# Banus/pano360

Hardware: AMD Instinct MI355X
Metric: blended megapixels/sec (multiband) (higher is better)
Workload: dtype f32; 1 GPU; cfg3: 32 synthetic 3840x2160 frames per image set, spherical warp + multiband blend L=5, native resolution (MAX_RESOLUTION uncapped); frames=32

## Files before the change

include/pano360.h:

```cpp
#ifndef PANO360_H
#define PANO360_H

#include <stddef.h>
#include <stdint.h>

#ifdef __cplusplus
extern "C" {
#endif

#define PANO_OK 0
#define PANO_EINVAL (-1)
#define PANO_EHIP (-2)
#define PANO_ELIMIT (-3)
#define PANO_ESOLVE (-4)

#define PANO_MAX_TAPS 129
#define PANO_MAX_LEVELS 8
#define PANO_TAP_LEAD 7
#define PANO_TAP_PAD 40
#ifndef PANO_INTERIOR_BLOCK
#define PANO_INTERIOR_BLOCK 4
#endif

typedef struct pano_patch {
    float *planes;
    uint8_t *mask;
    float *blurred;
    float *scratch;
    int32_t y0, x0, h, w;
    int32_t vy0, vx0, vh, vw;
    int32_t ay0, ax0, ah, aw;
    int32_t vpitch, apitch;
    int32_t index;
    int32_t tiles_off;
} pano_patch;

typedef struct pano_layout {
    int64_t planes_floats;
    int64_t blurred_floats;
    int64_t scratch_floats;
    int32_t n_records, n_tiles;
    int32_t max_vw, max_vh, max_aw, max_ah;
    int32_t missing;
} pano_layout;

typedef struct pano_camera {
    double proj[9];
    const uint8_t *frame;
    const double *hat_x;
    const double *hat_y;
    int32_t sh, sw;
    int32_t y0, x0, h, w;
} pano_camera;

typedef struct pano_pair {
    double minv[9];
    int32_t i, j;
} pano_pair;

typedef struct pano_sift_keypoint {
    float x, y;
    float size;
    float angle;
    float response;
    int32_t octave;
    int32_t r, c;
} pano_sift_keypoint;


const char *pano_version(void);
const char *pano_last_error(void);
int pano_device_count(void);
int pano_pitch(int w);
int pano_interior_block(void);

typedef struct pano_ctx pano_ctx;
#define PANO_OPT_BLUR_KERNEL 0
#define PANO_OPT_OWN_PRUNE 1
#define PANO_OPT_BLUR_SEGMENTS 2
#define PANO_OPT_BLUR_LEAN 3
#define PANO_OPT_STITCH_STREAMS 4
#define PANO_OPT_STITCH_ASYNC 5
#define PANO_OPT_BLUR_SEG_LEN 6
#define PANO_OPT_SIFT_GRAPH 7
#define PANO_OPT_LEVEL_CLASSES 8
#define PANO_OPT_COUNT 9
#define PANO_BLUR_MFMA 0
#define PANO_BLUR_VALU 1
int pano_ctx_create(int device, void *stream, pano_ctx **out);
int pano_ctx_destroy(pano_ctx *ctx);
int pano_ctx_set_stream(pano_ctx *ctx, void *stream);
int pano_ctx_set_option(pano_ctx *ctx, int option, int value);
int pano_ctx_get_option(const pano_ctx *ctx, int option, int *value);

int pano_timing_enable(pano_ctx *ctx, int on);
int pano_kernel_count(void);
const char *pano_kernel_name(int kid);
int pano_timing_read(pano_ctx *ctx, int kid, double *total_ms, int *launches);

int pano_add_weights(pano_ctx *ctx, const uint8_t *frame, int h, int w,
                     const float *lut255, const double *hat_x, const double *hat_y,
                     float *rgba);

int pano_warp_spherical(pano_ctx *ctx, const uint8_t *frame, int sh, int sw,
                        const double *proj, const double *sin_t, const double *cos_t,
                        const double *tan_p, const float *lut255, const double *hat_x,
                        const double *hat_y, int gx0, int gy0, int pw, int ph,
                        float *planes, uint8_t *mask, float *map_x, float *map_y);

int pano_warp_windows(pano_ctx *ctx, const pano_camera *cams, const pano_patch *patches,
                      int n, int max_vw, int max_vh, const double *sin_t,
                      const double *cos_t, const double *tan_p, const float *lut,
                      int lut_stride, const uint8_t *need);

int pano_ownership(pano_ctx *ctx, const pano_patch *patches, int n, int H, int W,
                   int16_t *owner, uint8_t *valid);

int pano_ownership_cameras(pano_ctx *ctx, const pano_camera *cams, int n, int H, int W,
                           int xs0, int xs1, const double *sin_t, const double *cos_t,
                           const double *tan_p, int16_t *owner, uint8_t *valid);

int pano_owned_regions(pano_ctx *ctx, const int16_t *owner, int H, int W, int xs0, int xs1,
                       int n, int min_gap, int max_spans, uint8_t *marks,
                       int32_t *regions);

int pano_ownership_regions(pano_ctx *ctx, const pano_camera *cams, int n, int H, int W,
                           int xs0, int xs1, const double *sin_t, const double *cos_t,
                           const double *tan_p, int16_t *owner, uint8_t *valid,
                           int min_gap, int max_spans, uint8_t *marks, int32_t *regions);

int pano_blur_tile_grid(const pano_ctx *ctx);
int pano_blur_tiles(pano_ctx *ctx, const pano_patch *patches, int n, int max_aw,
                    int max_ah, int W, int radius, const uint8_t *interior,
                    uint8_t *tile_flags, uint8_t *warp_need);
int pano_multiband_blur_prepare(pano_ctx *ctx, const pano_patch *patches, int n,
                                int max_aw, int max_ah, int W, const uint8_t *interior,
                                uint8_t *tile_flags);
int pano_multiband_blur(pano_ctx *ctx, const pano_patch *patches, int n, int max_aw,
                        int max_vh, int max_ah, const int16_t *owner, int W,
                        const float *taps, const int *ntaps, int n_blur,
                        const uint8_t *interior, uint8_t *tile_flags);

int pano_interior_map(pano_ctx *ctx, const int16_t *owner, int H, int W, int xs0, int xs1,
                      int radius, int16_t *block_owner, uint8_t *interior);
int pano_interior_classes(pano_ctx *ctx, const int16_t *owner, int H, int W, int xs0, int xs1,
                          const int *radii, int n_radii, int16_t *block_owner, uint8_t *interior,
                          uint8_t *classes);

int pano_layout_windows(int tile_grid, const int32_t *regions, int n, int max_spans,
                        const int32_t *rects, const uint8_t *have, int radius,
                        int xs0, int xs1, int n_blur, pano_patch *records, int cap,
                        pano_layout *out);
int pano_layout_place(pano_patch *records, int n_records, void *planes, void *blurred,
                      void *scratch);

int pano_multiband_compose(pano_ctx *ctx, const pano_patch *patches, int n, int H, int W,
                           int xs0, int xs1, int n_levels, const int16_t *owner,
                           const uint8_t *valid, const uint8_t *interior,
                           const uint8_t *classes, const pano_camera *cams,
                           const double *sin_t, const double *cos_t, const double *tan_p,
                           const float *lut, int lut_stride, uint8_t *mosaic,
                           float *mosaic_f32);

int pano_blend_cameras(pano_ctx *ctx, const pano_camera *cams, int n, int H, int W,
                       int xs0, int xs1, int linear, const double *sin_t,
                       const double *cos_t, const double *tan_p, const float *lut,
                       int lut_stride, uint8_t *mosaic, uint8_t *valid);

int pano_overlap_blocks(int h, int w);
int pano_overlap_stats(pano_ctx *ctx, const pano_camera *cams, const pano_pair *pairs,
                       int n_pairs, int h, int w, int bw0, const float *lut255,
                       double *partials, double *stats);

int pano_linear_blend(pano_ctx *ctx, const pano_patch *patches, int n, int H, int W,
                      uint8_t *mosaic);

int pano_no_blend(pano_ctx *ctx, const pano_patch *patches, int n, int H, int W,
                  uint8_t *mosaic);

int pano_crop_rect(pano_ctx *ctx, const uint8_t *valid, int H, int W, int32_t *heights,
                   int64_t *result);

int pano_blur_plane(pano_ctx *ctx, const float *src, float *dst, float *tmp, int h, int w,
                    int pitch, const float *taps, int ntaps);

int pano_pyr_down(pano_ctx *ctx, const float *src, int h, int w, float *dst);

int pano_gray_u8(pano_ctx *ctx, const uint8_t *bgr, int h, int w, float *out);
int pano_scale_step(pano_ctx *ctx, const float *src, int h, int w, const float *taps, int ntaps,
                    float *dst, float *dog);
int pano_scale_space(pano_ctx *ctx, const uint8_t *frame, int h, int w, int n_octaves,
                     int n_layers, const float *taps, const int *ntaps, float *const *gauss,
                     float *const *dog, float *work);
int pano_resize_up2(pano_ctx *ctx, const float *src, int h, int w, float *dst);
int pano_decimate2(pano_ctx *ctx, const float *src, int h, int w, float *dst);
int pano_subtract(pano_ctx *ctx, const float *a, const float *b, size_t n, float *out);

int pano_pyr_down_image(pano_ctx *ctx, const void *src, int h, int w, int c, int is_f64,
                        void *dst);
int pano_pyr_up_image(pano_ctx *ctx, const void *src, int sh, int sw, int c, int is_f64,
                      const void *other, int mode, void *dst, int oh, int ow);
int pano_u8_to_f32(pano_ctx *ctx, const uint8_t *src, size_t n, float *dst);
int pano_laplacian_mix(pano_ctx *ctx, const float *la, const float *lb, const void *gm, size_t n,
                       int is_f64, void *out);
int pano_clip_u8(pano_ctx *ctx, const void *src, size_t n, int is_f64, uint8_t *dst);

#define PANO_POISSON_CHUNK 32
int pano_poisson_blend(pano_ctx *ctx, const uint8_t *src, uint8_t *tgt, const uint8_t *mask,
                       int h, int w, int c, double rtol, int max_iters, double *solution,
                       int32_t *iters, double *resid);

#define PANO_SEAM_U8 0
#define PANO_SEAM_I16 1
#define PANO_SEAM_I32 2
#define PANO_SEAM_F32 3
#define PANO_SEAM_F64 4
#define PANO_SEAM_RESIDENT_CELLS 81408
#define PANO_SEAM_BATCH 64
int pano_seam_levels(pano_ctx *ctx, const void *img1, const void *img2, int dtype, int h, int w,
                     int c, int shrink, int16_t *level, int32_t *bad);
int pano_seam_flood(pano_ctx *ctx, const int16_t *level, int rows, int cols, int border,
                    int path, int8_t *labels, int32_t *stats);
int pano_seam_mask(pano_ctx *ctx, const int8_t *labels, int rows, int cols,
                   const int32_t *xtab, const int32_t *ytab, uint8_t *mask, int h, int w);
int pano_alpha_blend(pano_ctx *ctx, const void *img1, const void *img2, int dtype,
                     const void *mask, int mask_f64, int64_t mask_sy, int64_t mask_sx,
                     int64_t mask_sc, int h, int w, int c, uint8_t *out);

int pano_resize_u8(pano_ctx *ctx, const uint8_t *src, int sh, int sw, int c,
                   const int32_t *xtab, const int32_t *ytab, uint8_t *dst, int oh, int ow);

int pano_sift_extrema(pano_ctx *ctx, const float *dog, int rows, int cols, int octave,
                      int n_layers, float contrast_thr, float edge_thr, float sigma,
                      pano_sift_keypoint *cands, int *count, int max_cands);
int pano_sift_orient(pano_ctx *ctx, const float *const *gauss, const int *dims,
                     int n_layers, const pano_sift_keypoint *cands, const int *n_cands,
                     int max_cands, pano_sift_keypoint *kpts, int *count, int max_kpts);
int pano_sift_describe(pano_ctx *ctx, const float *const *gauss, const int *dims,
                       int first_octave, const pano_sift_keypoint *kpts, int n,
                       const int *n_dev, float *desc);
size_t pano_sift_sort_work_bytes(int n);
int pano_sift_sort_unique(pano_ctx *ctx, const pano_sift_keypoint *kpts, int n, const int *n_dev,
                          int first_octave, void *work, pano_sift_keypoint *out, int *n_out);

typedef struct pano_sift_args {
    const uint8_t *frame;
    uint8_t *frame_copy;
    int32_t h, w, n_octaves, n_layers;
    const float *taps;
    const int32_t *ntaps;
    float *const *gauss;
    float *const *dog;
    float *work;
    int32_t detect;
    float contrast_thr, edge_thr, sigma;
    int32_t first_octave, max_keypoints;
    const float *const *gauss_dev;
    const int32_t *dims_dev;
    pano_sift_keypoint *cands, *kpts;
    int32_t *counts;
    void *sort_work;
    float *desc;
} pano_sift_args;
int pano_sift_detect(pano_ctx *ctx, const pano_sift_args *args);
int pano_sift_detect_replaying(const pano_ctx *ctx);

size_t pano_knn2_work_bytes(int nq, int nt, int d);
int pano_knn2(pano_ctx *ctx, const float *query, int nq, const float *train, int nt, int d,
              float scale, void *work, int32_t *idx, float *dist, int *rescans);

int pano_match_pack(pano_ctx *ctx, const int32_t *idx, const float *dist, int nq, double ratio,
                    const float *kp_query, const float *kp_train, int nt, float *pts,
                    int32_t *match, int32_t *count);

size_t pano_hom_ransac_work_bytes(int n_pairs, int max_iters);
int pano_hom_ransac(pano_ctx *ctx, const float *pts, const int32_t *offsets, const int32_t *counts,
                    int n_pairs, int max_iters, float thresh, uint64_t seed, void *work,
                    double *hom, uint8_t *mask, int32_t *n_inliers, int32_t *hyp_inliers);

size_t pano_ba_work_bytes(int n_pairs);
int pano_ba_residuals(pano_ctx *ctx, const double *rows, const int32_t *pairs, int n_pairs,
                      const double *hom, double *ssq);
int pano_ba_normal(pano_ctx *ctx, const double *rows, const int32_t *pairs, int n_pairs,
                   const int32_t *slot, int n_active, const double *jtab, const double *hom_r,
                   double lambda, void *work, double *jtj, double *jtr);

#define PANO_JPEG_FIELDS 32
#define PANO_JPEG_CHUNK 1024
#define PANO_JPEG_SUBSEQ 1024
#define PANO_JPEG_HUFF_BYTES 1424
enum {
    PANO_JD_W, PANO_JD_H, PANO_JD_NC, PANO_JD_HMAX, PANO_JD_VMAX, PANO_JD_MCUX, PANO_JD_MCUY,
    PANO_JD_RI,
    PANO_JD_NINT,
    PANO_JD_BPM,
    PANO_JD_ORIENT, PANO_JD_DATA_OFF, PANO_JD_DATA_LEN, PANO_JD_TAB_OFF,
    PANO_JD_CHUNK0,
    PANO_JD_INT0,
    PANO_JD_SUB0,
    PANO_JD_BLK0, PANO_JD_PIX0,
    PANO_JD_DST_OFF,
    PANO_JD_PLANE0, PANO_JD_PLANE1, PANO_JD_PLANE2,
    PANO_JD_PITCH0, PANO_JD_PITCH1, PANO_JD_PITCH2,
    PANO_JD_OUT_OFF,
    PANO_JD_COMP_U,
    PANO_JD_SAMP,
    PANO_JD_TABSEL
};
enum {
    PANO_JB_N, PANO_JB_CHUNKS, PANO_JB_INTS, PANO_JB_SUBS, PANO_JB_BLOCKS, PANO_JB_PIXELS,
    PANO_JB_OUT_BYTES, PANO_JB_W_KEPT, PANO_JB_W_RST, PANO_JB_W_KEPTX, PANO_JB_W_RSTX,
    PANO_JB_W_DSTLEN, PANO_JB_W_ISTART, PANO_JB_W_IEND, PANO_JB_W_INSUB, PANO_JB_W_ISUBX,
    PANO_JB_W_STATE0, PANO_JB_W_STATE1, PANO_JB_W_CNTX, PANO_JB_W_FLAG, PANO_JB_W_COEF,
    PANO_JB_WORK_BYTES, PANO_JB_PACKED_BYTES
};
int pano_jpeg_decode(pano_ctx *ctx, const int64_t *desc, int n, const uint8_t *packed,
                     int64_t packed_bytes, void *work, int64_t work_bytes, uint8_t *out,
                     int64_t out_bytes);

#define PANO_JPEG_MAX_SIDE 65500
#define PANO_JPEG_BGR 1
size_t pano_jpeg_encode_work_bytes(int h, int w, int subsampling);
int pano_jpeg_encode(pano_ctx *ctx, const uint8_t *img, int h, int w, int64_t pitch, int flags,
                     int subsampling, const uint8_t *qt, void *work, int64_t work_bytes,
                     const uint8_t **stream, int64_t *stream_bytes);

#define PANO_EGROW 1
typedef struct pano_stitch_args {
    const pano_camera *cams;
    const int32_t *rects;
    const uint8_t *have;
    const double *sin_t, *cos_t, *tan_p;
    const float *lut;
    const float *taps;
    const int32_t *ntaps;
    int16_t *owner;
    uint8_t *valid;
    uint8_t *marks;
    int32_t *regions;
    int32_t *regions_host;
    int16_t *block_owner;
    uint8_t *interior;
    pano_patch *records_host;
    pano_patch *table;
    float *planes, *blurred, *scratch;
    uint8_t *tile_flags, *need;
    uint8_t *mosaic;
    float *mosaic_f32;
    int64_t planes_floats, blurred_floats, scratch_floats;
    int32_t n, H, W, xs0, xs1, own0, own1;
    int32_t lut_stride, n_levels, radius, shortcut, warp_need, max_spans, min_gap;
    int32_t cap_records, cap_tiles;
    int32_t used_need;
    int32_t trust_layout;
    uint8_t *classes;
    pano_layout layout;
} pano_stitch_args;
int pano_stitch_multiband(pano_ctx *ctx, pano_stitch_args *args, int resume);
int pano_stitch_verify(pano_ctx *ctx);
int pano_stitch_counts(const pano_ctx *ctx, int *device_layouts, int *fallbacks);

#ifdef __cplusplus
}
#endif
#endif
```

pano360_amd/_lib.py:

```python
import ctypes as C
import os
import subprocess

_HERE = os.path.dirname(os.path.abspath(__file__))
LIB_PATH = os.environ.get("PANO_LIB") or os.path.join(_HERE, "libpano360_hip.so")

MAX_TAPS = 129
MAX_LEVELS = 8
TAP_LEAD = 7
TAP_PAD = 40
OPT_BLUR_KERNEL, OPT_OWN_PRUNE, OPT_BLUR_SEGMENTS, OPT_BLUR_LEAN, OPT_STITCH_STREAMS = 0, 1, 2, 3, 4
OPT_STITCH_ASYNC = 5
OPT_BLUR_SEG_LEN = 6
OPT_SIFT_GRAPH = 7
OPT_LEVEL_CLASSES = 8
BLUR_MFMA, BLUR_VALU = 0, 1


class PanoError(RuntimeError):
    """A C-ABI call returned a negative status."""


class Patch(C.Structure):
    _fields_ = [("planes", C.c_void_p), ("mask", C.c_void_p),
                ("blurred", C.c_void_p), ("scratch", C.c_void_p),
                ("y0", C.c_int32), ("x0", C.c_int32), ("h", C.c_int32), ("w", C.c_int32),
                ("vy0", C.c_int32), ("vx0", C.c_int32), ("vh", C.c_int32), ("vw", C.c_int32),
                ("ay0", C.c_int32), ("ax0", C.c_int32), ("ah", C.c_int32), ("aw", C.c_int32),
                ("vpitch", C.c_int32), ("apitch", C.c_int32),
                ("index", C.c_int32), ("tiles_off", C.c_int32)]


class Layout(C.Structure):
    _fields_ = [("planes_floats", C.c_int64), ("blurred_floats", C.c_int64),
                ("scratch_floats", C.c_int64), ("n_records", C.c_int32), ("n_tiles", C.c_int32),
                ("max_vw", C.c_int32), ("max_vh", C.c_int32), ("max_aw", C.c_int32),
                ("max_ah", C.c_int32), ("missing", C.c_int32)]


class SiftArgs(C.Structure):
    _fields_ = [("frame", C.c_void_p), ("frame_copy", C.c_void_p),
                ("h", C.c_int32), ("w", C.c_int32), ("n_octaves", C.c_int32), ("n_layers", C.c_int32),
                ("taps", C.c_void_p), ("ntaps", C.c_void_p), ("gauss", C.c_void_p),
                ("dog", C.c_void_p), ("work", C.c_void_p), ("detect", C.c_int32),
                ("contrast_thr", C.c_float), ("edge_thr", C.c_float), ("sigma", C.c_float),
                ("first_octave", C.c_int32), ("max_keypoints", C.c_int32),
                ("gauss_dev", C.c_void_p), ("dims_dev", C.c_void_p), ("cands", C.c_void_p),
                ("kpts", C.c_void_p), ("counts", C.c_void_p), ("sort_work", C.c_void_p),
                ("desc", C.c_void_p)]


class StitchArgs(C.Structure):
    _fields_ = ([(k, C.c_void_p) for k in (
        "cams", "rects", "have", "sin_t", "cos_t", "tan_p", "lut", "taps", "ntaps", "owner",
        "valid", "marks", "regions", "regions_host", "block_owner", "interior", "records_host",
        "table", "planes", "blurred", "scratch", "tile_flags", "need", "mosaic", "mosaic_f32")]
        + [(k, C.c_int64) for k in ("planes_floats", "blurred_floats", "scratch_floats")]
        + [(k, C.c_int32) for k in (
            "n", "H", "W", "xs0", "xs1", "own0", "own1", "lut_stride", "n_levels", "radius",
            "shortcut", "warp_need", "max_spans", "min_gap", "cap_records", "cap_tiles",
            "used_need", "trust_layout")]
        + [("classes", C.c_void_p), ("layout", Layout)])


EINVAL = -1
ESOLVE = -4
SEAM_DTYPES = {"uint8": 0, "int16": 1, "int32": 2, "float32": 3, "float64": 4}
SEAM_RESIDENT_CELLS = 81408
EGROW = 1


class Pair(C.Structure):
    _fields_ = [("minv", C.c_double * 9), ("i", C.c_int32), ("j", C.c_int32)]


class SiftKeypoint(C.Structure):
    _fields_ = [("x", C.c_float), ("y", C.c_float), ("size", C.c_float), ("angle", C.c_float),
                ("response", C.c_float), ("octave", C.c_int32), ("r", C.c_int32), ("c", C.c_int32)]


class Camera(C.Structure):
    _fields_ = [("proj", C.c_double * 9), ("frame", C.c_void_p),
                ("hat_x", C.c_void_p), ("hat_y", C.c_void_p),
                ("sh", C.c_int32), ("sw", C.c_int32),
                ("y0", C.c_int32), ("x0", C.c_int32), ("h", C.c_int32), ("w", C.c_int32)]


_vp, _i = C.c_void_p, C.c_int
_SIGNATURES = {
    "pano_version": (C.c_char_p, []),
    "pano_last_error": (C.c_char_p, []),
    "pano_device_count": (_i, []),
    "pano_pitch": (_i, [_i]),
    "pano_interior_block": (_i, []),
    "pano_ctx_create": (_i, [_i, _vp, C.POINTER(C.c_void_p)]),
    "pano_ctx_destroy": (_i, [_vp]),
    "pano_ctx_set_stream": (_i, [_vp, _vp]),
    "pano_ctx_set_option": (_i, [_vp, _i, _i]),
    "pano_ctx_get_option": (_i, [_vp, _i, C.POINTER(C.c_int)]),
    "pano_timing_enable": (_i, [_vp, _i]),
    "pano_kernel_count": (_i, []),
    "pano_kernel_name": (C.c_char_p, [_i]),
    "pano_timing_read": (_i, [_vp, _i, C.POINTER(C.c_double), C.POINTER(C.c_int)]),
    "pano_add_weights": (_i, [_vp, _vp, _i, _i, _vp, _vp, _vp, _vp]),
    "pano_warp_spherical": (_i, [_vp, _vp, _i, _i, _vp, _vp, _vp, _vp, _vp, _vp, _vp, _i, _i, _i,
                                 _i, _vp, _vp, _vp, _vp]),
    "pano_warp_windows": (_i, [_vp, _vp, _vp, _i, _i, _i, _vp, _vp, _vp, _vp, _i, _vp]),
    "pano_blur_tiles": (_i, [_vp, _vp, _i, _i, _i, _i, _i, _vp, _vp, _vp]),
    "pano_ownership": (_i, [_vp, _vp, _i, _i, _i, _vp, _vp]),
    "pano_ownership_cameras": (_i, [_vp, _vp, _i, _i, _i, _i, _i, _vp, _vp, _vp, _vp, _vp]),
    "pano_owned_regions": (_i, [_vp, _vp, _i, _i, _i, _i, _i, _i, _i, _vp, _vp]),
    "pano_ownership_regions": (_i, [_vp, _vp, _i, _i, _i, _i, _i, _vp, _vp, _vp, _vp, _vp,
                                    _i, _i, _vp, _vp]),
    "pano_multiband_blur": (_i, [_vp, _vp, _i, _i, _i, _i, _vp, _i, _vp, C.POINTER(C.c_int), _i,
                                 _vp, _vp]),
    "pano_multiband_blur_prepare": (_i, [_vp, _vp, _i, _i, _i, _i, _vp, _vp]),
    "pano_layout_windows": (_i, [_i, _vp, _i, _i, _vp, _vp, _i, _i, _i, _i, _vp, _i, _vp]),
    "pano_layout_place": (_i, [_vp, _i, _vp, _vp, _vp]),
    "pano_interior_map": (_i, [_vp, _vp, _i, _i, _i, _i, _i, _vp, _vp]),
    "pano_interior_classes": (_i, [_vp, _vp, _i, _i, _i, _i, _vp, _i, _vp, _vp, _vp]),
    "pano_multiband_compose": (_i, [_vp, _vp, _i, _i, _i, _i, _i, _i, _vp, _vp, _vp, _vp, _vp, _vp,
                                    _vp, _vp, _vp, _i, _vp, _vp]),
    "pano_blend_cameras": (_i, [_vp, _vp, _i, _i, _i, _i, _i, _i, _vp, _vp, _vp, _vp, _i, _vp,
                                _vp]),
    "pano_blur_tile_grid": (_i, [_vp]),
    "pano_overlap_blocks": (_i, [_i, _i]),
    "pano_overlap_stats": (_i, [_vp, _vp, _vp, _i, _i, _i, _i, _vp, _vp, _vp]),
    "pano_linear_blend": (_i, [_vp, _vp, _i, _i, _i, _vp]),
    "pano_no_blend": (_i, [_vp, _vp, _i, _i, _i, _vp]),
    "pano_crop_rect": (_i, [_vp, _vp, _i, _i, _vp, _vp]),
    "pano_blur_plane": (_i, [_vp, _vp, _vp, _vp, _i, _i, _i, _vp, _i]),
    "pano_pyr_down": (_i, [_vp, _vp, _i, _i, _vp]),
    "pano_gray_u8": (_i, [_vp, _vp, _i, _i, _vp]),
    "pano_scale_step": (_i, [_vp, _vp, _i, _i, _vp, _i, _vp, _vp]),
    "pano_scale_space": (_i, [_vp, _vp, _i, _i, _i, _i, _vp, _vp, _vp, _vp, _vp]),
    "pano_resize_up2": (_i, [_vp, _vp, _i, _i, _vp]),
    "pano_decimate2": (_i, [_vp, _vp, _i, _i, _vp]),
    "pano_subtract": (_i, [_vp, _vp, _vp, C.c_size_t, _vp]),
    "pano_pyr_down_image": (_i, [_vp, _vp, _i, _i, _i, _i, _vp]),
    "pano_pyr_up_image": (_i, [_vp, _vp, _i, _i, _i, _i, _vp, _i, _vp, _i, _i]),
    "pano_u8_to_f32": (_i, [_vp, _vp, C.c_size_t, _vp]),
    "pano_laplacian_mix": (_i, [_vp, _vp, _vp, _vp, C.c_size_t, _i, _vp]),
    "pano_clip_u8": (_i, [_vp, _vp, C.c_size_t, _i, _vp]),
    "pano_poisson_blend": (_i, [_vp, _vp, _vp, _vp, _i, _i, _i, C.c_double, _i, _vp, _vp, _vp]),
    "pano_seam_levels": (_i, [_vp, _vp, _vp, _i, _i, _i, _i, _i, _vp, _vp]),
    "pano_seam_flood": (_i, [_vp, _vp, _i, _i, _i, _i, _vp, _vp]),
    "pano_seam_mask": (_i, [_vp, _vp, _i, _i, _vp, _vp, _vp, _i, _i]),
    "pano_alpha_blend": (_i, [_vp, _vp, _vp, _i, _vp, _i, C.c_int64, C.c_int64, C.c_int64, _i, _i,
                              _i, _vp]),
    "pano_resize_u8": (_i, [_vp, _vp, _i, _i, _i, _vp, _vp, _vp, _i, _i]),
    "pano_sift_extrema": (_i, [_vp, _vp, _i, _i, _i, _i, C.c_float, C.c_float, C.c_float, _vp,
                               _vp, _i]),
    "pano_sift_orient": (_i, [_vp, _vp, _vp, _i, _vp, _vp, _i, _vp, _vp, _i]),
    "pano_sift_describe": (_i, [_vp, _vp, _vp, _i, _vp, _i, _vp, _vp]),
    "pano_sift_sort_work_bytes": (C.c_size_t, [_i]),
    "pano_sift_sort_unique": (_i, [_vp, _vp, _i, _vp, _i, _vp, _vp, _vp]),
    "pano_knn2_work_bytes": (C.c_size_t, [_i, _i, _i]),
    "pano_knn2": (_i, [_vp, _vp, _i, _vp, _i, _i, C.c_float, _vp, _vp, _vp, _vp]),
    "pano_hom_ransac_work_bytes": (C.c_size_t, [_i, _i]),
    "pano_hom_ransac": (_i, [_vp, _vp, _vp, _vp, _i, _i, C.c_float, C.c_uint64, _vp, _vp, _vp, _vp,
                             _vp]),
    "pano_match_pack": (_i, [_vp, _vp, _vp, _i, C.c_double, _vp, _vp, _i, _vp, _vp, _vp]),
    "pano_ba_work_bytes": (C.c_size_t, [_i]),
    "pano_ba_residuals": (_i, [_vp, _vp, _vp, _i, _vp, _vp]),
    "pano_ba_normal": (_i, [_vp, _vp, _vp, _i, _vp, _i, _vp, _vp, C.c_double, _vp, _vp, _vp]),
    "pano_jpeg_decode": (_i, [_vp, _vp, _i, _vp, C.c_int64, _vp, C.c_int64, _vp, C.c_int64]),
    "pano_jpeg_encode_work_bytes": (C.c_size_t, [_i, _i, _i]),
    "pano_jpeg_encode": (_i, [_vp, _vp, _i, _i, C.c_int64, _i, _i, _vp, _vp, C.c_int64,
                             C.POINTER(C.c_void_p), C.POINTER(C.c_int64)]),
    "pano_sift_detect": (_i, [_vp, _vp]),
    "pano_sift_detect_replaying": (_i, [_vp]),
    "pano_stitch_multiband": (_i, [_vp, _vp, _i]),
    "pano_stitch_counts": (_i, [_vp, _vp, _vp]),
    "pano_stitch_verify": (_i, [_vp]),
}
EXPORTS = tuple(_SIGNATURES)


def sources_digest():
    import hashlib
    src = os.path.join(_HERE, "csrc")
    files = sorted(os.path.join(src, f) for f in os.listdir(src)
                   if f.endswith((".hip", ".h", ".inc")) or f == "Makefile")
    files.append(os.path.join(os.path.dirname(_HERE), "include", "pano360.h"))
    h = hashlib.sha256()
    for path in files:
        if not os.path.exists(path):
            continue
        h.update(os.path.basename(path).encode() + b"\0")
        with open(path, "rb") as fid:
            h.update(fid.read())
    return h.hexdigest()


BUILD_RECORD = os.path.join(_HERE, "csrc", ".build_stamp")


def build(force=False):
    import json
    src = os.path.join(_HERE, "csrc")
    digest = sources_digest()
    have = None
    try:
        with open(BUILD_RECORD) as fid:
            have = json.load(fid).get("sources_sha256")
    except (OSError, ValueError):
        pass
    full = force or have != digest or not os.path.exists(LIB_PATH)
    before = os.path.getmtime(LIB_PATH) if os.path.exists(LIB_PATH) else None
    cmd = ["make", "-C", src, "-s", "-j4"] + (["-B"] if full else [])
    subprocess.check_call(cmd)
    after = os.path.getmtime(LIB_PATH)
    mode = "full" if full else ("incremental" if after != before else "up to date")
    with open(BUILD_RECORD, "w") as fid:
        json.dump({"sources_sha256": digest, "mode": mode}, fid)
    return LIB_PATH


_lib = None


def lib():
    global _lib
    if _lib is None:
        if not os.path.exists(LIB_PATH):
            raise PanoError(
                f"{LIB_PATH} is missing: build it with "
                "`python -c 'import __graft_entry__ as g; g.build()'` "
                "(there is no CPU fallback)")
        import torch
        handle = C.CDLL(LIB_PATH)
        for name, (res, args) in _SIGNATURES.items():
            fn = getattr(handle, name)
            fn.restype, fn.argtypes = res, args
        _lib = handle
    return _lib


def check(status, what):
    if status != 0:
        msg = lib().pano_last_error().decode("utf-8", "replace")
        raise PanoError(f"{what} failed ({status}): {msg}")
```

pano360_amd/csrc/api.hip:

```cpp
#include <stdarg.h>
#include <stdio.h>
#include <stdlib.h>
#include <string.h>

#include <vector>

#include "common.h"
#include "layout.h"

static thread_local char g_error[512] = "";

void pano_set_error(const char *fmt, ...) {
    va_list ap;
    va_start(ap, fmt);
    vsnprintf(g_error, sizeof(g_error), fmt, ap);
    va_end(ap);
}

extern "C" const char *pano_version(void) { return "pano360_hip 0.1 (gfx950)"; }

extern "C" const char *pano_last_error(void) { return g_error; }

extern "C" int pano_device_count(void) {
    int n = 0;
    if (hipGetDeviceCount(&n) != hipSuccess) {
        (void)hipGetLastError();
        return 0;
    }
    return n;
}

extern "C" int pano_pitch(int w) { return pano_pitch_of(w); }

extern "C" int pano_interior_block(void) { return PANO_INTERIOR_BLOCK; }

extern "C" int pano_ctx_create(int device, void *stream, pano_ctx **out) {
    PANO_REQUIRE(out, "pano_ctx_create: null output");
    *out = nullptr;
    PANO_REQUIRE(device >= 0 && device < pano_device_count(), "pano_ctx_create: no device %d",
                 device);
    PANO_HIP(hipSetDevice(device));
    if (int rc = pano_blur_mfma_opt_in()) return rc;
    if (int rc = pano_blur_valu_opt_in()) return rc;
    pano_ctx *ctx = new pano_ctx();
    ctx->device = device;
    ctx->stream = (hipStream_t)stream;
    ctx->opt[PANO_OPT_BLUR_KERNEL] = PANO_BLUR_MFMA;
    ctx->opt[PANO_OPT_OWN_PRUNE] = 1;
    ctx->opt[PANO_OPT_BLUR_SEGMENTS] = 1;
    ctx->opt[PANO_OPT_BLUR_LEAN] = 1;
    ctx->opt[PANO_OPT_STITCH_STREAMS] = 1;
    ctx->opt[PANO_OPT_STITCH_ASYNC] = 0;
    ctx->opt[PANO_OPT_BLUR_SEG_LEN] = 0;
    ctx->opt[PANO_OPT_SIFT_GRAPH] = 1;
    ctx->opt[PANO_OPT_LEVEL_CLASSES] = 0;
    *out = ctx;
    return PANO_OK;
}

int pano_ctx_enter(pano_ctx *ctx) {
    if (!ctx->in_stitch) ctx->geom_valid = false;
    PANO_HIP(hipSetDevice(ctx->device));
    return PANO_OK;
}

static void timing_clear(pano_ctx *ctx) {
    for (int k = 0; k < PK_COUNT; ++k) {
        for (hipEvent_t e : ctx->t_begin[k]) (void)hipEventDestroy(e);
        for (hipEvent_t e : ctx->t_end[k]) (void)hipEventDestroy(e);
        ctx->t_begin[k].clear();
        ctx->t_end[k].clear();
    }
}

static void tap_set_free(PanoTapSet &ts) {
    if (ts.taps) (void)hipFree(ts.taps);
    if (ts.tables) (void)hipFree(ts.tables);
    if (ts.ready) (void)hipEventDestroy(ts.ready);
    free(ts.host);
    ts.taps = nullptr;
    ts.tables = nullptr;
    ts.ready = nullptr;
    ts.host = nullptr;
}

extern "C" int pano_ctx_destroy(pano_ctx *ctx) {
    if (!ctx) return PANO_OK;
    PANO_HIP(hipSetDevice(ctx->device));
    if (hipStreamSynchronize(ctx->stream) != hipSuccess) {
        (void)hipGetLastError();
        (void)hipDeviceSynchronize();
    }
    timing_clear(ctx);
    for (PanoTapSet &ts : ctx->tap_sets) tap_set_free(ts);
    if (ctx->item_buf) (void)hipFree(ctx->item_buf);
    if (ctx->item_counter) (void)hipFree(ctx->item_counter);
    if (ctx->sift_raw) (void)hipFree(ctx->sift_raw);
    if (ctx->enc_dev) (void)hipFree(ctx->enc_dev);
    if (ctx->enc_out) (void)hipFree(ctx->enc_out);
    if (ctx->enc_host) (void)hipHostFree(ctx->enc_host);
    if (ctx->poisson_dev) (void)hipFree(ctx->poisson_dev);
    if (ctx->poisson_host) (void)hipHostFree(ctx->poisson_host);
    if (ctx->seam_dev) (void)hipFree(ctx->seam_dev);
    if (ctx->seam_host) (void)hipHostFree(ctx->seam_host);
    pano_sift_graphs_free(ctx);
    if (ctx->lay_sum_host) (void)hipHostFree(ctx->lay_sum_host);
    if (ctx->lay_rects_dev) (void)hipFree(ctx->lay_rects_dev);
    if (ctx->lay_have_dev) (void)hipFree(ctx->lay_have_dev);
    if (ctx->side) {
        (void)hipStreamSynchronize(ctx->side);
        (void)hipStreamDestroy(ctx->side);
    }
    if (ctx->ev_fork) (void)hipEventDestroy(ctx->ev_fork);
    if (ctx->ev_join) (void)hipEventDestroy(ctx->ev_join);
    if (ctx->ev_regions) (void)hipEventDestroy(ctx->ev_regions);
    if (ctx->ev_upload) (void)hipEventDestroy(ctx->ev_upload);
    if (ctx->ev_copy) (void)hipEventDestroy(ctx->ev_copy);
    delete ctx;
    return PANO_OK;
}

int pano_ctx_side_stream(pano_ctx *ctx) {
    if (!ctx->ev_regions) PANO_HIP(hipEventCreateWithFlags(&ctx->ev_regions, hipEventDisableTiming));
    if (!ctx->ev_upload) PANO_HIP(hipEventCreateWithFlags(&ctx->ev_upload, hipEventDisableTiming));
    if (!ctx->ev_fork) PANO_HIP(hipEventCreateWithFlags(&ctx->ev_fork, hipEventDisableTiming));
    if (!ctx->ev_join) PANO_HIP(hipEventCreateWithFlags(&ctx->ev_join, hipEventDisableTiming));
    if (!ctx->ev_copy) PANO_HIP(hipEventCreateWithFlags(&ctx->ev_copy, hipEventDisableTiming));
    if (!ctx->side) PANO_HIP(hipStreamCreateWithFlags(&ctx->side, hipStreamNonBlocking));
    return PANO_OK;
}

extern "C" int pano_ctx_set_stream(pano_ctx *ctx, void *stream) {
    PANO_REQUIRE(ctx, "pano_ctx_set_stream: null context");
    if ((hipStream_t)stream != ctx->stream) ctx->geom_valid = false;
    ctx->stream = (hipStream_t)stream;
    return PANO_OK;
}

extern "C" int pano_ctx_set_option(pano_ctx *ctx, int option, int value) {
    PANO_REQUIRE(ctx, "pano_ctx_set_option: null context");
    PANO_REQUIRE(option >= 0 && option < PANO_OPT_COUNT, "pano_ctx_set_option: option %d", option);
    if (option == PANO_OPT_BLUR_KERNEL)
        PANO_REQUIRE(value == PANO_BLUR_MFMA || value == PANO_BLUR_VALU,
                     "pano_ctx_set_option: blur kernel %d", value);
    else if (option == PANO_OPT_STITCH_ASYNC)
        PANO_REQUIRE(value >= 0 && value <= 2, "pano_ctx_set_option: option %d takes 0, 1 or 2", option);
    else if (option == PANO_OPT_OWN_PRUNE)
        PANO_REQUIRE(value >= 0 && value <= 3, "pano_ctx_set_option: option %d takes 0 .. 3", option);
    else if (option == PANO_OPT_BLUR_SEG_LEN)
        PANO_REQUIRE(value == -1 || value == 0 || (value >= 4 && value <= 2047),
                     "pano_ctx_set_option: option %d takes -1, 0 or 4 .. 2047", option);
    else
        PANO_REQUIRE(value == 0 || value == 1, "pano_ctx_set_option: option %d takes 0 or 1", option);
    const bool changed = ctx->opt[option] != value;
    ctx->opt[option] = value;
    ctx->prepared_table = ctx->flags_table = ctx->list_table = nullptr;
    ctx->geom_valid = false;
    if (changed && option == PANO_OPT_BLUR_KERNEL)
        ctx->lay_prev_valid = ctx->lay_prev_verified = false;
    return PANO_OK;
}

extern "C" int pano_ctx_get_option(const pano_ctx *ctx, int option, int *value) {
    PANO_REQUIRE(ctx && value, "pano_ctx_get_option: null pointer");
    PANO_REQUIRE(option >= 0 && option < PANO_OPT_COUNT, "pano_ctx_get_option: option %d", option);
    *value = ctx->opt[option];
    return PANO_OK;
}

static uint64_t tap_hash(const float *taps, const int *ntaps, int n, size_t floats) {
    uint64_t h = 1469598103934665603ull;
    auto eat = [&](const void *p, size_t bytes) {
        const unsigned char *b = (const unsigned char *)p;
        for (size_t i = 0; i < bytes; ++i) h = (h ^ b[i]) * 1099511628211ull;
    };
    eat(&n, sizeof(n));
    eat(ntaps, n * sizeof(int));
    eat(taps, floats * sizeof(float));
    return h;
}

#define PANO_TAP_SETS_MAX 64
int pano_ctx_tap_set(pano_ctx *ctx, const float *taps, const int *ntaps, int n, size_t table_bytes,
                     PanoTapSet **out, bool *fresh) {
    size_t floats = 0;
    for (int k = 0; k < n; ++k) floats += (size_t)ntaps[k] + PANO_TAP_PAD;
    const uint64_t key = tap_hash(taps, ntaps, n, floats);
    *fresh = false;
    for (PanoTapSet &ts : ctx->tap_sets)
        if (ts.key == key && ts.n == n && !memcmp(ts.ntaps, ntaps, n * sizeof(int)) &&
            ts.floats == floats && !memcmp(ts.host, taps, floats * sizeof(float))) {
            ts.used = ++ctx->tick;
            if (ctx->stream != ts.built_on) PANO_HIP(hipStreamWaitEvent(ctx->stream, ts.ready, 0));
            if (table_bytes && !ts.tables) {
                PANO_HIP(hipMalloc((void **)&ts.tables, table_bytes));
                *fresh = true;
            }
            *out = &ts;
            return PANO_OK;
        }
    if (ctx->tap_sets.size() >= PANO_TAP_SETS_MAX) {
        size_t old = 0;
        for (size_t i = 1; i < ctx->tap_sets.size(); ++i)
            if (ctx->tap_sets[i].used < ctx->tap_sets[old].used) old = i;
        PANO_HIP(hipDeviceSynchronize());
        tap_set_free(ctx->tap_sets[old]);
        ctx->tap_sets.erase(ctx->tap_sets.begin() + old);
    }
    PanoTapSet ts = {};
    ts.key = key;
    ts.n = n;
    memcpy(ts.ntaps, ntaps, n * sizeof(int));
    ts.floats = floats;
    ts.host = (float *)malloc(floats * sizeof(float));
    PANO_REQUIRE(ts.host, "pano_ctx_tap_set: out of host memory");
    memcpy(ts.host, taps, floats * sizeof(float));
    PANO_HIP(hipMalloc((void **)&ts.taps, floats * sizeof(float)));
    PANO_HIP(hipMemcpyAsync(ts.taps, taps, floats * sizeof(float), hipMemcpyHostToDevice,
                            ctx->stream));
    PANO_HIP(hipEventCreateWithFlags(&ts.ready, hipEventDisableTiming));
    PANO_HIP(hipEventRecord(ts.ready, ctx->stream));
    ts.built_on = ctx->stream;
    if (table_bytes) {
        PANO_HIP(hipMalloc((void **)&ts.tables, table_bytes));
        *fresh = true;
    }
    ts.used = ++ctx->tick;
    ctx->tap_sets.push_back(ts);
    *out = &ctx->tap_sets.back();
    return PANO_OK;
}

int pano_ctx_tap_set_built(pano_ctx *ctx, PanoTapSet *set) {
    PANO_HIP(hipEventRecord(set->ready, ctx->stream));
    set->built_on = ctx->stream;
    return PANO_OK;
}

static const char *const g_kernel_names[] = {
    "add_weights_kernel", "warp_spherical_kernel", "ownership_kernel", "blur_rows_kernel",
    "blur_cols_kernel",   "multiband_compose_kernel", "linear_blend_kernel",
    "no_blend_kernel",    "crop_heights_kernel", "crop_rows_kernel", "pyr_down_kernel",
    "ownership_cameras_kernel", "owned_boxes_kernel", "warp_windows_kernel",
    "blend_cameras_kernel", "owned_spans_kernel",
    "block_owner_kernel", "tile_flags_kernel", "overlap_stats_kernel",
    "blur_mfma_kernel", "sift_extrema_kernel", "sift_orient_kernel", "sift_describe_kernel",
    "scale_step_kernel", "knn2_kernel", "blur_lean_kernel", "blur_lean5_kernel",
    "ransac_score_kernel", "ransac_finish_kernel", "match_pack_kernel",
    "ba_residual_kernel", "ba_pair_kernel", "ba_assemble_kernel",
    "jpeg_destuff_kernel", "jpeg_scan_kernel", "jpeg_intervals_kernel", "jpeg_huff_sync_kernel",
    "jpeg_huff_write_kernel", "jpeg_dc_kernel", "jpeg_idct_kernel", "jpeg_pixels_kernel",
    "jpeg_enc_blocks_kernel", "jpeg_enc_count_kernel", "jpeg_enc_scan_kernel", "jpeg_enc_emit_kernel",
    "jpeg_enc_stuff_kernel"};
static_assert(sizeof(g_kernel_names) / sizeof(g_kernel_names[0]) == PK_COUNT,
              "one name per PanoKernelId, in enum order");

void pano_timing_edge(pano_ctx *ctx, int kid, hipStream_t stream, bool begin) {
    hipEvent_t ev;
    if (hipEventCreate(&ev) != hipSuccess) return;
    (void)hipEventRecord(ev, stream);
    (begin ? ctx->t_begin : ctx->t_end)[kid].push_back(ev);
}

extern "C" int pano_timing_enable(pano_ctx *ctx, int on) {
    PANO_REQUIRE(ctx, "pano_timing_enable: null context");
    timing_clear(ctx);
    ctx->timing_on = on != 0;
    return PANO_OK;
}

extern "C" int pano_kernel_count(void) { return PK_COUNT; }

extern "C" const char *pano_kernel_name(int kid) {
    return kid >= 0 && kid < PK_COUNT ? g_kernel_names[kid] : "";
}

extern "C" int pano_timing_read(pano_ctx *ctx, int kid, double *total_ms, int *launches) {
    PANO_REQUIRE(ctx && kid >= 0 && kid < PK_COUNT && total_ms && launches,
                 "pano_timing_read: bad argument");
    double sum = 0.0;
    const size_t nb = ctx->t_begin[kid].size(), ne = ctx->t_end[kid].size();
    const size_t n = ne < nb ? ne : nb;
    for (size_t i = 0; i < n; ++i) {
        PANO_HIP(hipEventSynchronize(ctx->t_end[kid][i]));
        float ms = 0.f;
        PANO_HIP(hipEventElapsedTime(&ms, ctx->t_begin[kid][i], ctx->t_end[kid][i]));
        sum += ms;
    }
    *total_ms = sum;
    *launches = (int)n;
    return PANO_OK;
}

extern "C" int pano_layout_windows(int tile_grid, const int32_t *regions, int n, int max_spans,
                                   const int32_t *rects, const uint8_t *have, int radius,
                                   int xs0, int xs1, int n_blur, pano_patch *records, int cap,
                                   pano_layout *out) {
    PANO_REQUIRE(regions && rects && records && out, "pano_layout_windows: null pointer");
    PANO_REQUIRE(tile_grid == 0 || tile_grid == 32, "pano_layout_windows: tile grid %d", tile_grid);
    PANO_REQUIRE(n >= 0 && max_spans >= 1 && radius >= 0 && n_blur >= 0 && cap >= 0,
                 "pano_layout_windows: bad argument");
    const bool grid32 = tile_grid == 32;
    const int stride = 5 + 2 * max_spans;
    pano_layout lay = {};
    lay.missing = 0;
    long planes = 0, blurred = 0, scratch = 0, tiles = 0;
    int k = 0;
    for (int i = 0; i < n; ++i) {
        const int32_t *rg = regions + (size_t)i * stride;
        const int spans = rg[4] < max_spans ? rg[4] : max_spans;
        for (int sp = 0; sp < spans; ++sp) {
            pano_patch rec;
            LayoutSizes sz;
            if (!layout_record(rg, sp, rects + 4 * i, i, radius, xs0, xs1, n_blur, grid32, rec, sz))
                continue;
            PANO_REQUIRE(k < cap, "pano_layout_windows: more than %d records", cap);
            if (have && !have[i]) ++lay.missing;
            pano_patch &r = records[k++];
            r = rec;
            PANO_REQUIRE(layout_record_fits(r),
                         "pano_layout_windows: a plane of record %d exceeds 2 GiB", k - 1);
            r.planes = (float *)(uintptr_t)planes;
            r.blurred = (float *)(uintptr_t)(blurred + sz.lead);
            r.scratch = (float *)(uintptr_t)scratch;
            PANO_REQUIRE(tiles < (1l << 31), "pano_layout_windows: tile count overflow");
            r.tiles_off = (int)tiles;
            planes += sz.planes;
            blurred += sz.blurred;
            scratch += sz.scratch;
            tiles += sz.tiles;
            lay.max_vw = r.vw > lay.max_vw ? r.vw : lay.max_vw;
            lay.max_vh = r.vh > lay.max_vh ? r.vh : lay.max_vh;
            lay.max_aw = r.aw > lay.max_aw ? r.aw : lay.max_aw;
            lay.max_ah = r.ah > lay.max_ah ? r.ah : lay.max_ah;
        }
    }
    lay.n_records = k;
    lay.n_tiles = (int)tiles;
    lay.planes_floats = planes;
    lay.blurred_floats = blurred + 32;
    lay.scratch_floats = scratch;
    *out = lay;
    return PANO_OK;
}

extern "C" int pano_layout_place(pano_patch *records, int n_records, void *planes, void *blurred,
                                 void *scratch) {
    PANO_REQUIRE(records || n_records == 0, "pano_layout_place: null pointer");
    uintptr_t bbase = (uintptr_t)blurred;
    bbase += (uintptr_t)(-(intptr_t)bbase) % 128;
    for (int k = 0; k < n_records; ++k) {
        pano_patch &r = records[k];
        r.planes = (float *)planes + (uintptr_t)r.planes;
        r.blurred = blurred ? (float *)bbase + (uintptr_t)r.blurred : nullptr;
        r.scratch = scratch ? (float *)scratch + (uintptr_t)r.scratch : nullptr;
    }
    return PANO_OK;
}
```

pano360_amd/csrc/blur.hip:

```cpp
#include "common.h"

#define ROW_TW 512
#define ROW_RMAX 64
#define ROW_TILE (ROW_TW + 2 * ROW_RMAX + 16)
#define ROW_LDS (ROW_TILE + (ROW_TILE / 8) * 4 + 8)

#define COL_TW 64
#define COL_TH 128
#define COL_STEPS(ntaps) (((ntaps) + 7 + 7) & ~7)

struct LevelDesc {
    const float *wz;
    int ntaps;
    int start;
    int steps;
};

struct Levels {
    LevelDesc lv[PANO_MAX_LEVELS];
    int n;
    int rmax;
    int need;
};

// ... 34 lines not shown
    const int y = blockIdx.y * 4 + wv;
    const int yc = y < p.vh ? y : p.vh - 1;
    float *tile = s_row[wv];
    const float *__restrict__ src =
        c == alpha_ch ? nullptr : p.planes + (size_t)c * p.vh * p.vpitch;
    const int16_t *__restrict__ orow =
        owner + (size_t)(p.y0 + p.vy0 + yc) * W + p.x0;

    for (int i0 = lane; i0 < L.need; i0 += 256) {
        float v[4];
#pragma unroll
        for (int u = 0; u < 4; ++u) {
            const int i = i0 + 64 * u < L.need ? i0 + 64 * u : L.need - 1;
            const int pcol = reflect_101(p.ax0 + xt - L.rmax + i, p.w);
            if (src) {
                int vc = pcol - p.vx0;
                vc = vc < 0 ? 0 : (vc >= p.vw ? p.vw - 1 : vc);
                v[u] = src[(size_t)yc * p.vpitch + vc];
            } else {
                v[u] = orow[pcol] == p.index ? 1.0f : 0.0f;
            }
        }
#pragma unroll
        for (int u = 0; u < 4; ++u)
            if (i0 + 64 * u < L.need) tile[row_pos(i0 + 64 * u)] = v[u];
    }
    __syncthreads();

    const float *base = tile + 12 * lane;
    const int x = xt + 8 * lane;
    for (int k = 0; k < L.n; ++k) {
        const kptr_f32 wz = (kptr_f32)(uintptr_t)L.lv[k].wz;
        const int start = L.lv[k].start, steps = L.lv[k].steps;
        float acc[8];
#pragma unroll
        for (int o = 0; o < 8; ++o) acc[o] = 0.0f;
        for (int s = 0; s < steps; s += 2) {
            const int q0 = start + 4 * s, q1 = q0 + 4;
            const float4 va = *(const float4 *)(base + q0 + ((q0 >> 3) << 2));
            const float4 vb = *(const float4 *)(base + q1 + ((q1 >> 3) << 2));
            float wq[15];
#pragma unroll
            for (int j = 0; j < 15; ++j) wq[j] = wz[4 * s + j];
            const float in[8] = {va.x, va.y, va.z, va.w, vb.x, vb.y, vb.z, vb.w};
#pragma unroll
            for (int i = 0; i < 8; ++i) {
#pragma unroll
                for (int o = 0; o < 8; ++o)
                    acc[o] = __builtin_fmaf(wq[i + 7 - o], in[i], acc[o]);
            }
        }
        if (y < p.vh) {
            float *d = p.scratch + ((size_t)(k * nch + c) * p.vh + y) * p.apitch + x;
            if (x + 8 <= p.apitch) {
                *(float4 *)d = make_float4(acc[0], acc[1], acc[2], acc[3]);
                *(float4 *)(d + 4) = make_float4(acc[4], acc[5], acc[6], acc[7]);
            } else {
#pragma unroll
                for (int o = 0; o < 8; ++o)
                    if (x + o < p.aw) d[o] = acc[o];
            }
        }
    }
}

struct ColTrip {
    float w[15];
    float4 v[8];
};

__device__ __forceinline__ void col_trip_load(ColTrip &t, const float *base, kptr_f32 wz, int q) {
#pragma unroll
    for (int j = 0; j < 15; ++j) t.w[j] = wz[q + j];
#pragma unroll
    for (int s = 0; s < 8; ++s) t.v[s] = *(const float4 *)(base + (q + s) * COL_TW);
}

__device__ __forceinline__ void col_trip_fma(const ColTrip &t, float4 (&acc)[8]) {
#pragma unroll
    for (int s = 0; s < 8; ++s) {
#pragma unroll
        for (int o = 0; o < 8; ++o) {
            const float wgt = t.w[s + 7 - o];
            acc[o].x = __builtin_fmaf(wgt, t.v[s].x, acc[o].x);
            acc[o].y = __builtin_fmaf(wgt, t.v[s].y, acc[o].y);
            acc[o].z = __builtin_fmaf(wgt, t.v[s].z, acc[o].z);
            acc[o].w = __builtin_fmaf(wgt, t.v[s].w, acc[o].w);
        }
    }
}

template <bool TABLE>
__global__ __launch_bounds__(256) void blur_cols_kernel(
    const pano_patch *__restrict__ table, pano_patch single, int nch, int level,
    const float *wz_global, int ntaps, const uint8_t *__restrict__ flags) {
    const kptr_f32 wz = (kptr_f32)(uintptr_t)wz_global;
    extern __shared__ __attribute__((aligned(16))) float s_col[];
    const int pid = blockIdx.z / nch, c = blockIdx.z - pid * nch;
    const pano_patch p = TABLE ? table[pid] : single;
    const int x0 = blockIdx.x * COL_TW, y0 = blockIdx.y * COL_TH;
    if (x0 >= p.aw || y0 >= p.ah) return;
    if (p.h > 2 * (ntaps >> 1) + 2 && !col_tile_active(flags, p, blockIdx.x, blockIdx.y)) return;

    const float *__restrict__ src = p.scratch + (size_t)(level * nch + c) * p.vh * p.apitch;
    float *__restrict__ dst = p.blurred + (size_t)(level * nch + c) * p.ah * p.apitch;
    const int tx = threadIdx.x, ty = threadIdx.y;
    const int R = ntaps >> 1;
    const int steps = COL_STEPS(ntaps);
    const int rows = 8 * 15 + steps;
    const int x = x0 + 4 * tx;

    const int xl = x < p.apitch ? x : p.apitch - 4;
    const int wave4 = (ty >> 2) << 2;
    for (int r0 = 0; r0 < rows; r0 += 16) {
        const int r = r0 + ty;
        int vr = reflect_101(p.ay0 + y0 - R + (r < rows ? r : rows - 1), p.h) - p.vy0;
        vr = vr < 0 ? 0 : (vr >= p.vh ? p.vh - 1 : vr);
        __builtin_amdgcn_global_load_lds(
            (const __attribute__((address_space(1))) void *)(src + (size_t)vr * p.apitch + xl),
            (__attribute__((address_space(3))) void *)(s_col + (r0 + wave4) * COL_TW), 16, 0, 0);
    }
    __syncthreads();

    float4 acc[8];
#pragma unroll
    for (int o = 0; o < 8; ++o) acc[o] = make_float4(0.f, 0.f, 0.f, 0.f);
    const float *base = s_col + (8 * ty) * COL_TW + 4 * tx;
    for (int q = 0; q < steps; q += 8) {
        ColTrip a;
        col_trip_load(a, base, wz, q);
        col_trip_fma(a, acc);
    }
    if (x < p.apitch) {
#pragma unroll
        for (int o = 0; o < 8; ++o) {
            const int y = y0 + 8 * ty + o;
            if (y < p.ah) *(float4 *)(dst + (size_t)y * p.apitch + x) = acc[o];
        }
    }
}

__global__ __launch_bounds__(64) void tile_flags_kernel(const pano_patch *__restrict__ table,
                                                        const uint8_t *__restrict__ interior,
                                                        int W8, uint8_t *__restrict__ flags) {
    const pano_patch p = table[blockIdx.z];
    const int ntx = (p.aw + COL_TW - 1) / COL_TW, nty = (p.ah + COL_TH - 1) / COL_TH;
    const int tx = blockIdx.x, ty = blockIdx.y;
    if (tx >= ntx || ty >= nty) return;
    const int gx0 = p.x0 + p.ax0 + tx * COL_TW, gy0 = p.y0 + p.ay0 + ty * COL_TH;
    int gx1 = gx0 + COL_TW, gy1 = gy0 + COL_TH;
    const int ax1 = p.x0 + p.ax0 + p.aw, ay1 = p.y0 + p.ay0 + p.ah;
    gx1 = gx1 < ax1 ? gx1 : ax1;
    gy1 = gy1 < ay1 ? gy1 : ay1;
    const int bx0 = gx0 / PANO_INTERIOR_BLOCK, bx1 = (gx1 - 1) / PANO_INTERIOR_BLOCK;
    const int by0 = gy0 / PANO_INTERIOR_BLOCK, by1 = (gy1 - 1) / PANO_INTERIOR_BLOCK;
    const int nbx = bx1 - bx0 + 1, total = nbx * (by1 - by0 + 1);
    bool active = false;
    for (int i = threadIdx.x; i < total; i += 64)
        active |= interior[(size_t)(by0 + i / nbx) * W8 + bx0 + i % nbx] == 0;
    if (__ballot(active) && threadIdx.x == 0) flags[p.tiles_off + ty * ntx + tx] = 1;
    if (!__ballot(active) && threadIdx.x == 0) flags[p.tiles_off + ty * ntx + tx] = 0;
}

static int check_taps(int ntaps, const char *who) {
    PANO_REQUIRE(ntaps >= 1 && (ntaps & 1) && ntaps <= PANO_MAX_TAPS,
                 "%s: aperture %d must be odd and within [1, %d]", who, ntaps, PANO_MAX_TAPS);
    return PANO_OK;
}

static int make_levels(const float *taps, const int *ntaps, int n_blur, Levels *L,
                       const float **col_wz, const char *who) {
    PANO_REQUIRE(n_blur >= 1 && n_blur < PANO_MAX_LEVELS, "%s: %d blur levels", who, n_blur);
    L->n = n_blur;
    L->rmax = 0;
    for (int k = 0; k < n_blur; ++k) {
        if (int rc = check_taps(ntaps[k], who)) return rc;
        if (ntaps[k] / 2 > L->rmax) L->rmax = ntaps[k] / 2;
    }
    L->need = 0;
    size_t off = 0;
    for (int k = 0; k < n_blur; ++k) {
        const int delta = L->rmax - ntaps[k] / 2, extra = delta & 3;
        L->lv[k].wz = taps + off;
        L->lv[k].ntaps = ntaps[k];
        L->lv[k].start = delta - extra;
        L->lv[k].steps = (((ntaps[k] + extra + 7 + 3) >> 2) + 1) & ~1;
        col_wz[k] = taps + off + extra;
        const int need = 8 * 63 + L->lv[k].start + 4 * L->lv[k].steps;
        if (need > L->need) L->need = need;
        off += (size_t)ntaps[k] + PANO_TAP_PAD;
    }
    PANO_REQUIRE(L->need <= ROW_TILE, "%s: row tile %d exceeds %d", who, L->need, ROW_TILE);
    return PANO_OK;
}

static int launch_blur(pano_ctx *ctx, const pano_patch *table, const pano_patch &single, int n,
                       int nch, int alpha_ch, int max_aw, int max_vh, int max_ah,
                       const int16_t *owner, int W, const float *host_taps, const int *ntaps,
                       int n_blur, const uint8_t *interior, uint8_t *tile_flags, const char *who) {
    const hipStream_t stream = ctx->stream;
    PanoTapSet *set = nullptr;
    bool fresh = false;
    if (int rc = pano_ctx_tap_set(ctx, host_taps, ntaps, n_blur, 0, &set, &fresh)) return rc;
    Levels L = {};
    const float *col_wz[PANO_MAX_LEVELS];
    if (int rc = make_levels(set->taps, ntaps, n_blur, &L, col_wz, who)) return rc;
    const uint8_t *flags = nullptr;
    if (interior && table) {
        dim3 grid(ceil_div(max_aw, COL_TW), ceil_div(max_ah, COL_TH), n);
        PANO_TIMED(PK_TILE_FLAGS, stream,
                   hipLaunchKernelGGL(tile_flags_kernel, grid, dim3(64), 0, stream, table, interior,
                                      ceil_div(W, PANO_INTERIOR_BLOCK), tile_flags));
        PANO_LAUNCH_CHECK("tile_flags_kernel");
        flags = tile_flags;
    }
    {
        dim3 block(64, 4), grid(ceil_div(max_aw, ROW_TW), ceil_div(max_vh, 4), n * nch);
        if (table)
            PANO_TIMED(PK_BLUR_ROWS, stream,
                       hipLaunchKernelGGL(blur_rows_kernel<true>, grid, block, 0, stream, table,
                                          single, nch, alpha_ch, L, owner, W, flags));
        else
            PANO_TIMED(PK_BLUR_ROWS, stream,
                       hipLaunchKernelGGL(blur_rows_kernel<false>, grid, block, 0, stream, table,
                                          single, nch, alpha_ch, L, owner, W, flags));
        PANO_LAUNCH_CHECK("blur_rows_kernel");
    }
    for (int k = 0; k < n_blur; ++k) {
        const int rows = (8 * 15 + COL_STEPS(ntaps[k]) + 15) & ~15;
        const size_t lds = (size_t)rows * COL_TW * sizeof(float);
        dim3 block(16, 16), grid(ceil_div(max_aw, COL_TW), ceil_div(max_ah, COL_TH), n * nch);
#define LAUNCH_COLS(T)                                                                 \
    PANO_TIMED(PK_BLUR_COLS, stream,                                                   \
               hipLaunchKernelGGL(blur_cols_kernel<T>, grid, block, lds, stream, table, \
                                  single, nch, k, col_wz[k], ntaps[k], flags))
        if (table) LAUNCH_COLS(true); else LAUNCH_COLS(false);
#undef LAUNCH_COLS
        PANO_LAUNCH_CHECK("blur_cols_kernel");
    }
    return PANO_OK;
}

int pano_blur_valu_opt_in(void) {
    const void *fns[] = {(const void *)blur_cols_kernel<true>,
                         (const void *)blur_cols_kernel<false>};
    for (const void *fn : fns)
        PANO_HIP(hipFuncSetAttribute(fn, hipFuncAttributeMaxDynamicSharedMemorySize, 160 * 1024));
    return PANO_OK;
}

extern "C" int pano_blur_plane(pano_ctx *ctx, const float *src, float *dst, float *tmp, int h,
                               int w, int pitch, const float *taps, int ntaps) {
    PANO_ENTER(ctx, "pano_blur_plane");
    PANO_REQUIRE(src && dst && tmp && taps, "pano_blur_plane: null pointer");
    PANO_REQUIRE(h > 0 && w > 0 && pitch >= w && (pitch & 3) == 0,
                 "pano_blur_plane: bad shape %dx%d pitch %d", h, w, pitch);
    if (int rc = check_taps(ntaps, "pano_blur_plane")) return rc;
    pano_patch p = {};
    p.planes = const_cast<float *>(src);
    p.scratch = tmp;
    p.blurred = dst;
    p.h = p.vh = p.ah = h;
    p.w = p.vw = p.aw = w;
    p.vpitch = p.apitch = pitch;
    return launch_blur(ctx, nullptr, p, 1, 1, -1, w, h, h, nullptr, 0, taps, &ntaps, 1, nullptr,
                       nullptr, "pano_blur_plane");
}

extern "C" int pano_blur_tile_grid(const pano_ctx *ctx) {
    return ctx && !pano_blur_uses_mfma(ctx) ? 0 : 32;
}

extern "C" int pano_multiband_blur(pano_ctx *ctx, const pano_patch *patches, int n, int max_aw,
                                   int max_vh, int max_ah, const int16_t *owner, int W,
                                   const float *taps, const int *ntaps, int n_blur,
                                   const uint8_t *interior, uint8_t *tile_flags) {
    PANO_ENTER(ctx, "pano_multiband_blur");
    PANO_REQUIRE(patches && owner && taps && ntaps, "pano_multiband_blur: null pointer");
    PANO_REQUIRE(n >= 0 && n <= 32767 && W > 0, "pano_multiband_blur: bad argument");
    PANO_REQUIRE(max_aw >= 0 && max_vh >= 0 && max_ah >= 0, "pano_multiband_blur: bad extents");
    PANO_REQUIRE(!interior || tile_flags, "pano_multiband_blur: interior map without tile_flags");
    if (n == 0 || n_blur == 0 || max_aw == 0 || max_vh == 0 || max_ah == 0) return PANO_OK;
    PANO_REQUIRE(n_blur >= 1 && n_blur < PANO_MAX_LEVELS, "pano_multiband_blur: %d blur levels", n_blur);
    for (int k = 0; k < n_blur; ++k)
        if (int rc = check_taps(ntaps[k], "pano_multiband_blur")) return rc;
    if (pano_blur_uses_mfma(ctx))
        return pano_launch_blur_mfma(ctx, patches, n, max_aw, max_ah, owner, W, taps, ntaps, n_blur,
                                     interior, tile_flags);
    pano_patch none = {};
    return launch_blur(ctx, patches, none, n, 4, 3, max_aw, max_vh, max_ah, owner, W, taps, ntaps,
                       n_blur, interior, tile_flags, "pano_multiband_blur");
}

extern "C" int pano_blur_tiles(pano_ctx *ctx, const pano_patch *patches, int n, int max_aw,
                               int max_ah, int W, int radius, const uint8_t *interior,
                               uint8_t *tile_flags, uint8_t *warp_need) {
    PANO_ENTER(ctx, "pano_blur_tiles");
    PANO_REQUIRE(patches && interior && tile_flags, "pano_blur_tiles: null pointer");
    PANO_REQUIRE(n >= 0 && n <= 32767 && W > 0 && max_aw >= 0 && max_ah >= 0 && radius >= 0,
                 "pano_blur_tiles: bad argument");
    PANO_REQUIRE(pano_blur_uses_mfma(ctx), "pano_blur_tiles: needs the 32 x 32 tile grid");
    if (n == 0 || max_aw == 0 || max_ah == 0) return PANO_OK;
    return pano_tiles_blur_mfma(ctx, patches, n, max_aw, max_ah, W, radius, interior, tile_flags,
                                warp_need);
}

extern "C" int pano_multiband_blur_prepare(pano_ctx *ctx, const pano_patch *patches, int n,
                                           int max_aw, int max_ah, int W,
                                           const uint8_t *interior, uint8_t *tile_flags) {
    PANO_ENTER(ctx, "pano_multiband_blur_prepare");
    PANO_REQUIRE(patches, "pano_multiband_blur_prepare: null pointer");
    PANO_REQUIRE(n >= 0 && n <= 32767 && W > 0 && max_aw >= 0 && max_ah >= 0,
                 "pano_multiband_blur_prepare: bad argument");
    PANO_REQUIRE(!interior || tile_flags,
                 "pano_multiband_blur_prepare: interior map without tile_flags");
    if (n == 0 || max_aw == 0 || max_ah == 0 || !pano_blur_uses_mfma(ctx)) return PANO_OK;
    return pano_prepare_blur_mfma(ctx, patches, n, max_aw, max_ah, W, interior, tile_flags);
}

__global__ __launch_bounds__(256) void pyr_down_kernel(const float *__restrict__ src,
                                                       int h, int w,
                                                       float *__restrict__ dst,
                                                       int oh, int ow) {
    const int x = blockIdx.x * 64 + threadIdx.x, y = blockIdx.y * 4 + threadIdx.y;
    if (x >= ow || y >= oh) return;
    int cx[5], cy[5];
#pragma unroll
    for (int k = 0; k < 5; ++k) {
        cx[k] = reflect_101(2 * x - 2 + k, w);
        cy[k] = reflect_101(2 * y - 2 + k, h);
    }
    float rowv[5];
#pragma unroll
    for (int k = 0; k < 5; ++k) {
        const float *s = src + (size_t)cy[k] * w;
        rowv[k] = s[cx[2]] * 6.0f + (s[cx[1]] + s[cx[3]]) * 4.0f + s[cx[0]] + s[cx[4]];
    }
    dst[(size_t)y * ow + x] =
        (rowv[2] * 6.0f + (rowv[1] + rowv[3]) * 4.0f + rowv[0] + rowv[4]) * (1.0f / 256.0f);
}

extern "C" int pano_pyr_down(pano_ctx *ctx, const float *src, int h, int w, float *dst) {
    PANO_ENTER(ctx, "pano_pyr_down");
    PANO_REQUIRE(src && dst, "pano_pyr_down: null pointer");
    PANO_REQUIRE(h > 0 && w > 0, "pano_pyr_down: bad shape %dx%d", h, w);
    const int oh = (h + 1) / 2, ow = (w + 1) / 2;
    dim3 block(64, 4), grid(ceil_div(ow, 64), ceil_div(oh, 4));
    PANO_TIMED(PK_PYR_DOWN, (hipStream_t)stream,
               hipLaunchKernelGGL(pyr_down_kernel, grid, block, 0, (hipStream_t)stream, src,
                                  h, w, dst, oh, ow));
    PANO_LAUNCH_CHECK("pyr_down_kernel");
    return PANO_OK;
}
```

pano360_amd/csrc/blur_mfma.hip:

```cpp
#include <stdlib.h>
#include <string.h>

#include <type_traits>

#include "common.h"

#if defined(__HIP_DEVICE_COMPILE__) && !defined(__gfx950__)
#error "blur_mfma.hip is written for gfx950 (MI355X): its inline-asm wait states are that chip's"
#endif

typedef _Float16 half8 __attribute__((ext_vector_type(8)));
typedef _Float16 half4 __attribute__((ext_vector_type(4)));
typedef short shortx4 __attribute__((ext_vector_type(4)));
typedef float f32x16 __attribute__((ext_vector_type(16)));
typedef short short8 __attribute__((ext_vector_type(8)));
typedef float float4u __attribute__((ext_vector_type(4), aligned(4)));
#define GLOBAL_AS __attribute__((address_space(1)))
typedef const GLOBAL_AS float *gcf32;
typedef GLOBAL_AS float *gf32;
typedef const GLOBAL_AS int16_t *gci16;
typedef const GLOBAL_AS float4u *gcf32x4;

#define MB_XT 64
#define MB_PITCH 168
// ... 1021 lines not shown
#pragma unroll
                        for (int m = 0; m < 3; ++m) {
                            if (m == 0 && first) {
                                f32x16 zero;
#pragma unroll
                                for (int q = 0; q < 16; ++q) zero[q] = 0.0f;
                                A[k] = __builtin_amdgcn_mfma_f32_32x32x16_f16(
                                    t_hi[buf], operand_b(m_hi[s2]), zero, 0, 0, 0);
                            } else {
                                A[k] = __builtin_amdgcn_mfma_f32_32x32x16_f16(
                                    m == 1 ? t_lo[buf] : t_hi[buf],
                                    operand_b(m == 2 ? m_lo[s2] : m_hi[s2]), A[k], 0, 0, 0);
                            }
                            MS_PIN();
                            const int hg = b * 3 + m;
                            if (s2 == 0) {
#pragma unroll
                                for (int c = 0; c < PAIRS_PER; ++c) {
                                    const int pr = hg * PAIRS_PER + c;
                                    if (pr < 4)
                                        ms_split2(mid[8 + 2 * pr], mid[9 + 2 * pr], mid_scale,
                                                  m_hi[1][pr], m_lo[1][pr]);
                                }
                            } else if (COMMIT) {
                                if (hg == 0)
                                    commit_wait(pf, std::integral_constant<int, stores_before_commit>{});
                                if (hg < 3) commit_piece(pf, okv, off_nxt, hg);
                            }
                            fill(G0 + KSL * PR + s2 * GAPS_H + hg);
                            if (LAST && s2 == 1 && hg == GAPS_H - 1) prepare_next();
                            MS_PIN();
                        }
                    }
                };
                level(std::integral_constant<int, C>{}, std::integral_constant<int, 0>{}, std::true_type{},
                      std::integral_constant<bool, CB == 0>{}, acc, s_tx, s_ty);
                if constexpr (CB != 0)
                    level(std::integral_constant<int, CB>{}, std::integral_constant<int, GR_A + GC_A>{},
                          std::false_type{}, std::true_type{}, acc_b, s_tx_b, s_ty_b);
            }
            MS_PIN();
        };
        block(std::true_type{});
        prev_store = (inf >> (DMAX + 2)) & 1u;
        prev_o = t - DMAX;
        prev_u = U;
        const bool run_on = more && band_of(next) == t + 1;
        word = next;
        next = nn;
        {
            const int tmp = off_cur;
            off_cur = off_nxt;
            off_nxt = tmp;
        }
        ++i;
        return run_on;
    };
    while (i < nlist) {
#pragma unroll
        for (int k = 0; k < NB; ++k)
#pragma unroll
            for (int q = 0; q < 16; ++q) {
                acc[k][q] = 0.0f;
                if (CB) acc_b[CB ? k : 0][q] = 0.0f;
            }
        for (;;) {
            if (!step(std::integral_constant<int, 0>{})) break;
            if (!step(std::integral_constant<int, 1>{})) break;
            if (!step(std::integral_constant<int, 2>{})) break;
            if constexpr (NB > 3) {
                if (!step(std::integral_constant<int, 3>{})) break;
                if (!step(std::integral_constant<int, 4>{})) break;
            }
        }
        if (prev_store) store_prev_generic();
        s_at = OOB;
        store_edge = false;
    }
}

template <bool FIVE>
__device__ __forceinline__ void lean_kernel_body(
    const pano_patch *__restrict__ table, const MbLevels &L, const unsigned char *__restrict__ tables,
    const int16_t *__restrict__ owner, int W, const uint8_t *__restrict__ flags,
    const int2 *__restrict__ items, unsigned char *smem) {
    constexpr int GROUP = 4;
    const int tid = threadIdx.x, wv = tid >> 6, lane = tid & 63;
    constexpr bool five = FIVE;
    const int ngroups = five ? 1 : (L.n + GROUP - 1) / GROUP;
    const int per = 8 * ngroups, blk = blockIdx.x / per, within = blockIdx.x - blk * per;
    const int grp = within >> 3, pair = blk * 8 + (within & 7);
    const int ch = pair & 3, slot = pair >> 2;
    const int2 item = items[slot];
    if (item.x < 0) return;
    const int pid = item.x & 0xffff, tx0 = item.x >> 16;
    const pano_patch p = table[pid];
    const MbGeom g = mb_geom(p);
    const int l0 = GROUP * grp, nl = five ? 5 : (L.n - l0 < GROUP ? L.n - l0 : GROUP);
    MbShared sh;
    sh.CM = 1;
    for (int k = 0; k < nl; ++k) {
        const int ck = mb_c_of(L.ntaps[l0 + k]);
        sh.CM = ck > sh.CM ? ck : sh.CM;
    }
    const int n_seg = item.y >> 16, seg = (item.y >> 12) & 15, nty_all = g.O1 - g.O0 + 1;
    const int o_begin = n_seg > 1 ? nty_all * seg / n_seg : 0;
    const int o_end = n_seg > 1 ? nty_all * (seg + 1) / n_seg : nty_all;
    const int q = __builtin_amdgcn_readfirstlane(wv >> 1);
    const int lv = mb_level_of_pair(nl, q);
    const bool live = lv >= 0;
    const int level = l0 + (live ? lv : 0);
    const int ntaps = L.ntaps[level], c = mb_c_of(ntaps);
    const int lv_b = mb_second_level_of_pair(nl, q);
    const int level_b = l0 + (lv_b >= 0 ? lv_b : 0);
    int dmax_of[GROUP], rel = 0, my_tx = 0, my_ty = 0, my_tx_b = 0, my_ty_b = 0;
    for (int k = 0; k < GROUP; ++k) {
        const int lk = mb_level_of_pair(nl, k);
        dmax_of[k] = -1;
        if (lk < 0) continue;
        const int ck = mb_c_of(L.ntaps[l0 + lk]);
        dmax_of[k] = (ck + 1) / 2;
        if (k == q) {
            my_tx = rel;
            my_ty = rel + mb_tx_bytes(2 + 2 * ck);
        }
        rel += mb_table_bytes(L.ntaps[l0 + lk]);
        const int lk2 = mb_second_level_of_pair(nl, k);
        if (lk2 >= 0) {
            const int ck2 = mb_c_of(L.ntaps[l0 + lk2]);
            if (k == q) {
                my_tx_b = rel;
                my_ty_b = rel + mb_tx_bytes(2 + 2 * ck2);
            }
            rel += mb_table_bytes(L.ntaps[l0 + lk2]);
        }
    }
    sh.P = mb_pitch_of(sh.CM);
    sh.hi = (_Float16 *)smem;
    sh.lo = sh.hi + 32 * sh.P;
    sh.need = (uint8_t *)(sh.lo + 32 * sh.P);
    sh.any = sh.need + 2 * MB_NEED_LEN;
    sh.info = (uint16_t *)(sh.any + MB_NEED_LEN);
    sh.col = (short *)(sh.info + 2 * MB_NEED_LEN);
    uint32_t *list = (uint32_t *)sh.info;
    my_tx += mb_fixed_bytes(sh.CM);
    my_ty += mb_fixed_bytes(sh.CM);
    my_tx_b += mb_fixed_bytes(sh.CM);
    my_ty_b += mb_fixed_bytes(sh.CM);
    const int dmaxm = (sh.CM + 1) / 2;
    sh.t_lo = g.O0 - dmaxm;
    sh.t_hi = g.O1 + dmaxm;
    for (int which = 0; which < (lv_b >= 0 ? 2 : 1); ++which)
    if (live) {
        const uint4 *from = (const uint4 *)(tables + L.tab_off[which ? level_b : level]);
        uint4 *to = (uint4 *)(smem + (which ? my_tx_b : my_tx));
        const int n16 = mb_table_bytes(L.ntaps[which ? level_b : level]) >> 4;
        constexpr int DEPTH = 8;
        for (int i0 = tid & 127; i0 < n16; i0 += 128 * DEPTH) {
            uint4 v[DEPTH];
#pragma unroll
            for (int j = 0; j < DEPTH; ++j) v[j] = from[min(i0 + 128 * j, n16 - 1)];
#pragma unroll
            for (int j = 0; j < DEPTH; ++j) to[min(i0 + 128 * j, n16 - 1)] = v[j];
        }
    }
    const int X0 = g.gx0 + 32 * tx0;
    const int nty = g.O1 - g.O0 + 1;
    if (wv < 2) {
        const int txg = ((X0 - g.gx0) >> 5) + wv;
        for (int i = lane; i < nty + 2 * MB_NEED_PAD; i += 64) {
            const int o = i - MB_NEED_PAD;
            bool v = txg < g.ntx && o >= o_begin && o < o_end;
            if (v && flags) v = flags[p.tiles_off + o * g.ntx + txg] != 0;
            sh.need[wv * MB_NEED_LEN + i] = v ? 1 : 0;
        }
    }
    int *const s_count = (int *)sh.any;
    __syncthreads();
    if (wv == 0) {
        int count = 0;
        for (int base = 0; base <= sh.t_hi - sh.t_lo; base += 64) {
            const int i = base + lane, t = sh.t_lo + i;
            const int o = t - g.O0 + MB_NEED_PAD;
            bool any = false;
            unsigned w = 0;
            if (i <= sh.t_hi - sh.t_lo) {
#pragma unroll
                for (int col = 0; col < 2; ++col)
#pragma unroll
                    for (int d = -2; d <= 2; ++d)
                        w |= (sh.need[col * MB_NEED_LEN + o - d] ? 1u : 0u) << (16 + 8 * col + d + 2);
                const unsigned reach_bits = dmaxm >= 2 ? 0x1fu : 0x0eu;
                any = (((w >> 16) | (w >> 24)) & reach_bits) != 0;
                w |= (unsigned)(unsigned short)(short)t;
            }
            const unsigned long long bal = __ballot(any);
            if (any) list[count + __popcll(bal & ((1ull << lane) - 1ull))] = w;
            count += __popcll(bal);
        }
        if (lane == 0) *s_count = count;
    }
    __syncthreads();
    const int nlist = *s_count;
    const half8 *s_tx = (const half8 *)(smem + my_tx), *s_ty = (const half8 *)(smem + my_ty);
    const int out_level = L.out[level];
    const int second = (mb_fixed_bytes(sh.CM) + rel + 15) / 16 * 8;
#define ML_BODY_FN ms_body
    const bool edge = mb_item_edge(p, g.gx0, tx0, sh.CM);
    if constexpr (FIVE)
    if (lv_b >= 0) {
        const half8 *s_tx_b = (const half8 *)(smem + my_tx_b), *s_ty_b = (const half8 *)(smem + my_ty_b);
#define MS_DUAL(SH, ED)                                                                        \
    ms_body<2, SH, 1, ED>(p, ch, out_level, live, s_tx, s_ty, sh, list, nlist, owner, W, tx0,  \
                          second, L.out[level_b], s_tx_b, s_ty_b)
        if (edge) {
            if (ch == 3) MS_DUAL(true, true); else MS_DUAL(false, true);
        } else {
            if (ch == 3) MS_DUAL(true, false); else MS_DUAL(false, false);
        }
#undef MS_DUAL
        return;
    }
    if (edge) {
        switch (c) {
#define MS_EDGE(CC)                                                                            \
    if (ch == 3)                                                                               \
        ms_body<CC, true, 0, true>(p, ch, out_level, live, s_tx, s_ty, sh, list, nlist, owner, W, tx0, second); \
    else                                                                                       \
        ms_body<CC, false, 0, true>(p, ch, out_level, live, s_tx, s_ty, sh, list, nlist, owner, W, tx0, second); \
    break;
            case 1: MS_EDGE(1)
            case 2: MS_EDGE(2)
            default: MS_EDGE(3)
#undef MS_EDGE
        }
        return;
    }
    switch (c) {
#define ML_BODY(CC)                                                                            \
    if (ch == 3)                                                                               \
        ML_BODY_FN<CC, true>(p, ch, out_level, live, s_tx, s_ty, sh, list, nlist, owner, W, tx0, second); \
    else                                                                                       \
        ML_BODY_FN<CC, false>(p, ch, out_level, live, s_tx, s_ty, sh, list, nlist, owner, W, tx0, second); \
    break;
        case 1: ML_BODY(1)
        case 2: ML_BODY(2)
        case 3: ML_BODY(3)
        default: ML_BODY(4)
#undef ML_BODY
    }
}

__global__ __launch_bounds__(MB_THREADS_OF(4), 1) void blur_lean_kernel(
    const pano_patch *__restrict__ table, MbLevels L, const unsigned char *__restrict__ tables,
    const int16_t *__restrict__ owner, int W, const uint8_t *__restrict__ flags,
    const int2 *__restrict__ items) {
    extern __shared__ __attribute__((aligned(16))) unsigned char smem[];
    lean_kernel_body<false>(table, L, tables, owner, W, flags, items, smem);
}

__global__ __launch_bounds__(MB_THREADS_OF(4), 1) void blur_lean5_kernel(
    const pano_patch *__restrict__ table, MbLevels L, const unsigned char *__restrict__ tables,
    const int16_t *__restrict__ owner, int W, const uint8_t *__restrict__ flags,
    const int2 *__restrict__ items) {
    extern __shared__ __attribute__((aligned(16))) unsigned char smem[];
    lean_kernel_body<true>(table, L, tables, owner, W, flags, items, smem);
}

__global__ __launch_bounds__(256) void tile_flags32_kernel(const pano_patch *__restrict__ table,
                                                           const uint8_t *__restrict__ interior,
                                                           int W8, uint8_t *__restrict__ flags) {
    const pano_patch p = table[blockIdx.z];
    if (p.aw <= 0 || p.ah <= 0) return;
    const MbGeom g = mb_geom(p);
    const int tx = blockIdx.x * 32 + (threadIdx.x & 31), ty = blockIdx.y * 8 + (threadIdx.x >> 5);
    if (tx >= g.ntx || ty > g.O1 - g.O0) return;
    int x0 = g.gx0 + 32 * tx, y0 = 32 * (g.O0 + ty), x1 = x0 + 32, y1 = y0 + 32;
    x0 = max(x0, p.ax0);
    y0 = max(y0, p.ay0);
    x1 = min(x1, p.ax0 + p.aw);
    y1 = min(y1, p.ay0 + p.ah);
    const int bx0 = (p.x0 + x0) / PANO_INTERIOR_BLOCK, bx1 = (p.x0 + x1 - 1) / PANO_INTERIOR_BLOCK;
    const int by0 = (p.y0 + y0) / PANO_INTERIOR_BLOCK, by1 = (p.y0 + y1 - 1) / PANO_INTERIOR_BLOCK;
    bool active = false;
    static_assert(PANO_INTERIOR_BLOCK == 4, "a 32-pixel tile spans at most nine interior blocks");
    if (bx0 + 8 <= W8) {
        typedef uint64_t u64_any __attribute__((aligned(1)));
        const int nb = bx1 - bx0 + 1;
        const uint64_t ones = nb >= 8 ? 0x0101010101010101ull : (0x0101010101010101ull >> (8 * (8 - nb)));
        for (int by = by0; by <= by1; ++by) {
            const uint8_t *row = interior + (size_t)by * W8 + bx0;
            active |= (*(const u64_any *)row & ones) != ones;
            if (nb == 9) active |= row[8] == 0;
        }
    } else {
        for (int by = by0; by <= by1; ++by)
            for (int bx = bx0; bx <= bx1; ++bx) active |= interior[(size_t)by * W8 + bx] == 0;
    }
    flags[p.tiles_off + ty * g.ntx + tx] = active ? 1 : 0;
}

__global__ __launch_bounds__(256) void warp_need_kernel(const pano_patch *__restrict__ table,
                                                        const uint8_t *__restrict__ flags, int hx,
                                                        int vy, uint8_t *__restrict__ need) {
    const pano_patch p = table[blockIdx.z];
    if (p.aw <= 0 || p.ah <= 0) return;
    const MbGeom g = mb_geom(p);
    const int nty = g.O1 - g.O0 + 1;
    const int tx = blockIdx.x * 32 + (threadIdx.x & 31), ty = blockIdx.y * 8 + (threadIdx.x >> 5);
    if (tx >= g.ntx || ty >= nty) return;
    bool any = false;
    for (int y = max(ty - vy, 0); y <= min(ty + vy, nty - 1) && !any; ++y)
        for (int x = max(tx - hx, 0); x <= min(tx + hx, g.ntx - 1) && !any; ++x)
            any = flags[p.tiles_off + y * g.ntx + x] != 0;
    need[p.tiles_off + ty * g.ntx + tx] = any ? 1 : 0;
}

#define MB_SORT_BINS 2048
__global__ __launch_bounds__(256) void mb_items_kernel(const pano_patch *__restrict__ table,
                                                       const uint8_t *__restrict__ flags,
                                                       int2 *__restrict__ items,
                                                       int *__restrict__ counter, int cap) {
    __shared__ int16_t s_start[1024];
    __shared__ unsigned long long s_any[4];
    __shared__ int s_base;
    const pano_patch p = table[blockIdx.x];
    const int tid = threadIdx.x, lane = tid & 63, wave = tid >> 6;
    if (p.aw <= 0 || p.ah <= 0) return;
    const MbGeom g = mb_geom(p);
    const int nty = g.O1 - g.O0 + 1;
    const uint8_t *rec = flags ? flags + p.tiles_off : nullptr;
    __shared__ uint8_t s_flags[16384];
    if (rec && nty * g.ntx <= (int)sizeof(s_flags)) {
        for (int i = tid; i < nty * g.ntx; i += 256) s_flags[i] = rec[i];
        __syncthreads();
        rec = s_flags;
    }
    int count = 0;
    bool covered = false;
    for (int c0 = 0; c0 < g.ntx; c0 += 64) {
        const int tx = c0 + lane;
        bool any = false;
        if (tx < g.ntx) {
            any = rec == nullptr;
            if (rec)
#pragma unroll 4
                for (int ty = wave; ty < nty; ty += 4) any |= rec[ty * g.ntx + tx] != 0;
        }
        const unsigned long long mine = __ballot(any);
        __syncthreads();
        if (lane == 0) s_any[wave] = mine;
        __syncthreads();
        unsigned long long m = s_any[0] | s_any[1] | s_any[2] | s_any[3];
        if (covered) m &= ~1ull;
        covered = false;
        while (m) {
            const int b = __ffsll((long long)m) - 1;
            if (tid == 0 && count < 1024) s_start[count] = (int16_t)(c0 + b);
            ++count;
            m &= ~(3ull << b);
            covered = b == 63;
        }
    }
    count = count < 1024 ? count : 1024;
    if (tid == 0) s_base = atomicAdd(counter, count);
    __syncthreads();
    const int base = s_base;
    for (int k = wave; k < count; k += 4) {
        const int tx0 = s_start[k];
        const bool two = tx0 + 1 < g.ntx;
        int bands = 0;
        for (int r0 = 0; r0 < nty; r0 += 64) {
            const int ty = r0 + lane;
            bool reach = false;
            if (ty < nty) {
                reach = rec == nullptr;
                for (int d = -2; d <= 2 && rec; ++d) {
                    const int y = ty + d;
                    if (y < 0 || y >= nty) continue;
                    reach |= rec[y * g.ntx + tx0] != 0;
                    if (two) reach |= rec[y * g.ntx + tx0 + 1] != 0;
                }
            }
            bands += __popcll(__ballot(reach));
        }
        if (lane == 0 && base + k < cap)
            items[base + k] = make_int2((int)blockIdx.x | (tx0 << 16), bands + 4);
    }
}

#define MB_SEG_MAX 8
#define MB_SEG_LEAD 8
#define MB_SEG_SLOTS 192
__global__ __launch_bounds__(256) void mb_sort_kernel(const int2 *__restrict__ items,
                                                      int *__restrict__ counter, int cap, int scap,
                                                      int wgs_per_item, int slots,
                                                      int2 *__restrict__ sorted,
                                                      const pano_patch *__restrict__ table, int cm,
                                                      int force_t) {
    __shared__ int s_hist[MB_SORT_BINS];
    __shared__ int s_lmax, s_lsum, s_total;
    const int tid = threadIdx.x;
    const int n = min(*counter, cap);
    (void)table, (void)cm;
    int T = 0;
    constexpr int NCAND = 13, HL = 128;
    constexpr int MINE = 4;
    __shared__ int s_segs[NCAND], s_est[NCAND];
    __shared__ __align__(16) unsigned short s_len[NCAND][HL];
    const bool consider = slots > 0 && n > 0 && !force_t && (long long)n * wgs_per_item < 3ll * slots &&
                          n <= MINE * 256;
    if (slots > 0 && n > 0) {
        if (tid == 0) s_lmax = s_lsum = 0;
        if (tid < NCAND) s_segs[tid] = 0, s_est[tid] = 0x7fffffff;
        for (int i = tid; i < NCAND * HL / 2; i += 256) ((unsigned int *)&s_len[0][0])[i] = 0u;
        __syncthreads();
        int lmax = 0, lsum = 0, mine[MINE];
#pragma unroll
        for (int r = 0; r < MINE; ++r) {
            const int i = tid + 256 * r;
            mine[r] = 0;
            if (i < n) {
                const int2 it = items[i];
                lmax = max(lmax, it.y);
                lsum += it.y;
                mine[r] = it.y;
            }
        }
        for (int i = tid + 256 * MINE; i < n; i += 256) {
            const int2 it = items[i];
            lmax = max(lmax, it.y);
            lsum += it.y;
        }
        atomicMax(&s_lmax, lmax);
        atomicAdd(&s_lsum, lsum);
        __syncthreads();
        const int Lmax = s_lmax, Lsum = s_lsum;
        auto cand = [&](const int c) {
            if (c == 0) return 1 << 20;
            const int mul = c == 1 ? 32769 : c == 2 ? 21846 : c == 3 ? 16385 : c == 4 ? 13108
                          : c == 5 ? 10923 : c == 6 ? 9363 : 8193;
            const int t = c < 8 ? (int)((unsigned)((Lmax + c) * mul) >> 16) : 8 * (c - 6);
            return max(t, 8);
        };
        auto div_small = [](const int a, const int b, const float rcp_b) {
            int q = (int)((float)a * rcp_b);
            q -= q * b > a ? 1 : 0;
            q += (q + 1) * b <= a ? 1 : 0;
            return q;
        };
        if (consider) {
            const bool by_wave = n <= 64 * MINE;
            const int lane = tid & 63, wave = tid >> 6;
            if (by_wave) {
#pragma unroll
                for (int r = 0; r < MINE; ++r) {
                    const int i = lane + 64 * r;
                    mine[r] = i < n ? items[i].y : 0;
                }
            }
            const int rounds = by_wave ? (n + 63) >> 6 : (n + 255) >> 8;
#pragma unroll 1
            for (int c = by_wave ? wave : 0; c < NCAND; c += by_wave ? 4 : 1) {
                const int t = cand(c);
                const float rcp_t = 1.0f / (float)t;
                int segs = 0;
#pragma unroll
                for (int r = 0; r < MINE; ++r) {
                    if (r >= rounds) break;
                    const int len = mine[r];
                    if (len > 0) {
                        const int ns = min(MB_SEG_MAX, div_small(len + t - 1, t, rcp_t));
                        const int wl = min(div_small(len + ns - 1, ns, 1.0f / (float)ns) + MB_SEG_LEAD, HL - 1);
                        segs += ns;
                        atomicAdd((unsigned int *)&s_len[c][wl & ~1], (unsigned int)ns << (16 * (wl & 1)));
                    }
                }
                for (int off = 32; off > 0; off >>= 1) segs += __shfl_xor(segs, off, 64);
                if (lane == 0 && segs) atomicAdd(&s_segs[c], segs);
            }
        }
        __syncthreads();
        __shared__ int s_got[NCAND][4], s_lmin[NCAND];
        if (tid < NCAND) {
            s_got[tid][0] = s_got[tid][1] = s_got[tid][2] = s_got[tid][3] = 0;
            s_lmin[tid] = HL;
        }
        __syncthreads();
        static_assert(HL == 16 * 8 && NCAND * 16 <= 256, "16 chunks of eight bins per candidate");
        if (consider && tid < NCAND * 16) {
            const int c = tid >> 4, chunk = 15 - (tid & 15);
            const int W = s_segs[c] * wgs_per_item;
            const uint4 q = *(const uint4 *)&s_len[c][8 * chunk];
            const unsigned int word[4] = {q.x, q.y, q.z, q.w};
            int cnt[8], total = 0;
#pragma unroll
            for (int e = 0; e < 8; ++e) {
                cnt[e] = (int)((word[e >> 1] >> (16 * (e & 1))) & 0xffffu) * wgs_per_item;
                total += cnt[e];
            }
            int seen = total;
#pragma unroll
            for (int off = 1; off < 16; off <<= 1) {
                const int v = __shfl_up(seen, off, 16);
                if ((tid & 15) >= off) seen += v;
            }
            seen -= total;
            if (total) {
                const int want[4] = {1, slots, slots + 1, 2 * slots + 1 - W};
                int lmin = HL;
#pragma unroll
                for (int e = 7; e >= 0; --e) {
                    if (!cnt[e]) continue;
#pragma unroll
                    for (int u = 0; u < 4; ++u)
                        if (want[u] > seen && want[u] <= seen + cnt[e]) s_got[c][u] = 8 * chunk + e;
                    seen += cnt[e];
                    lmin = 8 * chunk + e;
                }
                atomicMin(&s_lmin[c], lmin);
            }
        }
        __syncthreads();
        if (consider && tid < NCAND) {
            const int c = tid, t = cand(c), segs = s_segs[c];
            int est = 0x7fffffff;
            if (c == 0 || (t < Lmax && segs > n && segs <= scap && segs <= n + MB_SEG_SLOTS)) {
                const int W = segs * wgs_per_item, lmin = s_lmin[c];
                const int *got = s_got[c];
                const int share = (int)(((long long)Lsum + (long long)segs * MB_SEG_LEAD) *
                                        wgs_per_item / slots);
                if (W <= slots)
                    est = got[0];
                else if (W <= 2 * slots)
                    est = max(max(got[0], got[1] + got[2]), max(got[3] + lmin, share));
                else
                    est = max(got[0], share + lmin / 2);
            }
            s_est[c] = est;
        }
        __syncthreads();
        const int base = s_est[0];
        int best = base;
        for (int c = 1; c < NCAND && consider; ++c) {
            const int m = s_est[c];
            if (m < best && (long long)m * 100 <= (long long)base * 85) {
                best = m;
                T = cand(c);
            }
        }
        if (force_t) {
            T = 0;
            if (force_t >= 4) {
                __syncthreads();
                if (tid == 0) s_segs[0] = 0;
                __syncthreads();
                int segs = 0;
                for (int i = tid; i < n; i += 256) segs += min(MB_SEG_MAX, (items[i].y + force_t - 1) / force_t);
                if (segs) atomicAdd(&s_segs[0], segs);
                __syncthreads();
                if (s_segs[0] <= scap && s_segs[0] <= n + MB_SEG_SLOTS) T = force_t;
            }
        }
        __syncthreads();
    }
    auto segments_of = [&](const int2 it) {
        return T ? min(MB_SEG_MAX, (it.y + T - 1) / T) : 1;
    };
    auto entry = [&](const int2 it, const int seg, const int ns) {
        const int len = ns == 1 ? it.y : (it.y + ns - 1) / ns + 4;
        return make_int2(it.x, min(len, MB_SORT_BINS - 1) | seg << 12 | (ns == 1 ? 0 : ns) << 16);
    };
    for (int i = tid; i < MB_SORT_BINS; i += 256) s_hist[i] = 0;
    if (tid == 0) s_total = 0;
    __syncthreads();
    for (int i = tid; i < n; i += 256) {
        const int2 it = items[i];
        const int ns = segments_of(it);
        for (int seg = 0; seg < ns; ++seg)
            atomicAdd(&s_hist[MB_SORT_BINS - 1 - (entry(it, seg, ns).y & 0xfff)], 1);
        atomicAdd(&s_total, ns);
    }
    __syncthreads();
    const int total = s_total;
    __shared__ int s_part[256];
    constexpr int PER = MB_SORT_BINS / 256;
    int mine[PER], sum = 0;
#pragma unroll
    for (int j = 0; j < PER; ++j) {
        mine[j] = s_hist[tid * PER + j];
        sum += mine[j];
    }
    s_part[tid] = sum;
    __syncthreads();
    for (int off = 1; off < 256; off <<= 1) {
        const int v = tid >= off ? s_part[tid - off] : 0;
        __syncthreads();
        s_part[tid] += v;
        __syncthreads();
    }
    int run = s_part[tid] - sum;
#pragma unroll
    for (int j = 0; j < PER; ++j) {
        s_hist[tid * PER + j] = run;
        run += mine[j];
    }
    __syncthreads();
    for (int i = tid; i < n; i += 256) {
        const int2 it = items[i];
        const int ns = segments_of(it);
        for (int seg = 0; seg < ns; ++seg) {
            const int2 e = entry(it, seg, ns);
            sorted[atomicAdd(&s_hist[MB_SORT_BINS - 1 - (e.y & 0xfff)], 1)] = e;
        }
    }
    for (int i = total + tid; i < scap; i += 256) sorted[i] = make_int2(-1, 0);
    __syncthreads();
    if (tid == 0) *counter = 0;
}

static inline int mb_sorted_slots(int cap) { return (cap + MB_SEG_SLOTS + 1) & ~1; }


static int launch_tile_flags(pano_ctx *ctx, const pano_patch *table, int n, int ntx_max,
                             int nty_max, int W, const uint8_t *interior, uint8_t *tile_flags) {
    const hipStream_t stream = ctx->stream;
    dim3 grid(ceil_div(ntx_max, 32), ceil_div(nty_max, 8), n);
    PANO_TIMED(PK_TILE_FLAGS, stream,
               hipLaunchKernelGGL(tile_flags32_kernel, grid, dim3(256), 0, stream, table, interior,
                                  ceil_div(W, PANO_INTERIOR_BLOCK), tile_flags));
    PANO_LAUNCH_CHECK("tile_flags32_kernel");
    return PANO_OK;
}

int pano_tiles_blur_mfma(pano_ctx *ctx, const pano_patch *table, int n, int max_aw, int max_ah,
                         int W, int radius, const uint8_t *interior, uint8_t *tile_flags,
                         uint8_t *warp_need) {
    const hipStream_t stream = ctx->stream;
    const int ntx_max = (max_aw + 62) / 32, nty_max = (max_ah + 62) / 32;
    if (int rc = launch_tile_flags(ctx, table, n, ntx_max, nty_max, W, interior, tile_flags))
        return rc;
    ctx->flags_table = table;
    ctx->flags_n = n;
    ctx->blur_cm = (radius + 15) / 16 < 1 ? 1 : (radius + 15) / 16;
    if (warp_need) {
        const int cm = (radius + 15) / 16 < 1 ? 1 : (radius + 15) / 16;
        const int hx = (16 * cm + 31) / 32 + 1, vy = (cm + 1) / 2;
        dim3 grid(ceil_div(ntx_max, 32), ceil_div(nty_max, 8), n);
        hipLaunchKernelGGL(warp_need_kernel, grid, dim3(256), 0, stream, table, tile_flags, hx, vy,
                           warp_need);
        PANO_LAUNCH_CHECK("warp_need_kernel");
    }
    return PANO_OK;
}

int pano_prepare_blur_mfma(pano_ctx *ctx, const pano_patch *table, int n, int max_aw, int max_ah,
                           int W, const uint8_t *interior, uint8_t *tile_flags) {
    const hipStream_t stream = ctx->stream;
    const int ntx_max = (max_aw + 62) / 32, nty_max = (max_ah + 62) / 32;
    PANO_REQUIRE(nty_max <= MB_NEED_MAX, "pano_multiband_blur: %d rows of tiles exceed %d", nty_max,
                 MB_NEED_MAX);
    const uint8_t *flags = nullptr;
    if (interior) {
        if (ctx->flags_table != table || ctx->flags_n != n)
            if (int rc = launch_tile_flags(ctx, table, n, ntx_max, nty_max, W, interior, tile_flags))
                return rc;
        ctx->flags_table = nullptr;
        flags = tile_flags;
    }
    const int cap = n * ceil_div(ntx_max, 2);
    if (cap > ctx->item_cap) {
        if (ctx->item_buf) {
            PANO_HIP(hipStreamSynchronize(stream));
            PANO_HIP(hipFree(ctx->item_buf));
            ctx->item_buf = nullptr;
        }
        ctx->item_cap = cap * 2;
        PANO_HIP(hipMalloc((void **)&ctx->item_buf,
                           ((size_t)ctx->item_cap * 2 + MB_SEG_SLOTS + 2) * sizeof(int2)));
    }
    if (!ctx->item_counter) {
        PANO_HIP(hipMalloc((void **)&ctx->item_counter, sizeof(int)));
        PANO_HIP(hipMemsetAsync(ctx->item_counter, 0, sizeof(int), stream));
    }
    hipLaunchKernelGGL(mb_items_kernel, dim3(n), dim3(256), 0, stream, table, flags, ctx->item_buf,
                       ctx->item_counter, cap);
    PANO_LAUNCH_CHECK("mb_items_kernel");
    const int force_t = ctx->opt[PANO_OPT_BLUR_SEG_LEN];
    hipLaunchKernelGGL(mb_sort_kernel, dim3(1), dim3(256), 0, stream, ctx->item_buf,
                       ctx->item_counter, cap, mb_sorted_slots(cap), 4,
                       ctx->opt[PANO_OPT_BLUR_SEGMENTS] ? 256 : 0,
                       ctx->item_buf + ctx->item_cap, table,
                       ctx->opt[PANO_OPT_BLUR_SEGMENTS] ? (ctx->blur_cm > 0 ? ctx->blur_cm : 3) : 0,
                       force_t);
    PANO_LAUNCH_CHECK("mb_sort_kernel");
    ctx->prepared_table = ctx->list_table = table;
    ctx->prepared_n = ctx->list_n = n;
    return PANO_OK;
}

int pano_blur_mfma_opt_in(void) {
    PANO_HIP(hipFuncSetAttribute((const void *)blur_mfma_kernel<2>,
                                 hipFuncAttributeMaxDynamicSharedMemorySize, 160 * 1024));
    PANO_HIP(hipFuncSetAttribute((const void *)blur_mfma_kernel<4>,
                                 hipFuncAttributeMaxDynamicSharedMemorySize, 160 * 1024));
    PANO_HIP(hipFuncSetAttribute((const void *)blur_lean_kernel,
                                 hipFuncAttributeMaxDynamicSharedMemorySize, 160 * 1024));
    PANO_HIP(hipFuncSetAttribute((const void *)blur_lean5_kernel,
                                 hipFuncAttributeMaxDynamicSharedMemorySize, 160 * 1024));
    return PANO_OK;
}

static int launch_levels(pano_ctx *ctx, const pano_patch *table, int n, int max_aw,
                         const int16_t *owner, int W, const float *host_taps_all,
                         const int *ntaps_all, int lev0, int cnt, int rmax_all, int group,
                         const uint8_t *flags) {
    const hipStream_t stream = ctx->stream;
    const int *ntaps = ntaps_all + lev0;
    size_t skip = 0;
    for (int k = 0; k < lev0; ++k) skip += (size_t)ntaps_all[k] + PANO_TAP_PAD;
    const float *host_taps = host_taps_all + skip;
    int ord[PANO_MAX_LEVELS];
    if (group == 2) {
        int by_size[PANO_MAX_LEVELS];
        for (int k = 0; k < cnt; ++k) by_size[k] = k;
        for (int a = 1; a < cnt; ++a)
            for (int b = a; b > 0 && ntaps[by_size[b]] > ntaps[by_size[b - 1]]; --b) {
                const int tmp = by_size[b];
                by_size[b] = by_size[b - 1];
                by_size[b - 1] = tmp;
            }
        for (int i = 0, lo = 0, hi = cnt - 1; i < cnt; ++i)
            ord[i] = (i & 1) ? by_size[hi--] : by_size[lo++];
    } else {
        for (int k = 0; k < cnt; ++k) ord[k] = k;
    }
    MbLevels L = {};
    L.n = cnt;
    int total = 0;
    for (int i = 0; i < cnt; ++i) {
        L.tab_off[i] = total;
        total += mb_table_bytes(ntaps[ord[i]]);
    }
    PanoTapSet *set = nullptr;
    bool fresh = false;
    if (int rc = pano_ctx_tap_set(ctx, host_taps, ntaps, cnt, (size_t)total, &set, &fresh))
        return rc;
    size_t first[PANO_MAX_LEVELS], off = 0;
    for (int k = 0; k < cnt; ++k) {
        first[k] = off + PANO_TAP_LEAD + ((rmax_all - ntaps[k] / 2) & 3);
        off += (size_t)ntaps[k] + PANO_TAP_PAD;
    }
    for (int i = 0; i < cnt; ++i) {
        L.w[i] = set->taps + first[ord[i]];
        L.ntaps[i] = ntaps[ord[i]];
        L.out[i] = lev0 + ord[i];
    }
    unsigned char *tables = set->tables;
    if (fresh) {
        hipLaunchKernelGGL(mb_tables_kernel, dim3(cnt), dim3(128), 0, stream, L, tables);
        PANO_LAUNCH_CHECK("mb_tables_kernel");
        if (int rc = pano_ctx_tap_set_built(ctx, set)) return rc;
    }
    const int ntx_max = (max_aw + 62) / 32;
    const int cap = mb_sorted_slots(n * ceil_div(ntx_max, 2));
    const int2 *sorted = ctx->item_buf + ctx->item_cap;
    const int ngroups = ceil_div(cnt, group);
    int lds = 0;
    for (int gidx = 0; gidx < ngroups; ++gidx) {
        int bytes = 0, cm = 1;
        for (int i = group * gidx; i < cnt && i < group * (gidx + 1); ++i) {
            bytes += mb_table_bytes(L.ntaps[i]);
            cm = mb_c_of(L.ntaps[i]) > cm ? mb_c_of(L.ntaps[i]) : cm;
        }
        bytes += mb_fixed_bytes(cm);
        lds = bytes > lds ? bytes : lds;
    }
    PANO_REQUIRE(lds <= 160 * 1024, "pano_multiband_blur: %d bytes of LDS tables", lds);
    PANO_REQUIRE((long long)cap * 4 * ngroups < (1ll << 31), "pano_multiband_blur: %d work items",
                 cap);
    dim3 grid((unsigned)cap * 4 * ngroups, 1, 1);
    int lean = ctx->opt[PANO_OPT_BLUR_LEAN] && group == 4 ? 1 : 0;
    const bool five = lean && cnt == 5 && mb_c_of(L.ntaps[0]) == 1 &&
                      mb_c_of(L.ntaps[1]) == 2;
    if (cnt > 4 && !five) lean = 0;
    for (int i = 0; i < cnt; ++i)
        if (L.ntaps[i] < 3) lean = 0;
    for (int i = 0; i < cnt; ++i)
        if (mb_c_of(L.ntaps[i]) > 3) lean = 0;
    int lds_lean = 0;
    for (int gidx = 0; gidx < (five ? 1 : ngroups); ++gidx) {
        int bytes = 0, cm = 1;
        for (int i = group * gidx; i < cnt && (five || i < group * (gidx + 1)); ++i) {
            bytes += mb_table_bytes(L.ntaps[i]);
            cm = mb_c_of(L.ntaps[i]) > cm ? mb_c_of(L.ntaps[i]) : cm;
        }
        bytes = (bytes + mb_fixed_bytes(cm) + 15) / 16 * 16 + 2 * 32 * mb_pitch_of(cm) * 2;
        lds_lean = bytes > lds_lean ? bytes : lds_lean;
    }
    if (lds_lean > 160 * 1024) lean = 0;
    if (lean) {
        if (five) {
            grid = dim3((unsigned)cap * 4, 1, 1);
            PANO_TIMED(PK_BLUR_LEAN5, stream,
                       hipLaunchKernelGGL(blur_lean5_kernel, grid, dim3(MB_THREADS_OF(4)), lds_lean,
                                          stream, table, L, tables, owner, W, flags, sorted));
            PANO_LAUNCH_CHECK("blur_lean5_kernel");
        } else {
            PANO_TIMED(PK_BLUR_LEAN, stream,
                       hipLaunchKernelGGL(blur_lean_kernel, grid, dim3(MB_THREADS_OF(4)), lds_lean,
                                          stream, table, L, tables, owner, W, flags, sorted));
            PANO_LAUNCH_CHECK("blur_lean_kernel");
        }
        return PANO_OK;
    }
    if (group == 2)
        PANO_TIMED(PK_BLUR_MFMA, stream,
                   hipLaunchKernelGGL(blur_mfma_kernel<2>, grid, dim3(MB_THREADS_OF(2)), lds, stream,
                                      table, L, tables, owner, W, flags, sorted));
    else
        PANO_TIMED(PK_BLUR_MFMA, stream,
                   hipLaunchKernelGGL(blur_mfma_kernel<4>, grid, dim3(MB_THREADS_OF(4)), lds, stream,
                                      table, L, tables, owner, W, flags, sorted));
    PANO_LAUNCH_CHECK("blur_mfma_kernel");
    return PANO_OK;
}

int pano_launch_blur_mfma(pano_ctx *ctx, const pano_patch *table, int n, int max_aw, int max_ah,
                          const int16_t *owner, int W, const float *host_taps, const int *ntaps,
                          int n_blur, const uint8_t *interior, uint8_t *tile_flags) {
    bool narrow = true;
    int rmax = 0;
    for (int k = 0; k < n_blur; ++k) {
        if (mb_c_of(ntaps[k]) > 3) narrow = false;
        rmax = ntaps[k] / 2 > rmax ? ntaps[k] / 2 : rmax;
    }
    if (ctx->prepared_table != table || ctx->prepared_n != n)
        if (int rc = pano_prepare_blur_mfma(ctx, table, n, max_aw, max_ah, W, interior, tile_flags))
            return rc;
    ctx->prepared_table = nullptr;
    const uint8_t *flags = interior ? tile_flags : nullptr;
    if (narrow && n_blur == 5 && ctx->opt[PANO_OPT_BLUR_LEAN] &&
        mb_c_of(ntaps[0]) == 1 && mb_c_of(ntaps[1]) == 2 && ntaps[0] >= 3)
        return launch_levels(ctx, table, n, max_aw, owner, W, host_taps, ntaps, 0, 5, rmax, 4, flags);
    if (narrow && (n_blur == 5 || n_blur == 6)) {
        const bool beside = ctx->opt[PANO_OPT_STITCH_STREAMS] != 0 && !ctx->timing_on;
        const hipStream_t main_stream = ctx->stream;
        if (beside) {
            if (int rc = pano_ctx_side_stream(ctx)) return rc;
            PANO_HIP(hipEventRecord(ctx->ev_fork, main_stream));
            PANO_HIP(hipStreamWaitEvent(ctx->side, ctx->ev_fork, 0));
        }
        if (int rc = launch_levels(ctx, table, n, max_aw, owner, W, host_taps, ntaps, 0, 4, rmax, 4,
                                   flags))
            return rc;
        if (beside) ctx->stream = ctx->side;
        const int rc2 = launch_levels(ctx, table, n, max_aw, owner, W, host_taps, ntaps, 4, n_blur - 4,
                                      rmax, 2, flags);
        ctx->stream = main_stream;
        if (rc2) return rc2;
        if (beside) {
            PANO_HIP(hipEventRecord(ctx->ev_join, ctx->side));
            PANO_HIP(hipStreamWaitEvent(main_stream, ctx->ev_join, 0));
        }
        return PANO_OK;
    }
    const int group = narrow && (n_blur <= 2 || n_blur == 5 || n_blur == 6) ? 2 : 4;
    return launch_levels(ctx, table, n, max_aw, owner, W, host_taps, ntaps, 0, n_blur, rmax, group,
                         flags);
}
```

pano360_amd/csrc/common.h:

```cpp
#pragma once
#include <hip/hip_runtime.h>
#include <stdint.h>

#include <vector>

#include "../../include/pano360.h"

void pano_set_error(const char *fmt, ...);

#define PANO_REQUIRE(cond, ...)          \
    do {                                 \
        if (!(cond)) {                   \
            pano_set_error(__VA_ARGS__); \
            return PANO_EINVAL;          \
        }                                \
    } while (0)

#define PANO_HIP(call)                                                         \
    do {                                                                       \
        hipError_t e_ = (call);                                                \
        if (e_ != hipSuccess) {                                                \
            pano_set_error("%s failed: %s", #call, hipGetErrorString(e_));     \
            return PANO_EHIP;                                                  \
        }                                                                      \
    } while (0)

#define PANO_LAUNCH_CHECK(name)                                                \
    do {                                                                       \
        hipError_t e_ = hipGetLastError();                                     \
        if (e_ != hipSuccess) {                                                \
            pano_set_error("launch of %s failed: %s", name,                    \
                           hipGetErrorString(e_));                             \
            return PANO_EHIP;                                                  \
        }                                                                      \
    } while (0)

enum PanoKernelId {
    PK_ADD_WEIGHTS = 0,
    PK_WARP,
    PK_OWNERSHIP,
    PK_BLUR_ROWS,
    PK_BLUR_COLS,
    PK_COMPOSE,
    PK_LINEAR,
    PK_NOBLEND,
    PK_CROP_HEIGHTS,
    PK_CROP_ROWS,
    PK_PYR_DOWN,
    PK_OWNERSHIP_CAMS,
    PK_OWNED_BOXES,
    PK_WARP_WINDOWS,
    PK_BLEND_CAMERAS,
    PK_OWNED_SPANS,
    PK_INTERIOR,
    PK_TILE_FLAGS,
    PK_OVERLAP,
    PK_BLUR_MFMA,
    PK_SIFT_EXTREMA,
    PK_SIFT_ORIENT,
    PK_SIFT_DESCRIBE,
    PK_SCALE_STEP,
    PK_KNN2,
    PK_BLUR_LEAN,
    PK_BLUR_LEAN5,
    PK_RANSAC_SCORE,
    PK_RANSAC_FINISH,
    PK_MATCH_PACK,
    PK_BA_RESIDUAL,
    PK_BA_PAIRS,
    PK_BA_ASSEMBLE,
    PK_JPEG_DESTUFF,
    PK_JPEG_SCAN,
    PK_JPEG_INTERVALS,
    PK_JPEG_HUFF_SYNC,
    PK_JPEG_HUFF_WRITE,
    PK_JPEG_DC,
    PK_JPEG_IDCT,
    PK_JPEG_PIXELS,
    PK_JPEG_ENC_BLOCKS,
    PK_JPEG_ENC_COUNT,
    PK_JPEG_ENC_SCAN,
    PK_JPEG_ENC_EMIT,
    PK_JPEG_ENC_STUFF,
    PK_COUNT
};
struct PanoTapSet {
    uint64_t key;
    int n, ntaps[PANO_MAX_LEVELS];
    float *taps;
    unsigned char *tables;
    uint64_t used;
    float *host;
    size_t floats;
    hipEvent_t ready;
    hipStream_t built_on;
};

struct LayoutSummary;
struct PanoSiftGraph {
    uint64_t key;
    hipGraphExec_t exec;
    int seen;
    uint64_t used;
};

#define GEOM_BUFS 11
#define STITCH_SIG 13
struct pano_ctx {
    int device;
    hipStream_t stream;
    int opt[PANO_OPT_COUNT];
    bool timing_on;
    std::vector<hipEvent_t> t_begin[PK_COUNT], t_end[PK_COUNT];
    int2 *item_buf;
    int *item_counter;
    int blur_cm;
    int item_cap;
    const pano_patch *prepared_table, *flags_table;
    int prepared_n, flags_n;
    const pano_patch *list_table;
    int list_n;
    std::vector<PanoTapSet> tap_sets;
    uint64_t tick;
    hipEvent_t ev_regions, ev_upload, ev_fork, ev_join, ev_copy;
    hipStream_t side;
    bool upload_pending;
    LayoutSummary *lay_sum_host;
    int32_t *lay_rects_dev;
    uint8_t *lay_have_dev;
    int lay_cap_n;
    std::vector<int32_t> lay_rects_host;
    std::vector<uint8_t> lay_have_host;
    pano_layout lay_prev;
    int lay_prev_sig[STITCH_SIG];
    bool lay_prev_valid;
    bool lay_prev_verified;
    bool trusted_pending;
    int lay_prev_used_need;
    bool geom_valid, in_stitch;
    const void *geom_bufs[GEOM_BUFS];
    int lay_count[2];
    uint32_t *sift_raw;
    size_t sift_raw_cap;
    bool sift_capturing;
    std::vector<PanoSiftGraph> sift_graphs;
    uint8_t *enc_dev, *enc_out, *enc_host;
    size_t enc_dev_cap, enc_out_cap, enc_host_cap;
    uint8_t *poisson_dev, *poisson_host;
    size_t poisson_cap;
    uint8_t *seam_dev, *seam_host;
};

int pano_ctx_enter(pano_ctx *ctx);
void pano_sift_graphs_free(pano_ctx *ctx);
int pano_sift_raw_reserve(pano_ctx *ctx, int rows, int cols);
int pano_zero_i32(hipStream_t s, int *p, int n);
int pano_ctx_side_stream(pano_ctx *ctx);
int pano_ctx_tap_set(pano_ctx *ctx, const float *taps, const int *ntaps, int n, size_t table_bytes,
                     PanoTapSet **out, bool *fresh);
int pano_ctx_tap_set_built(pano_ctx *ctx, PanoTapSet *set);

#define PANO_ENTER(ctx, who)                                       \
    PANO_REQUIRE((ctx) != nullptr, "%s: null context", who);       \
    if (int rc_ = pano_ctx_enter(ctx)) return rc_;                 \
    void *const stream = (void *)(ctx)->stream;                    \
    (void)stream

#define PANO_ENTER_READONLY(ctx, who)                              \
    const bool geom_keep_ = (ctx) != nullptr && (ctx)->geom_valid; \
    PANO_ENTER(ctx, who);                                          \
    (ctx)->geom_valid = geom_keep_

void pano_timing_edge(pano_ctx *ctx, int kid, hipStream_t stream, bool begin);

#define PANO_TIMED(kid, stream, ...)                                        \
    do {                                                                    \
        if (ctx->timing_on) pano_timing_edge(ctx, kid, stream, true);       \
        __VA_ARGS__;                                                        \
        if (ctx->timing_on) pano_timing_edge(ctx, kid, stream, false);      \
    } while (0)

static inline int pano_pitch_of(int w) { return (w + 3) & ~3; }

int pano_launch_blur_mfma(pano_ctx *ctx, const pano_patch *table, int n, int max_aw, int max_ah,
                          const int16_t *owner, int W, const float *taps, const int *ntaps,
                          int n_blur, const uint8_t *interior, uint8_t *tile_flags);
int pano_prepare_blur_mfma(pano_ctx *ctx, const pano_patch *table, int n, int max_aw, int max_ah,
                           int W, const uint8_t *interior, uint8_t *tile_flags);
int pano_tiles_blur_mfma(pano_ctx *ctx, const pano_patch *table, int n, int max_aw, int max_ah,
                         int W, int radius, const uint8_t *interior, uint8_t *tile_flags,
                         uint8_t *warp_need);
int pano_blur_mfma_opt_in(void);
int pano_blur_valu_opt_in(void);
static inline bool pano_blur_uses_mfma(const pano_ctx *ctx) {
    return ctx->opt[PANO_OPT_BLUR_KERNEL] == PANO_BLUR_MFMA;
}
static inline int ceil_div(int a, int b) { return (a + b - 1) / b; }

typedef const __attribute__((address_space(4))) float *kptr_f32;

__device__ __forceinline__ int reflect_edge(int p, int len) {
    if ((unsigned)p < (unsigned)len) return p;
    int per = 2 * len;
    int m = p % per;
    if (m < 0) m += per;
    return m < len ? m : per - 1 - m;
}

__device__ __forceinline__ int reflect_101(int p, int len) {
    if ((unsigned)p < (unsigned)len) return p;
    if (len == 1) return 0;
    int per = 2 * len - 2;
    int m = p % per;
    if (m < 0) m += per;
    return m < len ? m : per - m;
}

__device__ __forceinline__ int cv_round(float v) {
    const float r = rintf(v);
    return fabsf(r) < 2147483648.0f ? (int)r : (int)0x80000000;
}

__device__ __forceinline__ int sat16(int v) {
    return v < -32768 ? -32768 : (v > 32767 ? 32767 : v);
}
```

pano360_amd/csrc/layout.h:

```cpp
#pragma once
#include "common.h"

__host__ __device__ static inline void reflect_closed(long lo, long hi, long n, long &a, long &b) {
    if (n == 1) {
        a = 0;
        b = 1;
        return;
    }
    if (lo < -(n - 1) || hi > 2 * n - 1) {
        a = 0;
        b = n;
        return;
    }
    a = lo > 0 ? lo : 0;
    b = hi < n ? hi : n;
    if (lo < 0) {
        a = a < 1 ? a : 1;
        b = b > 1 - lo ? b : 1 - lo;
    }
    if (hi > n) {
        a = a < 2 * n - 1 - hi ? a : 2 * n - 1 - hi;
        b = b > n - 1 ? b : n - 1;
    }
    a = a > 0 ? a : 0;
    b = b < n ? b : n;
}

struct LayoutSizes {
    long planes, blurred, scratch, tiles, lead;
};

__host__ __device__ static inline bool layout_record(const int32_t *rg, int sp, const int32_t *rect,
                                                     int i, int radius, int xs0, int xs1,
                                                     int n_blur, bool grid32, pano_patch &r,
                                                     LayoutSizes &sz) {
    const long ymin = rg[0], ymax = rg[1];
    const long y0 = rect[0], y1 = rect[1], x0 = rect[2], x1 = rect[3];
    const long h = y1 - y0, w = x1 - x0;
    const long xmin = rg[5 + 2 * sp], xmax = rg[6 + 2 * sp];
    if (ymax < ymin || xmax < xmin) return false;
    long ay0 = ymin - y0 - radius, ay1 = ymax - y0 + 1 + radius;
    long ax0 = xmin - x0 - radius, ax1 = xmax - x0 + 1 + radius;
    ay0 = ay0 > 0 ? ay0 : 0;
    ay1 = ay1 < h ? ay1 : h;
    ax0 = ax0 > 0 ? ax0 : 0;
    ax1 = ax1 < w ? ax1 : w;
    ax0 = ax0 > xs0 - x0 ? ax0 : xs0 - x0;
    ax1 = ax1 < xs1 - x0 ? ax1 : xs1 - x0;
    if (ax1 <= ax0) return false;
    long vy0, vy1, vx0, vx1;
    reflect_closed(ay0 - radius, ay1 + radius, h, vy0, vy1);
    reflect_closed(ax0 - radius, ax1 + radius, w, vx0, vx1);
    vy0 = vy0 < ay0 ? vy0 : ay0;
    vy1 = vy1 > ay1 ? vy1 : ay1;
    vx0 = vx0 < ax0 ? vx0 : ax0;
    vx1 = vx1 > ax1 ? vx1 : ax1;
    vx0 &= ~3l;
    vx1 = (vx1 + 3) & ~3l;
    vx1 = vx1 < w ? vx1 : w;
    r = pano_patch{};
    r.y0 = (int)y0, r.x0 = (int)x0, r.h = (int)h, r.w = (int)w;
    r.index = i;
    r.vy0 = (int)vy0, r.vx0 = (int)vx0, r.vh = (int)(vy1 - vy0), r.vw = (int)(vx1 - vx0);
    r.ay0 = (int)ay0, r.ax0 = (int)ax0, r.ah = (int)(ay1 - ay0), r.aw = (int)(ax1 - ax0);
    r.vpitch = (r.vw + 3) & ~3;
    sz = LayoutSizes{};
    if (grid32) {
        r.apitch = (r.aw + 31) & ~31;
        sz.lead = r.ax0 & 31;
        sz.blurred = (long)n_blur * 4 * r.ah * r.apitch + 32;
        sz.tiles = (long)(((r.ax0 + r.aw - 1) >> 5) - (r.ax0 >> 5) + 1) *
                   (((r.ay0 + r.ah - 1) >> 5) - (r.ay0 >> 5) + 1);
    } else {
        r.apitch = (r.aw + 3) & ~3;
        sz.blurred = (long)n_blur * 4 * r.ah * r.apitch;
        sz.scratch = (long)n_blur * 4 * r.vh * r.apitch;
        sz.tiles = (long)((r.aw + 63) / 64) * ((r.ah + 127) / 128);
    }
    sz.planes = 3l * r.vh * r.vpitch;
    return true;
}

__host__ __device__ static inline bool layout_record_fits(const pano_patch &r) {
    return (long)r.vh * r.vpitch * 4 < (1l << 31) && (long)r.ah * r.apitch * 4 < (1l << 31);
}

struct LayoutSummary {
    int64_t planes_floats, blurred_floats, scratch_floats;
    int32_t n_records, n_tiles;
    int32_t max_vw, max_vh, max_aw, max_ah;
    int32_t missing;
    int32_t ok;
    int32_t why;
    int32_t pad;
};
```

pano360_amd/csrc/stitch.hip:

```cpp
#include <string.h>

#include "common.h"
#include "layout.h"


#define LAY_THREADS 512
__global__ __launch_bounds__(LAY_THREADS) void layout_windows_kernel(
    const int32_t *__restrict__ regions, const int32_t *__restrict__ rects,
    const uint8_t *__restrict__ have, int n, int max_spans, int radius, int xs0, int xs1,
    int n_blur, int grid32, float *planes, float *blurred, float *scratch, long cap_planes,
    long cap_blurred, long cap_scratch, int cap_tiles, int want_tiles, int b_nr, int b_vw,
    int b_vh, int b_aw, int b_ah, pano_patch *__restrict__ table,
    LayoutSummary *__restrict__ summary, LayoutSummary expect, int check_expect,
    int *__restrict__ sticky) {
    __shared__ long s_planes[LAY_THREADS], s_blurred[LAY_THREADS], s_scratch[LAY_THREADS];
    __shared__ int s_tiles[LAY_THREADS], s_slot[LAY_THREADS];
    __shared__ long s_run[4];
    __shared__ int s_count, s_max[4], s_missing, s_bad;
    const int tid = threadIdx.x, stride = 5 + 2 * max_spans;
    if (tid == 0) {
        s_run[0] = s_run[1] = s_run[2] = s_run[3] = 0;
        s_count = s_missing = s_bad = 0;
        s_max[0] = s_max[1] = s_max[2] = s_max[3] = 0;
    }
    __syncthreads();
    const int total = n * max_spans;
    for (int base = 0; base < total; base += LAY_THREADS) {
        const int c = base + tid, i = c / max_spans, sp = c - i * max_spans;
        pano_patch rec = pano_patch{};
        LayoutSizes sz = LayoutSizes{};
        bool ok = false;
        if (c < total) {
            const int32_t *rg = regions + (size_t)i * stride;
            const int spans = rg[4] < max_spans ? rg[4] : max_spans;
            if (sp < spans)
                ok = layout_record(rg, sp, rects + 4 * i, i, radius, xs0, xs1, n_blur, grid32 != 0,
                                   rec, sz);
        }
        s_slot[tid] = ok ? 1 : 0;
        s_planes[tid] = sz.planes;
        s_blurred[tid] = sz.blurred;
        s_scratch[tid] = sz.scratch;
        s_tiles[tid] = (int)(sz.tiles < (1l << 30) ? sz.tiles : (1l << 30));
        if (ok) {
            atomicMax(&s_max[0], rec.vw);
            atomicMax(&s_max[1], rec.vh);
            atomicMax(&s_max[2], rec.aw);
            atomicMax(&s_max[3], rec.ah);
            if (have && !have[i]) atomicAdd(&s_missing, 1);
            if (!layout_record_fits(rec)) atomicOr(&s_bad, 8);
        }
        __syncthreads();
        if (tid < 64) {
            long pl = s_run[0], bl = s_run[1], sc = s_run[2], tl = s_run[3];
            int k = s_count;
            const int cnt = min(LAY_THREADS, total - base);
            for (int t0 = 0; t0 < cnt; t0 += 64) {
                const int t = t0 + tid;
                const int has = s_slot[t];
                long v[4] = {has ? s_planes[t] : 0, has ? s_blurred[t] : 0, has ? s_scratch[t] : 0,
                             has ? (long)s_tiles[t] : 0};
                int one = has;
                const long own[4] = {v[0], v[1], v[2], v[3]};
#pragma unroll
                for (int off = 1; off < 64; off <<= 1) {
                    const int o1 = __shfl_up(one, off, 64);
                    long o[4];
#pragma unroll
                    for (int q = 0; q < 4; ++q) o[q] = __shfl_up(v[q], off, 64);
                    if (tid >= off) {
                        one += o1;
#pragma unroll
                        for (int q = 0; q < 4; ++q) v[q] += o[q];
                    }
                }
                s_slot[t] = has ? k + one - 1 : -1;
                s_planes[t] = pl + v[0] - own[0];
                s_blurred[t] = bl + v[1] - own[1];
                s_scratch[t] = sc + v[2] - own[2];
                const long toff = tl + v[3] - own[3];
                s_tiles[t] = (int)(toff < (1l << 30) ? toff : (1l << 30));
                k += __shfl(one, 63, 64);
                pl += __shfl(v[0], 63, 64);
                bl += __shfl(v[1], 63, 64);
                sc += __shfl(v[2], 63, 64);
                tl += __shfl(v[3], 63, 64);
            }
            for (int t = cnt + tid; t < LAY_THREADS; t += 64) s_slot[t] = -1;
            if (tid == 0) {
                s_run[0] = pl, s_run[1] = bl, s_run[2] = sc, s_run[3] = tl;
                s_count = k;
            }
        }
        __syncthreads();
        const int k = s_slot[tid];
        if (k >= 0 && k < b_nr) {
            rec.planes = planes + s_planes[tid];
            rec.blurred = blurred ? blurred + s_blurred[tid] + sz.lead : nullptr;
            rec.scratch = scratch ? scratch + s_scratch[tid] : nullptr;
            rec.tiles_off = s_tiles[tid];
            table[k] = rec;
        }
        __syncthreads();
    }
    const int nr = s_count;
    const long need_planes = s_run[0], need_blurred = s_run[1] + 32, need_scratch = s_run[2];
    int why = s_bad;
    if (need_planes > cap_planes || (n_blur > 0 && nr > 0 && (need_blurred > cap_blurred ||
                                                              need_scratch > cap_scratch)) ||
        (want_tiles && s_run[3] > cap_tiles))
        why |= 1;
    if (s_max[0] > b_vw || s_max[1] > b_vh || s_max[2] > b_aw || s_max[3] > b_ah) why |= 2;
    if (nr > b_nr) why |= 4;
    if (s_missing) why |= 16;
    for (int k = (why ? 0 : nr) + tid; k < b_nr; k += LAY_THREADS) table[k] = pano_patch{};
    if (tid == 0) {
        LayoutSummary out;
        out.planes_floats = need_planes;
        out.blurred_floats = need_blurred;
        out.scratch_floats = need_scratch;
        out.n_records = nr;
        out.n_tiles = (int)(s_run[3] < (1l << 30) ? s_run[3] : (1l << 30));
        out.max_vw = s_max[0], out.max_vh = s_max[1], out.max_aw = s_max[2], out.max_ah = s_max[3];
        out.missing = s_missing;
        out.ok = why == 0;
        out.why = why;
        out.pad = 0;
        *summary = out;
        if (check_expect &&
            !(out.ok && out.planes_floats == expect.planes_floats &&
              out.blurred_floats == expect.blurred_floats && out.scratch_floats == expect.scratch_floats &&
              out.n_records == expect.n_records && out.n_tiles == expect.n_tiles &&
              out.max_vw == expect.max_vw && out.max_vh == expect.max_vh && out.max_aw == expect.max_aw &&
              out.max_ah == expect.max_ah && out.missing == 0))
            *(volatile int *)sticky = 1;
    }
}

static int ensure_layout_buffers(pano_ctx *ctx, int n) {
    if (!ctx->lay_sum_host) {
        PANO_HIP(hipHostMalloc((void **)&ctx->lay_sum_host, sizeof(LayoutSummary) + 64, hipHostMallocDefault));
        memset(ctx->lay_sum_host, 0, sizeof(LayoutSummary) + 64);
    }
    if (n > ctx->lay_cap_n) {
        PANO_HIP(hipStreamSynchronize(ctx->stream));
        if (ctx->lay_rects_dev) PANO_HIP(hipFree(ctx->lay_rects_dev));
        if (ctx->lay_have_dev) PANO_HIP(hipFree(ctx->lay_have_dev));
        ctx->lay_rects_dev = nullptr;
        ctx->lay_have_dev = nullptr;
        PANO_HIP(hipMalloc((void **)&ctx->lay_rects_dev, (size_t)n * 4 * sizeof(int32_t)));
        PANO_HIP(hipMalloc((void **)&ctx->lay_have_dev, (size_t)n));
        ctx->lay_cap_n = n;
        ctx->lay_rects_host.clear();
        ctx->lay_have_host.clear();
    }
    return PANO_OK;
}

static LayoutSummary layout_expectation(const pano_layout &v) {
    LayoutSummary e = {};
    e.planes_floats = v.planes_floats, e.blurred_floats = v.blurred_floats;
    e.scratch_floats = v.scratch_floats;
    e.n_records = v.n_records, e.n_tiles = v.n_tiles;
    e.max_vw = v.max_vw, e.max_vh = v.max_vh, e.max_aw = v.max_aw, e.max_ah = v.max_ah;
    return e;
}
static int *layout_sticky(pano_ctx *ctx) {
    return (int *)((unsigned char *)ctx->lay_sum_host + sizeof(LayoutSummary));
}

static void stitch_signature(const pano_stitch_args *a, int tile_grid, int *sig) {
    const int v[STITCH_SIG] = {a->n, a->H, a->W, a->xs0, a->xs1, a->own0, a->own1, a->n_levels,
                               a->radius, a->max_spans, a->shortcut, a->min_gap, tile_grid};
    for (int k = 0; k < STITCH_SIG; ++k) sig[k] = v[k];
}

static int stitch_interior_map(pano_ctx *ctx, const pano_stitch_args *a, int n_blur) {
    if (a->classes && n_blur > 0 && ctx->opt[PANO_OPT_LEVEL_CLASSES]) {
        int radii[PANO_MAX_LEVELS];
        bool ascending = true;
        for (int k = 0; k < n_blur; ++k) {
            radii[k] = a->ntaps[k] / 2;
            if (k && radii[k] < radii[k - 1]) ascending = false;
        }
        if (ascending && radii[n_blur - 1] == a->radius)
            return pano_interior_classes(ctx, a->owner, a->H, a->W, a->own0, a->own1, radii, n_blur,
                                         a->block_owner, a->interior, a->classes);
    }
    return pano_interior_map(ctx, a->owner, a->H, a->W, a->own0, a->own1, a->radius, a->block_owner,
                             a->interior);
}

static bool stitch_has_classes(const pano_ctx *ctx, const pano_stitch_args *a, int n_blur) {
    if (!a->classes || n_blur <= 0 || !ctx->opt[PANO_OPT_LEVEL_CLASSES]) return false;
    for (int k = 0; k < n_blur; ++k)
        if (k && a->ntaps[k] / 2 < a->ntaps[k - 1] / 2) return false;
    return a->ntaps[n_blur - 1] / 2 == a->radius;
}

#define ON_SIDE(ctx, call)                  \
    do {                                    \
        const hipStream_t main_ = (ctx)->stream; \
        (ctx)->stream = (ctx)->side;        \
        const int rc_side_ = (call);        \
        (ctx)->stream = main_;              \
        if (rc_side_) return rc_side_;      \
    } while (0)

static int queue_tail(pano_ctx *ctx, pano_stitch_args *a, const pano_layout &lay, bool device_table,
                      int need_choice, bool two_streams, bool interior, int n_blur, int tile_grid,
                      bool kept = false) {
    const hipStream_t s = ctx->stream;
    const bool use_blur = n_blur > 0 && lay.n_records > 0;
    const int nr = lay.n_records;
    if (!device_table) {
        if (lay.planes_floats > a->planes_floats || (use_blur && lay.blurred_floats > a->blurred_floats) ||
            (use_blur && lay.scratch_floats > a->scratch_floats) ||
            (interior && lay.n_tiles > a->cap_tiles))
            return PANO_EGROW;
        PANO_REQUIRE(lay.planes_floats == 0 || a->planes, "pano_stitch_multiband: no plane arena");
        if (int rc = pano_layout_place(a->records_host, lay.n_records, a->planes, a->blurred, a->scratch))
            return rc;
        if (nr) {
            PANO_HIP(hipMemcpyAsync(a->table, a->records_host, (size_t)nr * sizeof(pano_patch),
                                    hipMemcpyHostToDevice, s));
            PANO_HIP(hipEventRecord(ctx->ev_upload, s));
            ctx->upload_pending = true;
        }
    }
    a->used_need = 0;
    if (kept) {
        a->used_need = need_choice == 1;
        two_streams = false;
    } else if (interior && tile_grid == 32 && nr && a->tile_flags && a->need) {
        bool on = need_choice == 1;
        if (need_choice < 0) {
            double sum = 0.0;
            for (int k = 0; k < nr; ++k) sum += a->records_host[k].aw;
            on = sum / nr >= 768.0;
        }
        if (on) {
            if (two_streams) {
                PANO_HIP(hipEventRecord(ctx->ev_join, ctx->side));
                PANO_HIP(hipStreamWaitEvent(s, ctx->ev_join, 0));
            }
            if (int rc = pano_blur_tiles(ctx, a->table, nr, lay.max_aw, lay.max_ah, a->W, a->radius,
                                         a->interior, a->tile_flags, a->need))
                return rc;
            a->used_need = 1;
        }
    }
    const bool fork2 = two_streams && interior && n_blur && nr &&
                       !a->used_need && tile_grid == 32 && a->tile_flags;
    if (fork2) {
        if (device_table) {
            PANO_HIP(hipEventRecord(ctx->ev_upload, s));
        }
        PANO_HIP(hipStreamWaitEvent(ctx->side, ctx->ev_upload, 0));
        ON_SIDE(ctx, pano_multiband_blur_prepare(ctx, a->table, nr, lay.max_aw, lay.max_ah, a->W,
                                                 a->interior, a->tile_flags));
        PANO_HIP(hipEventRecord(ctx->ev_join, ctx->side));
    } else if (two_streams && interior) {
        PANO_HIP(hipEventRecord(ctx->ev_join, ctx->side));
    }
    if (int rc = pano_warp_windows(ctx, a->cams, a->table, nr, lay.max_vw, lay.max_vh, a->sin_t,
                                   a->cos_t, a->tan_p, a->lut, a->lut_stride,
                                   a->used_need ? a->need : nullptr))
        return rc;
    if (two_streams && interior) PANO_HIP(hipStreamWaitEvent(s, ctx->ev_join, 0));
    if (kept && use_blur) {
        ctx->prepared_table = a->table;
        ctx->prepared_n = nr;
    }
    if (n_blur)
        if (int rc = pano_multiband_blur(ctx, a->table, nr, lay.max_aw, lay.max_vh, lay.max_ah,
                                         a->owner, a->W, a->taps, (const int *)a->ntaps, n_blur,
                                         interior ? a->interior : nullptr,
                                         interior ? a->tile_flags : nullptr))
            return rc;
    return pano_multiband_compose(ctx, a->table, nr, a->H, a->W, a->xs0, a->xs1, a->n_levels,
                                  a->owner, a->valid, interior ? a->interior : nullptr,
                                  interior && stitch_has_classes(ctx, a, n_blur) ? a->classes : nullptr,
                                  interior ? a->cams : nullptr, interior ? a->sin_t : nullptr,
                                  interior ? a->cos_t : nullptr, interior ? a->tan_p : nullptr,
                                  a->lut, a->lut_stride, a->mosaic, a->mosaic_f32);
}

static void geometry_buffers(const pano_stitch_args *a, const void *out[GEOM_BUFS]) {
    const void *v[GEOM_BUFS] = {a->owner, a->valid, a->table, a->interior, a->tile_flags, a->need,
                                a->planes, a->blurred, a->scratch, a->sin_t, a->classes};
    for (int k = 0; k < GEOM_BUFS; ++k) out[k] = v[k];
}
static void geometry_left(pano_ctx *ctx, const pano_stitch_args *a) {
    geometry_buffers(a, ctx->geom_bufs);
    ctx->geom_valid = true;
}

namespace {
struct StitchScope {
    pano_ctx *ctx;
    explicit StitchScope(pano_ctx *c) : ctx(c) { ctx->in_stitch = true; }
    ~StitchScope() { ctx->in_stitch = false; }
};
}

extern "C" int pano_stitch_multiband(pano_ctx *ctx, pano_stitch_args *a, int resume) {
    const bool geom_was_valid = ctx && ctx->geom_valid;
    PANO_ENTER(ctx, "pano_stitch_multiband");
    ctx->geom_valid = false;
    StitchScope scope(ctx);
    PANO_REQUIRE(a, "pano_stitch_multiband: null arguments");
    PANO_REQUIRE(a->cams && a->rects && a->sin_t && a->cos_t && a->tan_p && a->lut && a->owner &&
                     a->valid && a->marks && a->regions && a->regions_host && a->records_host &&
                     a->table && a->mosaic,
                 "pano_stitch_multiband: null pointer");
    PANO_REQUIRE(a->n > 0 && a->n <= 32767 && a->H > 0 && a->W > 0 && a->max_spans >= 1,
                 "pano_stitch_multiband: bad argument");
    PANO_REQUIRE(a->n_levels >= 1 && a->n_levels <= PANO_MAX_LEVELS,
                 "pano_stitch_multiband: n_levels %d outside [1, %d]", a->n_levels, PANO_MAX_LEVELS);
    PANO_REQUIRE(a->own0 <= a->xs0 && a->xs1 <= a->own1 && a->own0 >= 0 && a->own1 <= a->W,
                 "pano_stitch_multiband: strip [%d, %d) outside the ownership columns [%d, %d)",
                 a->xs0, a->xs1, a->own0, a->own1);
    PANO_REQUIRE(a->cap_records >= a->n * a->max_spans,
                 "pano_stitch_multiband: %d record slots for %d cameras x %d spans", a->cap_records,
                 a->n, a->max_spans);
    const int n_blur = a->n_levels - 1;
    PANO_REQUIRE(n_blur == 0 || (a->taps && a->ntaps), "pano_stitch_multiband: no tap tables");
    const bool interior = a->shortcut && n_blur > 0;
    PANO_REQUIRE(!interior || (a->block_owner && a->interior),
                 "pano_stitch_multiband: interior map without its buffers");
    const hipStream_t s = (hipStream_t)stream;
    if (int rc = pano_ctx_side_stream(ctx)) return rc;
    const bool big = (long long)a->H * (a->own1 - a->own0) >= (1ll << 24);
    const bool two_streams = ctx->opt[PANO_OPT_STITCH_STREAMS] != 0 && big;
    const int tile_grid = pano_blur_tile_grid(ctx);
    const int stride = 5 + 2 * a->max_spans;
    int sig[STITCH_SIG];
    stitch_signature(a, tile_grid, sig);

    if (!resume) {
        bool spec = ctx->opt[PANO_OPT_STITCH_ASYNC] != 0 && interior && tile_grid == 32 &&
                    ctx->lay_prev_valid && memcmp(sig, ctx->lay_prev_sig, sizeof(sig)) == 0 &&
                    ctx->lay_prev.n_records > 0 && a->planes && a->blurred && a->tile_flags;
        pano_layout bound = ctx->lay_prev;
        const bool want_keep = a->trust_layout == 3;
        const bool want_trust = a->trust_layout == 1 || want_keep;
        a->trust_layout = 0;
        if (ctx->trusted_pending && !(want_trust && spec))
            if (int rc = pano_stitch_verify(ctx)) return rc;
        const bool trusted = want_trust && spec && ctx->lay_prev_verified &&
                             ctx->opt[PANO_OPT_STITCH_ASYNC] == 1;
        const bool list_kept = n_blur == 0 || ctx->lay_prev.n_records == 0 ||
                               (ctx->item_buf && ctx->list_table == a->table &&
                                ctx->list_n == ctx->lay_prev.n_records);
        if (want_keep && trusted && geom_was_valid && tile_grid == 32 && list_kept) {
            const void *bufs[GEOM_BUFS];
            geometry_buffers(a, bufs);
            if (memcmp(bufs, ctx->geom_bufs, sizeof(bufs)) == 0) {
                if (int rc = queue_tail(ctx, a, ctx->lay_prev, true, ctx->lay_prev_used_need, false,
                                        interior, n_blur, tile_grid, true))
                    return rc;
                a->layout = ctx->lay_prev;
                a->trust_layout = 4;
                ctx->geom_valid = true;
                ++ctx->lay_count[0];
                return PANO_OK;
            }
        }
        if (spec) {
            if (int rc = ensure_layout_buffers(ctx, a->n)) return rc;
            const size_t nrect = (size_t)a->n * 4;
            if (ctx->lay_rects_host.size() != nrect ||
                memcmp(ctx->lay_rects_host.data(), a->rects, nrect * sizeof(int32_t)) != 0) {
                ctx->lay_rects_host.assign(a->rects, a->rects + nrect);
                PANO_HIP(hipMemcpyAsync(ctx->lay_rects_dev, ctx->lay_rects_host.data(),
                                        nrect * sizeof(int32_t), hipMemcpyHostToDevice, s));
            }
            std::vector<uint8_t> have(a->n, 1);
            if (a->have) have.assign(a->have, a->have + a->n);
            if (ctx->lay_have_host != have) {
                ctx->lay_have_host = have;
                PANO_HIP(hipMemcpyAsync(ctx->lay_have_dev, ctx->lay_have_host.data(), (size_t)a->n,
                                        hipMemcpyHostToDevice, s));
            }
            if (!trusted) {
                bound.n_records = bound.n_records + 2 < a->cap_records ? bound.n_records + 2 : a->cap_records;
                bound.max_vw += 64, bound.max_vh += 64, bound.max_aw += 64, bound.max_ah += 64;
            }
            if (ctx->opt[PANO_OPT_STITCH_ASYNC] == 2) {
                bound.n_records = ctx->lay_prev.n_records > 1 ? ctx->lay_prev.n_records - 1 : 1;
                bound.max_vw = ctx->lay_prev.max_vw - 1;
            }
        }
        if (int rc = pano_ownership_regions(ctx, a->cams, a->n, a->H, a->W, a->own0, a->own1,
                                            a->sin_t, a->cos_t, a->tan_p, a->owner, a->valid,
                                            a->min_gap, a->max_spans, a->marks, a->regions))
            return rc;
        const bool forked = two_streams;
        if (forked && interior) {
            PANO_HIP(hipEventRecord(ctx->ev_fork, s));
            PANO_HIP(hipStreamWaitEvent(ctx->side, ctx->ev_fork, 0));
            ON_SIDE(ctx, stitch_interior_map(ctx, a, n_blur));
        }
        bool interior_queued = forked && interior;
        if (spec) {
            if (ctx->upload_pending) {
                PANO_HIP(hipEventSynchronize(ctx->ev_upload));
                ctx->upload_pending = false;
            }
            uintptr_t bbase = (uintptr_t)a->blurred;
            bbase += (uintptr_t)(-(intptr_t)bbase) % 128;
            hipLaunchKernelGGL(layout_windows_kernel, dim3(1), dim3(LAY_THREADS), 0, s, a->regions,
                               ctx->lay_rects_dev, ctx->lay_have_dev, a->n, a->max_spans, a->radius,
                               a->xs0, a->xs1, n_blur, 1, a->planes, (float *)bbase, a->scratch,
                               (long)a->planes_floats, (long)a->blurred_floats,
                               (long)a->scratch_floats, a->cap_tiles, 1, bound.n_records,
                               bound.max_vw, bound.max_vh, bound.max_aw, bound.max_ah, a->table,
                               ctx->lay_sum_host, layout_expectation(ctx->lay_prev), trusted ? 1 : 0,
                               layout_sticky(ctx));
            PANO_LAUNCH_CHECK("layout_windows_kernel");
            PANO_HIP(hipEventRecord(ctx->ev_regions, s));
            if (!trusted) {
                PANO_HIP(hipStreamWaitEvent(ctx->side, ctx->ev_regions, 0));
                PANO_HIP(hipMemcpyAsync(a->records_host, a->table,
                                        (size_t)bound.n_records * sizeof(pano_patch),
                                        hipMemcpyDeviceToHost, ctx->side));
                PANO_HIP(hipEventRecord(ctx->ev_copy, ctx->side));
            }
            if (interior && !interior_queued) {
                if (int rc = stitch_interior_map(ctx, a, n_blur)) return rc;
                interior_queued = true;
            }
            if (int rc = queue_tail(ctx, a, bound, true, ctx->lay_prev_used_need, two_streams, interior,
                                    n_blur, tile_grid))
                return rc;
            if (trusted) {
                a->layout = ctx->lay_prev;
                a->used_need = ctx->lay_prev_used_need;
                a->trust_layout = 2;
                ctx->trusted_pending = true;
                geometry_left(ctx, a);
                ++ctx->lay_count[0];
                return PANO_OK;
            }
            PANO_HIP(hipEventSynchronize(ctx->ev_regions));
            PANO_HIP(hipEventSynchronize(ctx->ev_copy));
            const LayoutSummary sum = *ctx->lay_sum_host;
            a->layout.planes_floats = sum.planes_floats;
            a->layout.blurred_floats = sum.blurred_floats;
            a->layout.scratch_floats = sum.scratch_floats;
            a->layout.n_records = sum.n_records, a->layout.n_tiles = sum.n_tiles;
            a->layout.max_vw = sum.max_vw, a->layout.max_vh = sum.max_vh;
            a->layout.max_aw = sum.max_aw, a->layout.max_ah = sum.max_ah;
            a->layout.missing = sum.missing;
            if (sum.ok) {
                ctx->lay_prev = a->layout;
                ctx->lay_prev_used_need = a->used_need;
                ctx->lay_prev_verified = true;
                geometry_left(ctx, a);
                ++ctx->lay_count[0];
                return PANO_OK;
            }
            ++ctx->lay_count[1];
            ctx->lay_prev_valid = false;
            ctx->lay_prev_verified = false;
        }
        PANO_HIP(hipMemcpyAsync(a->regions_host, a->regions, (size_t)a->n * stride * sizeof(int32_t),
                                hipMemcpyDeviceToHost, s));
        PANO_HIP(hipEventRecord(ctx->ev_regions, s));
        if (interior && !interior_queued)
            if (int rc = stitch_interior_map(ctx, a, n_blur)) return rc;
        PANO_HIP(hipEventSynchronize(ctx->ev_regions));
        if (ctx->upload_pending) {
            PANO_HIP(hipEventSynchronize(ctx->ev_upload));
            ctx->upload_pending = false;
        }
        a->layout = pano_layout{};
        if (int rc = pano_layout_windows(tile_grid, a->regions_host, a->n, a->max_spans, a->rects,
                                         a->have, a->radius, a->xs0, a->xs1, n_blur,
                                         a->records_host, a->cap_records, &a->layout))
            return rc;
        if (a->layout.missing) {
            pano_set_error("pano_stitch_multiband: %d records of cameras whose frames are not "
                           "resident reach columns [%d, %d)", a->layout.missing, a->xs0, a->xs1);
            return PANO_EINVAL;
        }
    }
    const int rc = queue_tail(ctx, a, a->layout, false, a->warp_need, two_streams, interior, n_blur,
                              tile_grid);
    if (rc == PANO_OK) {
        ctx->lay_prev = a->layout;
        memcpy(ctx->lay_prev_sig, sig, sizeof(sig));
        ctx->lay_prev_used_need = a->used_need;
        ctx->lay_prev_valid = true;
        ctx->lay_prev_verified = true;
        geometry_left(ctx, a);
    }
    return rc;
}

extern "C" int pano_stitch_verify(pano_ctx *ctx) {
    PANO_REQUIRE(ctx, "pano_stitch_verify: null context");
    if (!ctx->trusted_pending) return PANO_OK;
    PANO_HIP(hipSetDevice(ctx->device));
    PANO_HIP(hipEventSynchronize(ctx->ev_regions));
    ctx->trusted_pending = false;
    const LayoutSummary sum = *ctx->lay_sum_host;
    const pano_layout &v = ctx->lay_prev;
    const int sticky = __atomic_exchange_n(layout_sticky(ctx), 0, __ATOMIC_SEQ_CST);
    const bool same = !sticky && sum.ok && sum.planes_floats == v.planes_floats &&
                      sum.blurred_floats == v.blurred_floats && sum.scratch_floats == v.scratch_floats &&
                      sum.n_records == v.n_records && sum.n_tiles == v.n_tiles &&
                      sum.max_vw == v.max_vw && sum.max_vh == v.max_vh && sum.max_aw == v.max_aw &&
                      sum.max_ah == v.max_ah && sum.missing == 0;
    if (!same) {
        ctx->lay_prev_valid = ctx->lay_prev_verified = false;
        ctx->geom_valid = false;
        pano_set_error("pano_stitch_verify: a trusted stitch laid out %d records (ok %d, why %d, an "
                       "earlier one differed: %d) where the verified layout has %d: the cameras were "
                       "not those of the verified stitch",
                       sum.n_records, sum.ok, sum.why, sticky, v.n_records);
        return PANO_EINVAL;
    }
    return PANO_OK;
}

extern "C" int pano_stitch_counts(const pano_ctx *ctx, int *device_layouts, int *fallbacks) {
    PANO_REQUIRE(ctx && device_layouts && fallbacks, "pano_stitch_counts: null pointer");
    *device_layouts = ctx->lay_count[0];
    *fallbacks = ctx->lay_count[1];
    return PANO_OK;
}
```

pano360_amd/csrc/warp.hip:

```cpp
#include "geom.h"

struct ProjK {
    double p[9];
};

template <bool FULL>
__global__ __launch_bounds__(256) void warp_spherical_kernel(
    const uint8_t *__restrict__ frame, int sh, int sw, ProjK K,
    const double *__restrict__ sin_t, const double *__restrict__ cos_t,
    const double *__restrict__ tan_p, const float *__restrict__ lut255,
    const double *__restrict__ hat_x, const double *__restrict__ hat_y,
    int gx0, int gy0, int pw, int ph, int pitch, float *__restrict__ planes,
    uint8_t *__restrict__ mask, float *__restrict__ map_x,
    float *__restrict__ map_y) {
    __shared__ float s_lut[256];
    s_lut[threadIdx.y * 64 + threadIdx.x] = lut255[threadIdx.y * 64 + threadIdx.x];
    __syncthreads();

    const int x = blockIdx.x * 64 + threadIdx.x;
    const int y = blockIdx.y * 4 + threadIdx.y;
    if (x >= pw || y >= ph) return;

    float px, py;
    const bool m = map_pixel(K.p, sin_t[gx0 + x], cos_t[gx0 + x], tan_p[gy0 + y], sw, sh,
                             px, py);
    const Taps tp = make_taps(px, py, sw, sh);
    const uint8_t *r0 = frame + (size_t)tp.y0 * sw * 3;
    const uint8_t *r1 = frame + (size_t)tp.y1 * sw * 3;
    const uint8_t *p00 = r0 + tp.x0 * 3, *p01 = r0 + tp.x1 * 3;
    const uint8_t *p10 = r1 + tp.x0 * 3, *p11 = r1 + tp.x1 * 3;
    const size_t plane = (size_t)ph * pitch;
    const size_t o = (size_t)y * pitch + x;
#pragma unroll
    for (int k = 0; k < 3; ++k)
        planes[k * plane + o] =
            lerp4(s_lut[p00[k]], s_lut[p01[k]], s_lut[p10[k]], s_lut[p11[k]], tp);
    if (FULL) {
        float a = alpha_at(hat_x, hat_y, tp);
        a = a * (m ? 0.0f : 1.0f);
        planes[3 * plane + o] = a;
        mask[(size_t)y * pw + x] = m ? 1 : 0;
        if (map_x) {
            map_x[(size_t)y * pw + x] = px;
            map_y[(size_t)y * pw + x] = py;
        }
    }
}

#define WARP_ROWS 4
__global__ __launch_bounds__(256) void warp_windows_kernel(
    const pano_camera *__restrict__ cams, const pano_patch *__restrict__ patches,
    const double *__restrict__ sin_t, const double *__restrict__ cos_t,
    const double *__restrict__ tan_p, const float *__restrict__ lut, int lut_stride,
    const uint8_t *__restrict__ need) {
    __shared__ float s_lut[256];
    const pano_patch p = patches[blockIdx.z];
    constexpr int BH = 4 * WARP_ROWS;
    if ((int)blockIdx.x * 64 >= p.vw || (int)blockIdx.y * BH >= p.vh) return;
    if (need) {
        const int ntx = ((p.ax0 + p.aw - 1) >> 5) - (p.ax0 >> 5) + 1;
        const int nty = ((p.ay0 + p.ah - 1) >> 5) - (p.ay0 >> 5) + 1;
        const int px0 = p.vx0 + (int)blockIdx.x * 64, py0 = p.vy0 + (int)blockIdx.y * BH;
        const int ty0 = min(max((py0 >> 5) - (p.ay0 >> 5), 0), nty - 1);
        const int ty1 = min(max(((py0 + BH - 1) >> 5) - (p.ay0 >> 5), 0), nty - 1);
        const int tx0 = min(max((px0 >> 5) - (p.ax0 >> 5), 0), ntx - 1);
        const int tx1 = min(max(((px0 + 63) >> 5) - (p.ax0 >> 5), 0), ntx - 1);
        bool any = false;
        for (int ty = ty0; ty <= ty1; ++ty)
            for (int tx = tx0; tx <= tx1; ++tx) any |= need[p.tiles_off + ty * ntx + tx] != 0;
        if (!any) return;
    }
    s_lut[threadIdx.y * 64 + threadIdx.x] =
        lut[(size_t)p.index * lut_stride + threadIdx.y * 64 + threadIdx.x];
    __syncthreads();

    const int x = blockIdx.x * 64 + threadIdx.x;
    const int y0 = blockIdx.y * BH + threadIdx.y;
    if (x >= p.vw || y0 >= p.vh) return;
    const pano_camera *cam = cams + p.index;
    const int sw = cam->sw, sh = cam->sh;
    const int gx = p.x0 + p.vx0 + x;
    const double s = table_f64(sin_t, gx), c = table_f64(cos_t, gx);
    double t[WARP_ROWS];
#pragma unroll
    for (int j = 0; j < WARP_ROWS; ++j)
        t[j] = table_f64(tan_p, p.y0 + p.vy0 + min(y0 + 4 * j, p.vh - 1));
    Taps tp[WARP_ROWS];
    TapBytes tb[WARP_ROWS];
    bool inner = true;
#pragma unroll
    for (int j = 0; j < WARP_ROWS; ++j) {
        float px, py;
        map_pixel(cam->proj, s, c, t[j], sw, sh, px, py);
        tp[j] = tap_base(px, py);
        inner &= taps_interior(tp[j], sw, sh);
    }
    if (__ballot(!inner) == 0ull) {
#pragma unroll
        for (int j = 0; j < WARP_ROWS; ++j) tb[j] = load_taps_interior(cam->frame, sw, tp[j]);
    } else {
#pragma unroll
        for (int j = 0; j < WARP_ROWS; ++j) {
            reflect_taps(tp[j], sw, sh);
            tb[j] = load_taps(cam->frame, sw, tp[j]);
        }
    }
    typedef __attribute__((address_space(1))) float *plane_ptr;
    typedef __attribute__((address_space(1))) char *byte_ptr;
    const size_t plane = (size_t)p.vh * p.vpitch;
    const byte_ptr out[3] = {(byte_ptr)p.planes, (byte_ptr)(p.planes + plane),
                             (byte_ptr)(p.planes + 2 * plane)};
#pragma unroll
    for (int j = 0; j < WARP_ROWS; ++j) {
        const int y = y0 + 4 * j;
        if (y >= p.vh) break;
        const uint32_t o = ((uint32_t)y * (uint32_t)p.vpitch + (uint32_t)x) * 4u;
#pragma unroll
        for (int k = 0; k < 3; ++k) {
            *(plane_ptr)(out[k] + o) = lerp4(lut_at(s_lut, tb[j].v[0][k]), lut_at(s_lut, tb[j].v[1][k]),
                                             lut_at(s_lut, tb[j].v[2][k]), lut_at(s_lut, tb[j].v[3][k]), tp[j]);
        }
    }
}

__global__ __launch_bounds__(256) void add_weights_kernel(
    const uint8_t *__restrict__ frame, int h, int w,
    const float *__restrict__ lut255, const double *__restrict__ hat_x,
    const double *__restrict__ hat_y, float4 *__restrict__ rgba) {
    const int x = blockIdx.x * 64 + threadIdx.x;
    const int y = blockIdx.y * 4 + threadIdx.y;
    if (x >= w || y >= h) return;
    const uint8_t *s = frame + ((size_t)y * w + x) * 3;
    float4 v;
    v.x = lut255[s[0]];
    v.y = lut255[s[1]];
    v.z = lut255[s[2]];
    v.w = (float)(hat_y[y] * hat_x[x]);
    rgba[(size_t)y * w + x] = v;
}

extern "C" int pano_add_weights(pano_ctx *ctx, const uint8_t *frame, int h, int w,
                                const float *lut255, const double *hat_x, const double *hat_y,
                                float *rgba) {
    PANO_ENTER(ctx, "pano_add_weights");
    PANO_REQUIRE(frame && lut255 && hat_x && hat_y && rgba, "pano_add_weights: null pointer");
    PANO_REQUIRE(h > 0 && w > 0, "pano_add_weights: bad shape %dx%d", h, w);
    dim3 block(64, 4), grid(ceil_div(w, 64), ceil_div(h, 4));
    PANO_TIMED(PK_ADD_WEIGHTS, (hipStream_t)stream,
               hipLaunchKernelGGL(add_weights_kernel, grid, block, 0, (hipStream_t)stream,
                                  frame, h, w, lut255, hat_x, hat_y, (float4 *)rgba));
    PANO_LAUNCH_CHECK("add_weights_kernel");
    return PANO_OK;
}

static int check_frame(const char *who, int sh, int sw, int pw, int ph, int gx0, int gy0) {
    PANO_REQUIRE(sh > 0 && sw > 0 && sh < 32767 && sw < 32767,
                 "%s: frame %dx%d outside (0, 32767)", who, sh, sw);
    PANO_REQUIRE(pw > 0 && ph > 0 && gx0 >= 0 && gy0 >= 0, "%s: bad rectangle", who);
    return PANO_OK;
}

extern "C" int pano_warp_spherical(pano_ctx *ctx, const uint8_t *frame, int sh, int sw,
                                   const double *proj, const double *sin_t, const double *cos_t,
                                   const double *tan_p, const float *lut255, const double *hat_x,
                                   const double *hat_y, int gx0, int gy0, int pw, int ph,
                                   float *planes, uint8_t *mask, float *map_x, float *map_y) {
    PANO_ENTER(ctx, "pano_warp_spherical");
    PANO_REQUIRE(frame && proj && sin_t && cos_t && tan_p && lut255 && hat_x &&
                     hat_y && planes && mask,
                 "pano_warp_spherical: null pointer");
    PANO_REQUIRE((map_x == nullptr) == (map_y == nullptr),
                 "pano_warp_spherical: map_x and map_y must both be given or both be NULL");
    if (int rc = check_frame("pano_warp_spherical", sh, sw, pw, ph, gx0, gy0)) return rc;
    ProjK K;
    for (int i = 0; i < 9; ++i) K.p[i] = proj[i];
    dim3 block(64, 4), grid(ceil_div(pw, 64), ceil_div(ph, 4));
    PANO_TIMED(PK_WARP, (hipStream_t)stream,
               hipLaunchKernelGGL(warp_spherical_kernel<true>, grid, block, 0,
                                  (hipStream_t)stream, frame, sh, sw, K, sin_t, cos_t, tan_p,
                                  lut255, hat_x, hat_y, gx0, gy0, pw, ph, pano_pitch_of(pw),
                                  planes, mask, map_x, map_y));
    PANO_LAUNCH_CHECK("warp_spherical_kernel");
    return PANO_OK;
}

extern "C" int pano_warp_windows(pano_ctx *ctx, const pano_camera *cams, const pano_patch *patches,
                                 int n, int max_vw, int max_vh, const double *sin_t,
                                 const double *cos_t, const double *tan_p, const float *lut,
                                 int lut_stride, const uint8_t *need) {
    PANO_ENTER(ctx, "pano_warp_windows");
    PANO_REQUIRE(cams && patches && sin_t && cos_t && tan_p && lut && lut_stride >= 0,
                 "pano_warp_windows: null pointer");
    PANO_REQUIRE(n >= 0 && n <= 65535 && max_vw >= 0 && max_vh >= 0,
                 "pano_warp_windows: bad argument");
    if (n == 0 || max_vw == 0 || max_vh == 0) return PANO_OK;
    dim3 block(64, 4), grid(ceil_div(max_vw, 64), ceil_div(max_vh, 4 * WARP_ROWS), n);
    PANO_TIMED(PK_WARP_WINDOWS, (hipStream_t)stream,
               hipLaunchKernelGGL(warp_windows_kernel, grid, block, 0, (hipStream_t)stream,
                                  cams, patches, sin_t, cos_t, tan_p, lut, lut_stride, need));
    PANO_LAUNCH_CHECK("warp_windows_kernel");
    return PANO_OK;
}
```

Baseline: 206,200 MP/s.

## Compact warp grid with per-record block prefix sums and per-record need gating

Replaces the padded 3D warp grid (max window size × records) with a flat 1D grid whose blocks map to records through a prefix-summed block-offset table. The table is built in the layout kernel or on the host. The warp-need tile gating now switches per record by area width instead of on the average width, so gated and ungated records can take separate launches. This removes idle blocks launched for small windows, at the cost of a ballot search per block and extra layout bookkeeping and verification.

```diff
diff --git a/include/pano360.h b/include/pano360.h
--- a/include/pano360.h
+++ b/include/pano360.h
@@ -153,6 +153,9 @@
                         pano_layout *out);
 int pano_layout_place(pano_patch *records, int n_records, void *planes, void *blurred,
                       void *scratch);
+
+int pano_warp_blocks(const pano_patch *records, int n, int gate_aw, int32_t *first_ungated,
+                     int32_t *first_gated);
 
 int pano_multiband_compose(pano_ctx *ctx, const pano_patch *patches, int n, int H, int W,
                            int xs0, int xs1, int n_levels, const int16_t *owner,
diff --git a/pano360_amd/_lib.py b/pano360_amd/_lib.py
--- a/pano360_amd/_lib.py
+++ b/pano360_amd/_lib.py
@@ -117,6 +117,7 @@
     "pano_multiband_blur_prepare": (_i, [_vp, _vp, _i, _i, _i, _i, _vp, _vp]),
     "pano_layout_windows": (_i, [_i, _vp, _i, _i, _vp, _vp, _i, _i, _i, _i, _vp, _i, _vp]),
     "pano_layout_place": (_i, [_vp, _i, _vp, _vp, _vp]),
+    "pano_warp_blocks": (_i, [_vp, _i, _i, _vp, _vp]),
     "pano_interior_map": (_i, [_vp, _vp, _i, _i, _i, _i, _i, _vp, _vp]),
     "pano_interior_classes": (_i, [_vp, _vp, _i, _i, _i, _i, _vp, _i, _vp, _vp, _vp]),
     "pano_multiband_compose": (_i, [_vp, _vp, _i, _i, _i, _i, _i, _i, _vp, _vp, _vp, _vp, _vp, _vp,
diff --git a/pano360_amd/csrc/api.hip b/pano360_amd/csrc/api.hip
--- a/pano360_amd/csrc/api.hip
+++ b/pano360_amd/csrc/api.hip
@@ -107,6 +107,8 @@
     if (ctx->lay_sum_host) (void)hipHostFree(ctx->lay_sum_host);
     if (ctx->lay_rects_dev) (void)hipFree(ctx->lay_rects_dev);
     if (ctx->lay_have_dev) (void)hipFree(ctx->lay_have_dev);
+    if (ctx->warp_first_dev) (void)hipFree(ctx->warp_first_dev);
+    if (ctx->warp_first_host) (void)hipHostFree(ctx->warp_first_host);
     if (ctx->side) {
         (void)hipStreamSynchronize(ctx->side);
         (void)hipStreamDestroy(ctx->side);
@@ -344,6 +346,19 @@
     return PANO_OK;
 }
 
+extern "C" int pano_warp_blocks(const pano_patch *records, int n, int gate_aw,
+                                int32_t *first_ungated, int32_t *first_gated) {
+    PANO_REQUIRE((records || n == 0) && n >= 0, "pano_warp_blocks: bad argument");
+    long run[2] = {0, 0};
+    for (int k = 0; k <= n; ++k) {
+        if (first_ungated) first_ungated[k] = (int32_t)run[0];
+        if (first_gated) first_gated[k] = (int32_t)run[1];
+        if (k < n) run[warp_record_gated(records[k], gate_aw) ? 1 : 0] += warp_blocks_of(records[k]);
+        PANO_REQUIRE(run[0] < (1l << 31) && run[1] < (1l << 31), "pano_warp_blocks: block count overflow");
+    }
+    return PANO_OK;
+}
+
 extern "C" int pano_layout_place(pano_patch *records, int n_records, void *planes, void *blurred,
                                  void *scratch) {
     PANO_REQUIRE(records || n_records == 0, "pano_layout_place: null pointer");
diff --git a/pano360_amd/csrc/blur.hip b/pano360_amd/csrc/blur.hip
--- a/pano360_amd/csrc/blur.hip
+++ b/pano360_amd/csrc/blur.hip
@@ -360,7 +360,7 @@
     PANO_REQUIRE(pano_blur_uses_mfma(ctx), "pano_blur_tiles: needs the 32 x 32 tile grid");
     if (n == 0 || max_aw == 0 || max_ah == 0) return PANO_OK;
     return pano_tiles_blur_mfma(ctx, patches, n, max_aw, max_ah, W, radius, interior, tile_flags,
-                                warp_need);
+                                warp_need, INT32_MIN);
 }
 
 extern "C" int pano_multiband_blur_prepare(pano_ctx *ctx, const pano_patch *patches, int n,
diff --git a/pano360_amd/csrc/blur_mfma.hip b/pano360_amd/csrc/blur_mfma.hip
--- a/pano360_amd/csrc/blur_mfma.hip
+++ b/pano360_amd/csrc/blur_mfma.hip
@@ -1347,9 +1347,10 @@
 
 __global__ __launch_bounds__(256) void warp_need_kernel(const pano_patch *__restrict__ table,
                                                         const uint8_t *__restrict__ flags, int hx,
-                                                        int vy, uint8_t *__restrict__ need) {
+                                                        int vy, uint8_t *__restrict__ need,
+                                                        int gate_aw) {
     const pano_patch p = table[blockIdx.z];
-    if (p.aw <= 0 || p.ah <= 0) return;
+    if (p.aw <= 0 || p.ah <= 0 || p.aw < gate_aw) return;
     const MbGeom g = mb_geom(p);
     const int nty = g.O1 - g.O0 + 1;
     const int tx = blockIdx.x * 32 + (threadIdx.x & 31), ty = blockIdx.y * 8 + (threadIdx.x >> 5);
@@ -1680,7 +1681,7 @@
 
 int pano_tiles_blur_mfma(pano_ctx *ctx, const pano_patch *table, int n, int max_aw, int max_ah,
                          int W, int radius, const uint8_t *interior, uint8_t *tile_flags,
-                         uint8_t *warp_need) {
+                         uint8_t *warp_need, int gate_aw) {
     const hipStream_t stream = ctx->stream;
     const int ntx_max = (max_aw + 62) / 32, nty_max = (max_ah + 62) / 32;
     if (int rc = launch_tile_flags(ctx, table, n, ntx_max, nty_max, W, interior, tile_flags))
@@ -1693,7 +1694,7 @@
         const int hx = (16 * cm + 31) / 32 + 1, vy = (cm + 1) / 2;
         dim3 grid(ceil_div(ntx_max, 32), ceil_div(nty_max, 8), n);
         hipLaunchKernelGGL(warp_need_kernel, grid, dim3(256), 0, stream, table, tile_flags, hx, vy,
-                           warp_need);
+                           warp_need, gate_aw);
         PANO_LAUNCH_CHECK("warp_need_kernel");
     }
     return PANO_OK;
diff --git a/pano360_amd/csrc/common.h b/pano360_amd/csrc/common.h
--- a/pano360_amd/csrc/common.h
+++ b/pano360_amd/csrc/common.h
@@ -137,6 +137,10 @@
     bool lay_prev_verified;
     bool trusted_pending;
     int lay_prev_used_need;
+    int lay_prev_choice;
+    int32_t *warp_first_dev, *warp_first_host;
+    int warp_first_cap;
+    int lay_prev_blocks[2], lay_prev_slack[2];
     bool geom_valid, in_stitch;
     const void *geom_bufs[GEOM_BUFS];
     int lay_count[2];
@@ -189,7 +193,11 @@
                            int W, const uint8_t *interior, uint8_t *tile_flags);
 int pano_tiles_blur_mfma(pano_ctx *ctx, const pano_patch *table, int n, int max_aw, int max_ah,
                          int W, int radius, const uint8_t *interior, uint8_t *tile_flags,
-                         uint8_t *warp_need);
+                         uint8_t *warp_need, int gate_aw);
+int pano_launch_warp_windows(pano_ctx *ctx, const pano_camera *cams, const pano_patch *patches,
+                             int n, int max_vw, int max_vh, const double *sin_t,
+                             const double *cos_t, const double *tan_p, const float *lut,
+                             int lut_stride, const uint8_t *need, const int32_t *first, int total);
 int pano_blur_mfma_opt_in(void);
 int pano_blur_valu_opt_in(void);
 static inline bool pano_blur_uses_mfma(const pano_ctx *ctx) {
diff --git a/pano360_amd/csrc/layout.h b/pano360_amd/csrc/layout.h
--- a/pano360_amd/csrc/layout.h
+++ b/pano360_amd/csrc/layout.h
@@ -85,6 +85,29 @@
     return (long)r.vh * r.vpitch * 4 < (1l << 31) && (long)r.ah * r.apitch * 4 < (1l << 31);
 }
 
+#define PANO_WARP_BW 64
+#define PANO_WARP_BH 16
+#ifndef PANO_WARP_GATE_AW
+#define PANO_WARP_GATE_AW 768
+#endif
+#define PANO_WARP_GATE_NONE 2147483647
+#define PANO_WARP_GATE_ALL (-2147483647 - 1)
+
+__host__ __device__ static inline int warp_blocks_of(const pano_patch &r) {
+    if (r.vw <= 0 || r.vh <= 0) return 0;
+    return ((r.vw + PANO_WARP_BW - 1) / PANO_WARP_BW) * ((r.vh + PANO_WARP_BH - 1) / PANO_WARP_BH);
+}
+__host__ __device__ static inline int warp_blocks_slack(const pano_patch &r) {
+    if (r.vw <= 0 || r.vh <= 0) return 0;
+    return 4 * ((r.vw + PANO_WARP_BW - 1) / PANO_WARP_BW) + (r.vh + PANO_WARP_BH - 1) / PANO_WARP_BH + 4;
+}
+__host__ __device__ static inline bool warp_record_gated(const pano_patch &r, int gate) {
+    return r.aw >= gate;
+}
+static inline int warp_gate_of_mode(int mode) {
+    return mode == 0 ? PANO_WARP_GATE_NONE : mode == 1 ? PANO_WARP_GATE_ALL : PANO_WARP_GATE_AW;
+}
+
 struct LayoutSummary {
     int64_t planes_floats, blurred_floats, scratch_floats;
     int32_t n_records, n_tiles;
@@ -93,4 +116,5 @@
     int32_t ok;
     int32_t why;
     int32_t pad;
+    int32_t blocks[2], slack[2];
 };
diff --git a/pano360_amd/csrc/stitch.hip b/pano360_amd/csrc/stitch.hip
--- a/pano360_amd/csrc/stitch.hip
+++ b/pano360_amd/csrc/stitch.hip
@@ -12,16 +12,18 @@
     long cap_blurred, long cap_scratch, int cap_tiles, int want_tiles, int b_nr, int b_vw,
     int b_vh, int b_aw, int b_ah, pano_patch *__restrict__ table,
     LayoutSummary *__restrict__ summary, LayoutSummary expect, int check_expect,
-    int *__restrict__ sticky) {
+    int *__restrict__ sticky, int gate_aw, int32_t *__restrict__ first, int first_stride,
+    int b_blocks0, int b_blocks1) {
     __shared__ long s_planes[LAY_THREADS], s_blurred[LAY_THREADS], s_scratch[LAY_THREADS];
     __shared__ int s_tiles[LAY_THREADS], s_slot[LAY_THREADS];
     __shared__ long s_run[4];
-    __shared__ int s_count, s_max[4], s_missing, s_bad;
+    __shared__ int s_count, s_max[4], s_missing, s_bad, s_slack[2], s_blocks[2];
     const int tid = threadIdx.x, stride = 5 + 2 * max_spans;
     if (tid == 0) {
         s_run[0] = s_run[1] = s_run[2] = s_run[3] = 0;
         s_count = s_missing = s_bad = 0;
         s_max[0] = s_max[1] = s_max[2] = s_max[3] = 0;
+        s_slack[0] = s_slack[1] = 0;
     }
     __syncthreads();
     const int total = n * max_spans;
@@ -100,12 +102,41 @@
             rec.scratch = scratch ? scratch + s_scratch[tid] : nullptr;
             rec.tiles_off = s_tiles[tid];
             table[k] = rec;
+            const int g = warp_record_gated(rec, gate_aw) ? 1 : 0;
+            first[g * first_stride + k] = warp_blocks_of(rec);
+            first[(1 - g) * first_stride + k] = 0;
+            atomicAdd(&s_slack[g], warp_blocks_slack(rec));
         }
         __syncthreads();
     }
     const int nr = s_count;
+    for (int k = (nr < b_nr ? nr : b_nr) + tid; k <= b_nr; k += LAY_THREADS)
+        first[k] = first[first_stride + k] = 0;
+    __threadfence_block();
+    __syncthreads();
+    if (tid < 64) {
+        int run[2] = {0, 0};
+        for (int t0 = 0; t0 <= b_nr; t0 += 64) {
+            const int t = t0 + tid;
+#pragma unroll
+            for (int q = 0; q < 2; ++q) {
+                const int own = t <= b_nr ? first[q * first_stride + t] : 0;
+                int v = own;
+#pragma unroll
+                for (int off = 1; off < 64; off <<= 1) {
+                    const int o = __shfl_up(v, off, 64);
+                    if (tid >= off) v += o;
+                }
+                if (t <= b_nr) first[q * first_stride + t] = run[q] + v - own;
+                run[q] += __shfl(v, 63, 64);
+            }
+        }
+        if (tid == 0) s_blocks[0] = run[0], s_blocks[1] = run[1];
+    }
+    __syncthreads();
     const long need_planes = s_run[0], need_blurred = s_run[1] + 32, need_scratch = s_run[2];
     int why = s_bad;
+    if (s_blocks[0] > b_blocks0 || s_blocks[1] > b_blocks1) why |= 2;
     if (need_planes > cap_planes || (n_blur > 0 && nr > 0 && (need_blurred > cap_blurred ||
                                                               need_scratch > cap_scratch)) ||
         (want_tiles && s_run[3] > cap_tiles))
@@ -114,6 +145,8 @@
     if (nr > b_nr) why |= 4;
     if (s_missing) why |= 16;
     for (int k = (why ? 0 : nr) + tid; k < b_nr; k += LAY_THREADS) table[k] = pano_patch{};
+    if (why)
+        for (int k = tid; k <= b_nr; k += LAY_THREADS) first[k] = first[first_stride + k] = 0;
     if (tid == 0) {
         LayoutSummary out;
         out.planes_floats = need_planes;
@@ -126,13 +159,16 @@
         out.ok = why == 0;
         out.why = why;
         out.pad = 0;
+        out.blocks[0] = s_blocks[0], out.blocks[1] = s_blocks[1];
+        out.slack[0] = s_slack[0], out.slack[1] = s_slack[1];
         *summary = out;
         if (check_expect &&
             !(out.ok && out.planes_floats == expect.planes_floats &&
               out.blurred_floats == expect.blurred_floats && out.scratch_floats == expect.scratch_floats &&
               out.n_records == expect.n_records && out.n_tiles == expect.n_tiles &&
               out.max_vw == expect.max_vw && out.max_vh == expect.max_vh && out.max_aw == expect.max_aw &&
-              out.max_ah == expect.max_ah && out.missing == 0))
+              out.max_ah == expect.max_ah && out.missing == 0 &&
+              out.blocks[0] == expect.blocks[0] && out.blocks[1] == expect.blocks[1]))
             *(volatile int *)sticky = 1;
     }
 }
@@ -157,8 +193,28 @@
     return PANO_OK;
 }
 
-static LayoutSummary layout_expectation(const pano_layout &v) {
+static int ensure_warp_first(pano_ctx *ctx, int cap) {
+    if (ctx->warp_first_dev && cap <= ctx->warp_first_cap) return PANO_OK;
+    PANO_HIP(hipDeviceSynchronize());
+    if (ctx->warp_first_dev) PANO_HIP(hipFree(ctx->warp_first_dev));
+    if (ctx->warp_first_host) PANO_HIP(hipHostFree(ctx->warp_first_host));
+    ctx->warp_first_dev = ctx->warp_first_host = nullptr;
+    ctx->warp_first_cap = 0;
+    const size_t bytes = 2 * ((size_t)cap + 1) * sizeof(int32_t);
+    PANO_HIP(hipMalloc((void **)&ctx->warp_first_dev, bytes));
+    PANO_HIP(hipHostMalloc((void **)&ctx->warp_first_host, bytes, hipHostMallocDefault));
+    ctx->warp_first_cap = cap;
+    return PANO_OK;
+}
+
+struct WarpLaunches {
+    int mode, blocks[2], slack[2];
+};
+
+static LayoutSummary layout_expectation(const pano_ctx *ctx) {
+    const pano_layout &v = ctx->lay_prev;
     LayoutSummary e = {};
+    e.blocks[0] = ctx->lay_prev_blocks[0], e.blocks[1] = ctx->lay_prev_blocks[1];
     e.planes_floats = v.planes_floats, e.blurred_floats = v.blurred_floats;
     e.scratch_floats = v.scratch_floats;
     e.n_records = v.n_records, e.n_tiles = v.n_tiles;
@@ -208,11 +264,12 @@
     } while (0)
 
 static int queue_tail(pano_ctx *ctx, pano_stitch_args *a, const pano_layout &lay, bool device_table,
-                      int need_choice, bool two_streams, bool interior, int n_blur, int tile_grid,
+                      WarpLaunches &wl, bool two_streams, bool interior, int n_blur, int tile_grid,
                       bool kept = false) {
     const hipStream_t s = ctx->stream;
     const bool use_blur = n_blur > 0 && lay.n_records > 0;
     const int nr = lay.n_records;
+    const int stride = ctx->warp_first_cap + 1;
     if (!device_table) {
         if (lay.planes_floats > a->planes_floats || (use_blur && lay.blurred_floats > a->blurred_floats) ||
             (use_blur && lay.scratch_floats > a->scratch_floats) ||
@@ -221,53 +278,81 @@
         PANO_REQUIRE(lay.planes_floats == 0 || a->planes, "pano_stitch_multiband: no plane arena");
         if (int rc = pano_layout_place(a->records_host, lay.n_records, a->planes, a->blurred, a->scratch))
             return rc;
+        int mode = 0;
+        if (interior && tile_grid == 32 && nr && a->tile_flags && a->need) {
+            mode = wl.mode == 1 ? 1 : 0;
+            if (wl.mode < 0) {
+                int gated = 0, live = 0;
+                for (int k = 0; k < nr; ++k) {
+                    if (warp_blocks_of(a->records_host[k]) == 0) continue;
+                    ++live;
+                    if (warp_record_gated(a->records_host[k], PANO_WARP_GATE_AW)) ++gated;
+                }
+                mode = gated == 0 ? 0 : gated == live ? 1 : 2;
+            }
+        }
+        wl = WarpLaunches{};
+        wl.mode = mode;
         if (nr) {
+            int32_t *first = ctx->warp_first_host;
+            if (int rc = pano_warp_blocks(a->records_host, nr, warp_gate_of_mode(mode), first, first + stride))
+                return rc;
+            wl.blocks[0] = first[nr], wl.blocks[1] = first[stride + nr];
+            for (int k = 0; k < nr; ++k)
+                wl.slack[warp_record_gated(a->records_host[k], warp_gate_of_mode(mode)) ? 1 : 0] +=
+                    warp_blocks_slack(a->records_host[k]);
+            PANO_HIP(hipMemcpyAsync(ctx->warp_first_dev, first, (size_t)(stride + nr + 1) * sizeof(int32_t),
+                                    hipMemcpyHostToDevice, s));
             PANO_HIP(hipMemcpyAsync(a->table, a->records_host, (size_t)nr * sizeof(pano_patch),
                                     hipMemcpyHostToDevice, s));
             PANO_HIP(hipEventRecord(ctx->ev_upload, s));
             ctx->upload_pending = true;
         }
     }
-    a->used_need = 0;
-    if (kept) {
-        a->used_need = need_choice == 1;
-        two_streams = false;
-    } else if (interior && tile_grid == 32 && nr && a->tile_flags && a->need) {
-        bool on = need_choice == 1;
-        if (need_choice < 0) {
-            double sum = 0.0;
-            for (int k = 0; k < nr; ++k) sum += a->records_host[k].aw;
-            on = sum / nr >= 768.0;
-        }
-        if (on) {
-            if (two_streams) {
-                PANO_HIP(hipEventRecord(ctx->ev_join, ctx->side));
-                PANO_HIP(hipStreamWaitEvent(s, ctx->ev_join, 0));
-            }
-            if (int rc = pano_blur_tiles(ctx, a->table, nr, lay.max_aw, lay.max_ah, a->W, a->radius,
-                                         a->interior, a->tile_flags, a->need))
-                return rc;
-            a->used_need = 1;
-        }
-    }
-    const bool fork2 = two_streams && interior && n_blur && nr &&
-                       !a->used_need && tile_grid == 32 && a->tile_flags;
+    const int mode = wl.mode;
+    const int gate = warp_gate_of_mode(mode);
+    a->used_need = mode != 0;
+    if (kept) two_streams = false;
+    if (!kept && mode == 1) {
+        if (two_streams) {
+            PANO_HIP(hipEventRecord(ctx->ev_join, ctx->side));
+            PANO_HIP(hipStreamWaitEvent(s, ctx->ev_join, 0));
+        }
+        if (int rc = pano_tiles_blur_mfma(ctx, a->table, nr, lay.max_aw, lay.max_ah, a->W, a->radius,
+                                          a->interior, a->tile_flags, a->need, gate))
+            return rc;
+    }
+    const bool fork2 = two_streams && interior && n_blur && nr && mode != 1 && tile_grid == 32 &&
+                       a->tile_flags;
     if (fork2) {
         if (device_table) {
             PANO_HIP(hipEventRecord(ctx->ev_upload, s));
         }
         PANO_HIP(hipStreamWaitEvent(ctx->side, ctx->ev_upload, 0));
+        if (mode == 2)
+            ON_SIDE(ctx, pano_tiles_blur_mfma(ctx, a->table, nr, lay.max_aw, lay.max_ah, a->W, a->radius,
+                                              a->interior, a->tile_flags, a->need, gate));
         ON_SIDE(ctx, pano_multiband_blur_prepare(ctx, a->table, nr, lay.max_aw, lay.max_ah, a->W,
                                                  a->interior, a->tile_flags));
         PANO_HIP(hipEventRecord(ctx->ev_join, ctx->side));
     } else if (two_streams && interior) {
         PANO_HIP(hipEventRecord(ctx->ev_join, ctx->side));
     }
-    if (int rc = pano_warp_windows(ctx, a->cams, a->table, nr, lay.max_vw, lay.max_vh, a->sin_t,
-                                   a->cos_t, a->tan_p, a->lut, a->lut_stride,
-                                   a->used_need ? a->need : nullptr))
-        return rc;
+    if (!kept && mode == 2 && !fork2)
+        if (int rc = pano_tiles_blur_mfma(ctx, a->table, nr, lay.max_aw, lay.max_ah, a->W, a->radius,
+                                          a->interior, a->tile_flags, a->need, gate))
+            return rc;
+    if (mode != 1)
+        if (int rc = pano_launch_warp_windows(ctx, a->cams, a->table, nr, lay.max_vw, lay.max_vh,
+                                              a->sin_t, a->cos_t, a->tan_p, a->lut, a->lut_stride,
+                                              nullptr, ctx->warp_first_dev, wl.blocks[0]))
+            return rc;
     if (two_streams && interior) PANO_HIP(hipStreamWaitEvent(s, ctx->ev_join, 0));
+    if (mode != 0)
+        if (int rc = pano_launch_warp_windows(ctx, a->cams, a->table, nr, lay.max_vw, lay.max_vh,
+                                              a->sin_t, a->cos_t, a->tan_p, a->lut, a->lut_stride,
+                                              a->need, ctx->warp_first_dev + stride, wl.blocks[1]))
+            return rc;
     if (kept && use_blur) {
         ctx->prepared_table = a->table;
         ctx->prepared_n = nr;
@@ -337,12 +422,16 @@
     const int stride = 5 + 2 * a->max_spans;
     int sig[STITCH_SIG];
     stitch_signature(a, tile_grid, sig);
+    if (int rc = ensure_warp_first(ctx, a->cap_records)) return rc;
 
     if (!resume) {
         bool spec = ctx->opt[PANO_OPT_STITCH_ASYNC] != 0 && interior && tile_grid == 32 &&
                     ctx->lay_prev_valid && memcmp(sig, ctx->lay_prev_sig, sizeof(sig)) == 0 &&
-                    ctx->lay_prev.n_records > 0 && a->planes && a->blurred && a->tile_flags;
+                    ctx->lay_prev.n_records > 0 && a->planes && a->blurred && a->tile_flags &&
+                    a->warp_need == ctx->lay_prev_choice;
         pano_layout bound = ctx->lay_prev;
+        WarpLaunches wl = {ctx->lay_prev_used_need,
+                           {ctx->lay_prev_blocks[0], ctx->lay_prev_blocks[1]}, {0, 0}};
         const bool want_keep = a->trust_layout == 3;
         const bool want_trust = a->trust_layout == 1 || want_keep;
         a->trust_layout = 0;
@@ -357,8 +446,8 @@
             const void *bufs[GEOM_BUFS];
             geometry_buffers(a, bufs);
             if (memcmp(bufs, ctx->geom_bufs, sizeof(bufs)) == 0) {
-                if (int rc = queue_tail(ctx, a, ctx->lay_prev, true, ctx->lay_prev_used_need, false,
-                                        interior, n_blur, tile_grid, true))
+                if (int rc = queue_tail(ctx, a, ctx->lay_prev, true, wl, false, interior, n_blur,
+                                        tile_grid, true))
                     return rc;
                 a->layout = ctx->lay_prev;
                 a->trust_layout = 4;
@@ -386,6 +475,7 @@
             if (!trusted) {
                 bound.n_records = bound.n_records + 2 < a->cap_records ? bound.n_records + 2 : a->cap_records;
                 bound.max_vw += 64, bound.max_vh += 64, bound.max_aw += 64, bound.max_ah += 64;
+                wl.blocks[0] += ctx->lay_prev_slack[0], wl.blocks[1] += ctx->lay_prev_slack[1];
             }
             if (ctx->opt[PANO_OPT_STITCH_ASYNC] == 2) {
                 bound.n_records = ctx->lay_prev.n_records > 1 ? ctx->lay_prev.n_records - 1 : 1;
@@ -416,8 +506,9 @@
                                (long)a->planes_floats, (long)a->blurred_floats,
                                (long)a->scratch_floats, a->cap_tiles, 1, bound.n_records,
                                bound.max_vw, bound.max_vh, bound.max_aw, bound.max_ah, a->table,
-                               ctx->lay_sum_host, layout_expectation(ctx->lay_prev), trusted ? 1 : 0,
-                               layout_sticky(ctx));
+                               ctx->lay_sum_host, layout_expectation(ctx), trusted ? 1 : 0,
+                               layout_sticky(ctx), warp_gate_of_mode(wl.mode), ctx->warp_first_dev,
+                               ctx->warp_first_cap + 1, wl.blocks[0], wl.blocks[1]);
             PANO_LAUNCH_CHECK("layout_windows_kernel");
             PANO_HIP(hipEventRecord(ctx->ev_regions, s));
             if (!trusted) {
@@ -431,12 +522,11 @@
                 if (int rc = stitch_interior_map(ctx, a, n_blur)) return rc;
                 interior_queued = true;
             }
-            if (int rc = queue_tail(ctx, a, bound, true, ctx->lay_prev_used_need, two_streams, interior,
-                                    n_blur, tile_grid))
+            if (int rc = queue_tail(ctx, a, bound, true, wl, two_streams, interior, n_blur, tile_grid))
                 return rc;
             if (trusted) {
                 a->layout = ctx->lay_prev;
-                a->used_need = ctx->lay_prev_used_need;
+                a->used_need = ctx->lay_prev_used_need != 0;
                 a->trust_layout = 2;
                 ctx->trusted_pending = true;
                 geometry_left(ctx, a);
@@ -455,7 +545,9 @@
             a->layout.missing = sum.missing;
             if (sum.ok) {
                 ctx->lay_prev = a->layout;
-                ctx->lay_prev_used_need = a->used_need;
+                ctx->lay_prev_used_need = wl.mode;
+                for (int q = 0; q < 2; ++q)
+                    ctx->lay_prev_blocks[q] = sum.blocks[q], ctx->lay_prev_slack[q] = sum.slack[q];
                 ctx->lay_prev_verified = true;
                 geometry_left(ctx, a);
                 ++ctx->lay_count[0];
@@ -486,12 +578,16 @@
             return PANO_EINVAL;
         }
     }
-    const int rc = queue_tail(ctx, a, a->layout, false, a->warp_need, two_streams, interior, n_blur,
+    WarpLaunches host_wl = {a->warp_need, {0, 0}, {0, 0}};
+    const int rc = queue_tail(ctx, a, a->layout, false, host_wl, two_streams, interior, n_blur,
                               tile_grid);
     if (rc == PANO_OK) {
         ctx->lay_prev = a->layout;
         memcpy(ctx->lay_prev_sig, sig, sizeof(sig));
-        ctx->lay_prev_used_need = a->used_need;
+        ctx->lay_prev_used_need = host_wl.mode;
+        ctx->lay_prev_choice = a->warp_need;
+        for (int q = 0; q < 2; ++q)
+            ctx->lay_prev_blocks[q] = host_wl.blocks[q], ctx->lay_prev_slack[q] = host_wl.slack[q];
         ctx->lay_prev_valid = true;
         ctx->lay_prev_verified = true;
         geometry_left(ctx, a);
@@ -512,7 +608,8 @@
                       sum.blurred_floats == v.blurred_floats && sum.scratch_floats == v.scratch_floats &&
                       sum.n_records == v.n_records && sum.n_tiles == v.n_tiles &&
                       sum.max_vw == v.max_vw && sum.max_vh == v.max_vh && sum.max_aw == v.max_aw &&
-                      sum.max_ah == v.max_ah && sum.missing == 0;
+                      sum.max_ah == v.max_ah && sum.missing == 0 &&
+                      sum.blocks[0] == ctx->lay_prev_blocks[0] && sum.blocks[1] == ctx->lay_prev_blocks[1];
     if (!same) {
         ctx->lay_prev_valid = ctx->lay_prev_verified = false;
         ctx->geom_valid = false;
diff --git a/pano360_amd/csrc/warp.hip b/pano360_amd/csrc/warp.hip
--- a/pano360_amd/csrc/warp.hip
+++ b/pano360_amd/csrc/warp.hip
@@ -1,4 +1,5 @@
 #include "geom.h"
+#include "layout.h"
 
 struct ProjK {
     double p[9];
@@ -48,19 +49,42 @@
 }
 
 #define WARP_ROWS 4
+static_assert(4 * WARP_ROWS == PANO_WARP_BH, "the layout counts blocks of this height");
 __global__ __launch_bounds__(256) void warp_windows_kernel(
     const pano_camera *__restrict__ cams, const pano_patch *__restrict__ patches,
     const double *__restrict__ sin_t, const double *__restrict__ cos_t,
     const double *__restrict__ tan_p, const float *__restrict__ lut, int lut_stride,
-    const uint8_t *__restrict__ need) {
+    const uint8_t *__restrict__ need, const int32_t *__restrict__ first, int n) {
     __shared__ float s_lut[256];
-    const pano_patch p = patches[blockIdx.z];
     constexpr int BH = 4 * WARP_ROWS;
-    if ((int)blockIdx.x * 64 >= p.vw || (int)blockIdx.y * BH >= p.vh) return;
+    int rec = blockIdx.z, bx = blockIdx.x, by = blockIdx.y, start = 0;
+    if (first) {
+        const int b = blockIdx.x;
+        rec = -1;
+        for (int base = 0; base <= n; base += 64) {
+            const int i = base + (int)threadIdx.x;
+            const int v = i <= n ? first[i] : 0x7fffffff;
+            const unsigned long long m = __ballot(v <= b);
+            if (m == 0ull) break;
+            const int c = __popcll(m);
+            rec = base + c - 1;
+            start = __builtin_amdgcn_readlane(v, c - 1);
+            if (c < 64) break;
+        }
+        if (rec < 0 || rec >= n) return;
+    }
+    const pano_patch p = patches[rec];
+    if (first) {
+        if (p.vw <= 0) return;
+        const int nbx = (p.vw + 63) >> 6, local = (int)blockIdx.x - start;
+        by = local / nbx;
+        bx = local - by * nbx;
+    }
+    if (bx * 64 >= p.vw || by * BH >= p.vh) return;
     if (need) {
         const int ntx = ((p.ax0 + p.aw - 1) >> 5) - (p.ax0 >> 5) + 1;
         const int nty = ((p.ay0 + p.ah - 1) >> 5) - (p.ay0 >> 5) + 1;
-        const int px0 = p.vx0 + (int)blockIdx.x * 64, py0 = p.vy0 + (int)blockIdx.y * BH;
+        const int px0 = p.vx0 + bx * 64, py0 = p.vy0 + by * BH;
         const int ty0 = min(max((py0 >> 5) - (p.ay0 >> 5), 0), nty - 1);
         const int ty1 = min(max(((py0 + BH - 1) >> 5) - (p.ay0 >> 5), 0), nty - 1);
         const int tx0 = min(max((px0 >> 5) - (p.ax0 >> 5), 0), ntx - 1);
@@ -74,8 +98,8 @@
         lut[(size_t)p.index * lut_stride + threadIdx.y * 64 + threadIdx.x];
     __syncthreads();
 
-    const int x = blockIdx.x * 64 + threadIdx.x;
-    const int y0 = blockIdx.y * BH + threadIdx.y;
+    const int x = bx * 64 + threadIdx.x;
+    const int y0 = by * BH + threadIdx.y;
     if (x >= p.vw || y0 >= p.vh) return;
     const pano_camera *cam = cams + p.index;
     const int sw = cam->sw, sh = cam->sh;
@@ -184,6 +208,21 @@
     return PANO_OK;
 }
 
+int pano_launch_warp_windows(pano_ctx *ctx, const pano_camera *cams, const pano_patch *patches,
+                             int n, int max_vw, int max_vh, const double *sin_t,
+                             const double *cos_t, const double *tan_p, const float *lut,
+                             int lut_stride, const uint8_t *need, const int32_t *first, int total) {
+    const hipStream_t stream = ctx->stream;
+    if (n == 0 || (first ? total <= 0 : (max_vw == 0 || max_vh == 0))) return PANO_OK;
+    dim3 block(64, 4), grid(ceil_div(max_vw, 64), ceil_div(max_vh, 4 * WARP_ROWS), n);
+    if (first) grid = dim3(total);
+    PANO_TIMED(PK_WARP_WINDOWS, stream,
+               hipLaunchKernelGGL(warp_windows_kernel, grid, block, 0, stream, cams, patches, sin_t,
+                                  cos_t, tan_p, lut, lut_stride, need, first, n));
+    PANO_LAUNCH_CHECK("warp_windows_kernel");
+    return PANO_OK;
+}
+
 extern "C" int pano_warp_windows(pano_ctx *ctx, const pano_camera *cams, const pano_patch *patches,
                                  int n, int max_vw, int max_vh, const double *sin_t,
                                  const double *cos_t, const double *tan_p, const float *lut,
@@ -193,11 +232,6 @@
                  "pano_warp_windows: null pointer");
     PANO_REQUIRE(n >= 0 && n <= 65535 && max_vw >= 0 && max_vh >= 0,
                  "pano_warp_windows: bad argument");
-    if (n == 0 || max_vw == 0 || max_vh == 0) return PANO_OK;
-    dim3 block(64, 4), grid(ceil_div(max_vw, 64), ceil_div(max_vh, 4 * WARP_ROWS), n);
-    PANO_TIMED(PK_WARP_WINDOWS, (hipStream_t)stream,
-               hipLaunchKernelGGL(warp_windows_kernel, grid, block, 0, (hipStream_t)stream,
-                                  cams, patches, sin_t, cos_t, tan_p, lut, lut_stride, need));
-    PANO_LAUNCH_CHECK("warp_windows_kernel");
-    return PANO_OK;
-}
+    return pano_launch_warp_windows(ctx, cams, patches, n, max_vw, max_vh, sin_t, cos_t, tan_p, lut,
+                                    lut_stride, need, nullptr, 0);
+}
```

Result: faster. 208,600 MP/s (median of 6 runs) (+1.2%).
